# xiaoxiaokuye/CODLAD

Measured on AMD Instinct MI355X. Metric: sampled all-atom structures/sec (100-step DDPM, PED), higher is better.
Workload: dtype f32 as f16x3 split (each fp32 operand = fp16 hi + fp16 lo, 22-bit; 3 f16 MFMAs per product, fp32 accumulate); everything outside the contractions fp32; 1 GPU; cfg2: PED-shaped test set, 4 proteins L=46/87/92/129 x 10 frames x num_ensemble 10 = 400 structures per GPU, 100-step DDPM (mpnn_diffusion) + VQ(4096x3) + IC_Decoder N6 + ic_to_xyz; structures_rank0=400, nodes_rank0=35400, edges_rank0=2182800, ddpm_steps=100, parallelism=replicas x1

## Files before the change

codlad_amd/_lib.py:

```python
import ctypes as C
import os

import torch

_HERE = os.path.dirname(os.path.abspath(__file__))
ABI_VERSION = 19
LIB_PATH = os.environ.get("CODLAD_HIP_LIB") or os.path.join(_HERE, "libcodlad_hip.so")

P = C.c_void_p


class EncLayer(C.Structure):
    _fields_ = [(n, P) for n in ("W1e", "W2", "W3", "W11e", "W12", "W13", "W1a", "W1c", "W11a", "W11c")] + \
               [("Win", P * 4), ("Wout", P * 4)] + \
               [(n, P) for n in ("b1", "b2", "b3", "b11", "b12", "b13", "b_in", "b_out")]


class DecLayer(C.Structure):
    _fields_ = [(n, P) for n in ("W1e", "W2", "W3", "W1a", "W1v", "TS")] + \
               [("Win", P * 4), ("Wout", P * 4)] + \
               [(n, P) for n in ("b1", "b2", "b3", "b_in", "b_out")]


class EncLayerH(C.Structure):
    _fields_ = [(n, P) for n in ("W1e", "W2", "W3", "W11e", "W12", "W13", "W1a", "W1c", "W11a", "W11c")] + \
               [("Win", P * 4), ("Wout", P * 4)] + \
               [(n, P) for n in ("b1", "b2", "b3", "b11", "b12", "b13", "b_in", "b_out")] + \
               [(n, C.c_int) for n in ("e1", "e2", "e3", "e11", "e12", "e13", "e_in", "e_out")]


class DecLayerH(C.Structure):
    _fields_ = [(n, P) for n in ("W1e", "W2", "W3", "W1a", "W1v")] + [("Win", P * 4), ("Wout", P * 4)] + \
               [(n, P) for n in ("TS", "b1", "b2", "b3", "b_in", "b_out")] + \
               [(n, C.c_int) for n in ("e1", "e2", "e3", "e_in", "e_out")]


class DenoiserWeights(C.Structure):
    _fields_ = [(n, P) for n in ("freqs", "rbf_mu", "t_w0", "t_b0", "t_w2", "t_b2")] + \
               [("ada_w", P * 7), ("ada_b", P * 7)] + \
               [(n, P) for n in ("x_in_w", "x_in_b", "pos_w", "pos_b", "edge_wT", "norm_w", "norm_b",
                                 "We_wT", "We_b", "out_w", "out_b")] + \
               [("enc", EncLayer * 3), ("dec", DecLayer * 3), ("precision", C.c_int),
                ("enc_h", EncLayerH * 3), ("dec_h", DecLayerH * 3), ("self_condition", C.c_int), ("out_dim", C.c_int)]


class Workspace(C.Structure):
    _fields_ = [(n, P) for n in ("hV", "hVenc", "S", "PQ", "hE", "status", "tile_list")] + [("n_tiles", C.c_int32), ("xcd_bounds", P)]


class JobDesc(C.Structure):
    _fields_ = [("node_info", P), ("n_nodes", C.c_int), ("E_idx", P), ("h_E0", P), ("E1", P), ("n_snodes", C.c_int),
                ("ws", C.POINTER(Workspace))]


class DecoderWeights(C.Structure):
    _fields_ = [("angle", C.c_int), ("map_out_w", P), ("map_out_b", P), ("res_embed", P)] + \
               [(n, P * 4) for n in ("inv0_w", "inv0_b", "inv1_w", "inv1_b", "dist_w", "dist_b",
                                     "dense1_w", "dense1_b", "dense3_w", "dense3_b")] + \
               [(n, P) for n in ("bb_dist", "sc_dist", "bb_ang1_w", "bb_ang1_b", "bb_ang3_w", "bb_ang3_b",
                                 "sc_angle_emb", "sc_ang1_w", "sc_ang1_b", "sc_ang3_w", "sc_ang3_b",
                                 "bb_tor1_w", "bb_tor1_b", "bb_tor3_w", "bb_tor3_b")] + \
               [(n, P * 4) for n in ("tor1_w", "tor1_b", "tor3_w", "tor3_b")] + \
               [(n, P) for n in ("fin1_w", "fin1_b", "fin3_w", "fin3_b")]


class TpConvArgs(C.Structure):
    _fields_ = [("ptr", P), ("snd", P), ("n_recv", C.c_int32), ("xyz_recv", P), ("xyz_snd", P), ("typ_recv", P),
                ("typ_snd", P), ("r_sign", C.c_float), ("smear_stop", C.c_float), ("emb0_w", P), ("emb0_b", P),
                ("emb3_w", P), ("emb3_b", P), ("emb_in", C.c_int32), ("h_recv", P), ("d_recv", C.c_int32), ("h_snd", P),
                ("d_snd", C.c_int32), ("attr_recv_first", C.c_int32), ("fc0_w", P), ("fc0_b", P), ("fc3_w", P),
                ("fc3_b", P), ("depth", C.c_int32), ("out", P), ("accumulate", C.c_int32), ("group", C.c_int32),
                ("packed", P)]


class XyzGroup(C.Structure):
    _fields_ = [("ca_full", P), ("ic", P), ("orders", P), ("slot_to_out", P), ("xyz_out", P),
                ("B", C.c_int32), ("L", C.c_int32), ("n_atoms", C.c_int32), ("first_row", C.c_int32)]


class MetricInputs(C.Structure):
    _fields_ = [("xyz_recon", P), ("xyz", P), ("n_atoms", C.c_int64),
                ("edge_list", P), ("n_edges", C.c_int64), ("clash_list", P), ("n_clash", C.c_int64),
                ("bb_NO_list", P), ("n_bb", C.c_int64), ("interaction_list", P), ("n_inter", C.c_int64),
                ("pi_pi_list", P), ("n_pipi", C.c_int64),
                ("ic", P), ("ic_recon", P), ("ic_mask", P), ("n_ic", C.c_int64)]


class LossTerms(C.Structure):
    _fields_ = [(n, P) for n in ("kl", "nll", "vb", "mse", "xstart_mse", "eps_mse", "pred_xstart")]


class FmLossOut(C.Structure):
    _fields_ = [(n, P) for n in ("l2", "l1", "huber", "smooth_l1", "log_cosh")]


class OdeState(C.Structure):
    _fields_ = [(n, C.c_double) for n in ("t", "h", "t_end", "ratio", "hh")] + \
               [(n, C.c_int32) for n in ("accepted", "n_accept", "n_reject", "clipped", "nonfinite", "status")] + \
               [("hh_f", C.c_float), ("tf", C.c_float * 6), ("pad_", C.c_float)]


class OdeDopri5Bufs(C.Structure):
    _fields_ = [("y", P), ("y1", P), ("xin", P), ("k", P * 7), ("mods", P), ("state", P), ("norm", P)]


FM_KINDS = {"icfm": 0, "target": 1, "vp": 2}
FM_TARGET_FLOW = 3
ODE_METHODS = {"euler": 0, "midpoint": 1, "rk4": 2}
GEOM_BOND_FLAG = 1 << 30
STEREO_COLUMNS, STEREO_N_COUNTS, STEREO_KIND_PRO = 9, 6, 1
STEREO_FLAGS = {"inverted_ca": 1, "inverted_side": 2, "cis": 4, "twisted": 8, "undefined": 16}
SASA_MAX_POINTS = 1024
DSSP_MAX_RES = 4096
DSSP_CODES = " HBEGITS"
DSSP_KIND_PRO, DSSP_KIND_CHAIN_START, DSSP_GEOM_LINK, DSSP_GEOM_BEND, DSSP_UNDEFINED = 1, 2, 1, 2, 255
SAXS_MAX_Q, SAXS_MAX_TYPES, SAXS_Q_CHUNK = 512, 32, 16
SAXS_X_MAX, SAXS_X_SMALL, SAXS_SIN_ULPS = 25600.0, 0.125, 5
SAXS_HYD_PARTIALS, SAXS_HYD_Q_CHUNK, SAXS_HYD_MAX_GRID = 6, 8, 4096
ODE_NORM_WORDS = 257

_JOB = [C.POINTER(DenoiserWeights), C.POINTER(JobDesc)]

_SIGS = {
    "codlad_abi_version": (C.c_int, []),
    "codlad_probe_edge_launches": (C.c_int, [C.c_int]),
    "codlad_probe_read": (C.c_int, [C.c_int, C.POINTER(C.c_double)]),
    "codlad_dispatch_read": (C.c_int, [P, C.c_int]),
    "codlad_metrics_scratch_bytes": (C.c_int, []),
    "codlad_eval_metrics": (C.c_int, [C.POINTER(MetricInputs), P, P, P]),
    "codlad_bond_graph_counts": (C.c_int, [P, P, P, P, P, C.c_int, C.c_int, C.c_float, P, P]),
    "codlad_ens_moments": (C.c_int, [P, C.c_int, C.c_int, P, C.c_int, P, P]),
    "codlad_ens_pair_msd": (C.c_int, [P, P, C.c_int, P, P, C.c_int, C.c_int, P, C.c_int, P, C.c_int, C.c_int, P, P, P]),
    "codlad_ens_apply": (C.c_int, [P, P, C.c_int, C.c_int, P, P]),
    "codlad_ens_pairwise": (C.c_int, [P, P, C.c_int, C.c_int, C.c_int, P, C.c_int, C.c_int, P, P]),
    "codlad_geometry_check": (C.c_int, [P, C.c_int, C.c_int, P, P, P, P, C.c_int, C.c_float, C.c_float, C.c_float, P, P, P]),
    "codlad_stereo_check": (C.c_int, [P, C.c_int, C.c_int, P, P, C.c_int, P, P, P, P]),
    "codlad_relax_scratch_bytes": (C.c_longlong, [C.c_int] * 5),
    "codlad_relax_energy": (C.c_int, [P, P, C.c_int, C.c_int, P, P, P, P, P, P, C.c_int, P, C.c_int, P, P, C.c_int] +
                            [C.c_float] * 4 + [P] * 5),
    "codlad_relax": (C.c_int, [P, C.c_int, C.c_int, P, P, P, P, P, P, C.c_int, P, C.c_int, P, P, C.c_int] +
                     [C.c_float] * 6 + [C.c_int] + [P] * 9),
    "codlad_sasa": (C.c_int, [P, C.c_int, C.c_int, P, P, P, C.c_int, P, C.c_int, P, P, P, P, P, P]),
    "codlad_contact_counts": (C.c_int, [P, C.c_int, C.c_int, P, C.c_int, C.c_float, P, P]),
    "codlad_dssp_hbonds": (C.c_int, [P, C.c_int, C.c_int, P, P, C.c_int, P, P, P, P, P, P, P, P]),
    "codlad_dssp_assign": (C.c_int, [P, P, P, P, C.c_int, C.c_int, P, P, P, P]),
    "codlad_saxs_debye": (C.c_int, [P, C.c_int, C.c_int, P, C.c_int, P, P, C.c_int, P, P, P, P, P]),
    "codlad_saxs_partials": (C.c_int, [P, C.c_int, C.c_int, P, C.c_int, P, P, P, P, C.c_int, P, P, P, P, P]),
    "codlad_saxs_hydration_fit": (C.c_int, [P, C.c_int, C.c_int, P, P, C.c_int, P, C.c_int, P, P, P, P, P, P, P, P]),
    "codlad_last_error": (C.c_char_p, []),
    "codlad_struct_sizes": (None, [C.POINTER(C.c_int)]),
    "codlad_pack_block_host": (None, [P, C.c_int, C.c_float, P]),
    "codlad_features_prepass": (C.c_int, [C.POINTER(DenoiserWeights), P, P, C.c_int, C.c_int, P, P, P]),
    "codlad_step_mods": (C.c_int, [C.POINTER(DenoiserWeights), P, C.c_int, P, P]),
    "codlad_step_mods_f": (C.c_int, [C.POINTER(DenoiserWeights), P, C.c_int, P, P]),
    "codlad_ode_combine": (C.c_int, [P, P, P, C.c_int, C.c_float, C.c_size_t, P, P]),
    "codlad_ode_error_norm": (C.c_int, [P, P, P, C.c_size_t, C.c_float, C.c_float, P, P]),
    "codlad_ode_loop": (C.c_int, _JOB + [P, P, P, C.c_int, P, C.c_int, P, P]),
    "codlad_ode_dopri5_attempt": (C.c_int, _JOB + [C.POINTER(OdeDopri5Bufs), C.c_double, C.c_float, C.c_float, P]),
    "codlad_layer0_edge_terms": (C.c_int, [C.POINTER(DenoiserWeights), P, C.c_int, P, P, P]),
    "codlad_denoiser_forward": (C.c_int, _JOB + [P, P, P, P, P]),
    "codlad_status_check": (C.c_int, [P, P]),
    "codlad_set_option": (C.c_int, [C.c_int, C.c_int]),
    "codlad_edge_plan_host": (C.c_int, [P, C.c_int, C.c_int, C.c_int, C.c_int, P, P]),
    "codlad_ddpm_update": (C.c_int, [P, P, P, P, C.c_int, P, P, P]),
    "codlad_ddpm_pred_xstart": (C.c_int, [P, P, P, C.c_int, P, P]),
    "codlad_ddpm_posterior_step": (C.c_int, [P, P, P, P, P, P, C.c_float, C.c_int, P, P, P]),
    "codlad_sample_loop": (C.c_int, _JOB + [P, P, P, P, P, C.c_int, P]),
    "codlad_sample_loop_pinned": (C.c_int, _JOB + [P, P, P, P, P, C.c_int, P, P, P]),
    "codlad_ddim_loop": (C.c_int, _JOB + [P, P, P, P, P, C.c_int, C.c_int, C.c_int, P, P, P]),
    "codlad_ddim_step": (C.c_int, [P, P, P, P, P, C.c_int, C.c_int, P, P, P]),
    "codlad_dpm_loop": (C.c_int, _JOB + [P, P, P, P, C.c_int, C.c_int, P, P, P]),
    "codlad_dpm_step": (C.c_int, [P, P, P, P, P, C.c_int, P, P, P]),
    "codlad_q_sample": (C.c_int, [P, P, P, C.c_int, P, C.c_int, P, C.c_int, P, P, P, P]),
    "codlad_q_posterior": (C.c_int, [P, P, P, C.c_int, P, C.c_int, P, C.c_int, P, P, P, P]),
    "codlad_vb_terms": (C.c_int, [P, P, P, P, P, C.c_int, P, C.c_int, P, C.c_int, C.POINTER(LossTerms), P]),
    "codlad_prior_bpd": (C.c_int, [P, P, C.c_int, P, C.c_int, P, P]),
    "codlad_loss_forward": (C.c_int, _JOB + [P, P, P, P, P, P, C.c_int, C.c_int, P, C.c_int, P, C.POINTER(LossTerms), P]),
    "codlad_bpd_loop": (C.c_int, _JOB + [P, P, P, P, P, C.c_int, P, C.c_int, P, P, P, P, P, P]),
    "codlad_fm_path": (C.c_int, [P, P, P, P, C.c_int, P, C.c_float, C.c_int, C.c_double, P, P, P]),
    "codlad_fm_terms": (C.c_int, [P, P, P, C.c_int, C.POINTER(FmLossOut), P]),
    "codlad_fm_loss_forward": (C.c_int, _JOB + [P, P, P, P, C.c_int, P, C.POINTER(FmLossOut), P]),
    "codlad_fm_loss_loop": (C.c_int, _JOB + [P, P, P, C.c_int, C.c_double, P, C.c_int, P, P, C.c_int, P, P,
                                             C.POINTER(FmLossOut), P]),
    "codlad_vq_lookup": (C.c_int, [P, C.c_int, P, P, P, C.c_int, P, P, P, P]),
    "codlad_ic_decode": (C.c_int, [C.POINTER(DecoderWeights), P, P, P, P, P, C.c_int, P, P, P]),
    "codlad_cg_graph": (C.c_int, [P, P, C.c_int, C.c_float, P, P, P, P]),
    "codlad_ic_to_xyz": (C.c_int, [P, P, P, P, C.c_int, C.c_int, C.c_int, P, P]),
    "codlad_ic_to_xyz_groups": (C.c_int, [P, C.c_int, C.c_int, P]),
    "codlad_xyz_to_ic": (C.c_int, [P, C.c_int, C.c_int, P, C.c_int, P, P]),
    "codlad_tp_conv_image_bytes": (C.c_int, [C.c_int]),
    "codlad_tp_conv_pack": (C.c_int, [P, P, P]),
    "codlad_receiver_csr": (C.c_int, [P, C.c_int, C.c_int, C.c_int, P, P, P, P]),
    "codlad_bench_edge_launch": (C.c_int, [C.POINTER(DenoiserWeights), P, C.c_int, P, P, P,
                                           C.POINTER(Workspace), C.c_int, C.c_int, P]),
    "codlad_tp_conv": (C.c_int, [C.POINTER(TpConvArgs), P]),
    "codlad_tp_conv_args_size": (C.c_int, []),
    "codlad_mlp_rows": (C.c_int, [P, C.c_int, C.c_int, P, P, C.c_int, P, P, C.c_int, C.c_int, C.c_int, P, P]),
    "codlad_bead_mean": (C.c_int, [P, P, P, P, C.c_int, P, P]),
    "codlad_embed_rows": (C.c_int, [P, P, C.c_int, C.c_int, P, P]),
    "codlad_selftest_gemm128": (C.c_int, [P, P, P, C.c_int, C.c_int, P, P]),
    "codlad_selftest_gemm128_h": (C.c_int, [P, P, P, C.c_int, C.c_int, C.c_int, P, P]),
}

_lib = None


def lib():
    global _lib
    if _lib is None:
        if not os.path.exists(LIB_PATH):
            raise RuntimeError(
                f"{LIB_PATH} is missing: the HIP extension is the only implementation of this path "
                "(build it with `python -m codlad_amd.build`)")
        handle = C.CDLL(LIB_PATH, mode=C.RTLD_GLOBAL)
        for name, (res, args) in _SIGS.items():
            try:
                fn = getattr(handle, name)
            except AttributeError:
                raise RuntimeError(f"{LIB_PATH} does not export {name}: it was built from an older include/codlad_hip.h "
                                   f"(ABI version {ABI_VERSION} covers additions); rebuild it") from None
            fn.restype = res
            fn.argtypes = args
        if handle.codlad_abi_version() != ABI_VERSION:
            raise RuntimeError("libcodlad_hip.so ABI version mismatch")
        _lib = handle
    return _lib


OPT_NODEQ_MAX_TILES, OPT_EDGE_TILE_MAX_NODES, OPT_DEC_EDGE_VARIANT, OPT_TP_CONV_VARIANT, OPT_EDGE_UPD_VARIANT, OPT_EDGE_CUS, OPT_EDGE_WIDE_MAX_TILES, OPT_NODE_QUAD_MAX_TILES = 0, 1, 3, 4, 5, 6, 7, 2
OPT_EDGE_PAIR = 8
EDGE_GRID = (256, 8)


def edge_plan(K, pair=True, grid=EDGE_GRID):
    import numpy as np
    K = np.ascontiguousarray(K, dtype=np.int32)
    bounds, stats = np.zeros(9, dtype=np.int32), np.zeros(20, dtype=np.int64)
    check(lib().codlad_edge_plan_host(K.ctypes.data_as(P), K.shape[0], grid[0], grid[1], int(bool(pair)),
                                      bounds.ctypes.data_as(P), stats.ctypes.data_as(P)), "codlad_edge_plan_host")
    return bounds, stats


DISPATCH_WORDS = ("edge", "node_in", "node_upd", "chunked_in", "chunked_upd", "grid_edge_msg", "grid_edge_upd", "grid_node_in",
                  "grid_node_upd")
EDGE_KINDS = ("f32", "wide", "tile", "node", "node_upd1")
NODE_KINDS = ("f32", "w", "q", "h4", "h8")


def dispatch_read():
    out = (C.c_int32 * len(DISPATCH_WORDS))()
    n = lib().codlad_dispatch_read(out, len(DISPATCH_WORDS))
    if n != len(DISPATCH_WORDS):
        raise RuntimeError(f"codlad_dispatch_read: the library keeps {n} words, this binding knows {len(DISPATCH_WORDS)}")
    rec = dict(zip(DISPATCH_WORDS, (int(v) for v in out)))
    rec["edge"] = EDGE_KINDS[rec["edge"]]
    rec["node_in"], rec["node_upd"] = NODE_KINDS[rec["node_in"]], NODE_KINDS[rec["node_upd"]]
    rec["chunked_in"], rec["chunked_upd"] = bool(rec["chunked_in"]), bool(rec["chunked_upd"])
    return rec


def set_option(option, value):
    check(lib().codlad_set_option(option, value), "codlad_set_option")


def exported_symbols():
    return list(_SIGS)


def check(rc, what):
    if rc != 0:
        msg = lib().codlad_last_error().decode() or "unknown error"
        raise RuntimeError(f"{what} failed (rc={rc}): {msg}")


class _TensorPtr(C.c_void_p):
    """c_void_p that keeps its tensor alive for as long as the argument object lives, i.e. until
    the foreign call has been enqueued.  (A bare integer would let a temporary such as
    `x.contiguous()` be freed - and its block reused by the next temporary - before the launch.)"""


def ptr(t):
    if t is None:
        return None
    assert t.is_contiguous(), "non-contiguous tensor handed to the C ABI"
    p = _TensorPtr(t.data_ptr())
    p._keepalive = t
    return p


def stream_ptr(device=None):
    return C.c_void_p(torch.cuda.current_stream(device).cuda_stream)
```

codlad_amd/csrc/denoiser_forward.hip:

```cpp
#include "node_args.h"
#include "sampler_args.h"
#include "loss_args.h"
#include "flow_loss_args.h"
#include "ode_args.h"

static struct {
    int32_t v[CODLAD_DISPATCH_WORDS] = {};
    int grid_word = -1, node_word = -1, chunked_word = -1;
} g_dispatch;

void dispatch_note(int grid, int stream_waves, bool chunked) {
    if (g_dispatch.grid_word >= 0) g_dispatch.v[g_dispatch.grid_word] = grid;
    if (g_dispatch.node_word >= 0 && stream_waves)
        g_dispatch.v[g_dispatch.node_word] = stream_waves == 8 ? CODLAD_NODE_KIND_H8 : CODLAD_NODE_KIND_H4;
    if (g_dispatch.chunked_word >= 0) g_dispatch.v[g_dispatch.chunked_word] = chunked;
    g_dispatch.grid_word = g_dispatch.node_word = g_dispatch.chunked_word = -1;
}

extern "C" int codlad_dispatch_read(int32_t *out, int n) {
    CODLAD_REQUIRE(out && n >= 0, "bad arguments");
    for (int i = 0; i < n && i < CODLAD_DISPATCH_WORDS; ++i) out[i] = g_dispatch.v[i];
    return CODLAD_DISPATCH_WORDS;
}

static void launch_edge_now(bool update, const EdgeArgs &ea, int precision, hipStream_t st, const int2 *tile_list,
                            int n_tiles) {
    const int terms = precision == 2 ? 3 : (precision == 1 ? 4 : 0);
    auto kind = [&](int k) {
        if (k > g_dispatch.v[CODLAD_DISPATCH_EDGE]) g_dispatch.v[CODLAD_DISPATCH_EDGE] = k;
        g_dispatch.grid_word = update ? CODLAD_DISPATCH_GRID_EDGE_UPD : CODLAD_DISPATCH_GRID_EDGE_MSG;
    };
    if (!terms) { kind(CODLAD_EDGE_KIND_F32); return launch_edge_f32(update, ea, st); }
    if (tile_list && n_tiles <= option_value(CODLAD_OPT_EDGE_WIDE_MAX_TILES)) {
        kind(CODLAD_EDGE_KIND_WIDE);
        return launch_edge_wide(terms, update, ea, tile_list, n_tiles, st);
    }
    if (tile_list) { kind(CODLAD_EDGE_KIND_TILE); return launch_edge_tile(terms, update, ea, tile_list, n_tiles, st); }
    if (update) {
        const bool two_tiles_each = n_tiles > 0 && 20ll * n_tiles >= 19ll * 2 * ea.n_nodes;
        const int variant = option_value(CODLAD_OPT_EDGE_UPD_VARIANT);
        if ((variant == 1 && two_tiles_each) || variant == 2) {
            kind(CODLAD_EDGE_KIND_NODE_UPD1);
            launch_edge_upd1(terms, ea, st);
        } else {
            kind(CODLAD_EDGE_KIND_NODE);
            launch_edge_upd(terms, ea, st);
        }
    } else {
        kind(CODLAD_EDGE_KIND_NODE);
        launch_edge_msg(terms, ea, st);
    }
}

#define PROBE_MAX 4096
static struct {
    bool on = false;
    int used = 0;
    hipEvent_t ev[PROBE_MAX][2] = {};
    bool made[PROBE_MAX] = {};
    int kind[PROBE_MAX] = {};
} g_probe;

static void launch_edge(bool update, const EdgeArgs &ea, int precision, hipStream_t st, const int2 *tile_list = nullptr,
                        int n_tiles = 0) {
    const int i = g_probe.used;
    bool rec = g_probe.on && i < PROBE_MAX;
    if (rec && !g_probe.made[i]) {
        rec = hipEventCreate(&g_probe.ev[i][0]) == hipSuccess && hipEventCreate(&g_probe.ev[i][1]) == hipSuccess;
        g_probe.made[i] = rec;
    }
    if (rec) (void)hipEventRecord(g_probe.ev[i][0], st);
    launch_edge_now(update, ea, precision, st, tile_list, n_tiles);
    if (rec) {
        (void)hipEventRecord(g_probe.ev[i][1], st);
        g_probe.kind[i] = (update ? 1 : 0) + (ea.E1 ? 2 : 0);
        g_probe.used = i + 1;
    }
}

extern "C" int codlad_probe_edge_launches(int enable) {
    g_probe.on = enable != 0;
    if (enable) g_probe.used = 0;
    return 0;
}

extern "C" int codlad_probe_read(int kind, double *total_ms) {
    CODLAD_REQUIRE(total_ms && kind >= 0 && kind < 4, "bad arguments");
    double sum = 0.0;
    int n = 0;
    for (int i = 0; i < g_probe.used; ++i) {
        if (g_probe.kind[i] != kind) continue;
        float ms = 0.f;
        hipError_t e = hipEventSynchronize(g_probe.ev[i][1]);
        if (e == hipSuccess) e = hipEventElapsedTime(&ms, g_probe.ev[i][0], g_probe.ev[i][1]);
        if (e != hipSuccess) { codlad_set_error("codlad_probe_read: %s", hipGetErrorString(e)); return -(int)e - 1000; }
        sum += ms;
        ++n;
    }
    *total_ms = sum;
    return n;
}

static void launch_node(bool upd, const NodeArgs &na, int precision, hipStream_t st) {
    const int terms = precision == 2 ? 3 : (precision == 1 ? 4 : 0);
    auto kind = [&](int k) {
        g_dispatch.node_word = upd ? CODLAD_DISPATCH_NODE_UPD : CODLAD_DISPATCH_NODE_IN;
        g_dispatch.v[g_dispatch.node_word] = k;
        g_dispatch.grid_word = upd ? CODLAD_DISPATCH_GRID_NODE_UPD : CODLAD_DISPATCH_GRID_NODE_IN;
        g_dispatch.chunked_word = upd ? CODLAD_DISPATCH_CHUNKED_UPD : CODLAD_DISPATCH_CHUNKED_IN;
    };
    if (!terms) { kind(CODLAD_NODE_KIND_F32); return launch_node_f32(upd, na, st); }
    const int tiles = (na.n_nodes + 31) / 32;
    if (upd && tiles <= option_value(CODLAD_OPT_NODE_QUAD_MAX_TILES)) {
        kind(CODLAD_NODE_KIND_Q);
        launch_node_quad(terms, na, st);
    } else if (tiles <= option_value(CODLAD_OPT_NODEQ_MAX_TILES)) {
        kind(CODLAD_NODE_KIND_W);
        launch_node_wide(terms, upd, na, st);
    } else {
        kind(CODLAD_NODE_KIND_H4);
        launch_node_stream(terms, tiles > 4 * num_cu() ? 8 : 4, upd, na, st);
    }
}

struct Job {
    const codlad_denoiser_weights *w;
    const int4 *ni;
    const int32_t *E_idx;
    int n_nodes;
    const codlad_workspace *ws;
    bool split;
    float *PQ(int k) const { return ws->PQ + (size_t)k * n_nodes * HD; }
};
static Job make_job(const codlad_denoiser_weights *w, const codlad_job *d) {
    return {w, reinterpret_cast<const int4 *>(d->node_info), d->E_idx, d->n_nodes, d->ws, w->precision != 0};
}

static EdgeArgs edge_args(const Job &j, const float *hE_in, bool in_by_src) {
    EdgeArgs ea = {};
    ea.node_info = j.ni; ea.E_idx = j.E_idx; ea.n_nodes = j.n_nodes;
    ea.hE_in = hE_in; ea.in_by_src = in_by_src;
    ea.pair = option_value(CODLAD_OPT_EDGE_PAIR) != 0;
    ea.xcd_bounds = ea.pair ? j.ws->xcd_bounds : nullptr;
    return ea;
}
template <class Layer, class LayerH>
static EdgeArgs msg_args(const Job &j, const Layer &L, const LayerH &Lh, const float *hE_in, bool in_by_src) {
    EdgeArgs ea = edge_args(j, hE_in, in_by_src);
    ea.P = j.PQ(0); ea.Q = j.PQ(1); ea.W1 = L.W1e; ea.W2 = L.W2; ea.S = j.ws->S;
    ea.W1h = Lh.W1e; ea.W2h = Lh.W2;
    ea.b2 = j.split ? Lh.b2 : L.b2;
    ea.gelu_a = gelu_consts(j.split ? Lh.e1 : 0);
    ea.gelu_b = gelu_consts(j.split ? Lh.e1 + Lh.e2 : 0);
    ea.res_scale = 1.0f; ea.ln_eps = 1e-6f;
    return ea;
}
static EdgeArgs upd_args(const Job &j, const codlad_enc_layer &L, const codlad_enc_layer_h &Lh, const float *hE_in,
                         bool in_by_src, const float *m) {
    EdgeArgs eu = edge_args(j, hE_in, in_by_src);
    eu.hE_out = j.ws->hE;
    eu.P = j.PQ(2); eu.Q = j.PQ(3); eu.W1 = L.W11e; eu.W2 = L.W12; eu.W3 = L.W13;
    eu.mods3 = m + 6 * HD;
    eu.W1h = Lh.W11e; eu.W2h = Lh.W12; eu.W3h = Lh.W13;
    eu.b2 = j.split ? Lh.b12 : L.b12; eu.b3 = j.split ? Lh.b13 : L.b13;
    const int E2 = j.split ? Lh.e11 + Lh.e12 : 0, E3 = j.split ? E2 + Lh.e13 : 0;
    eu.gelu_a = gelu_consts(j.split ? Lh.e11 : 0);
    eu.gelu_b = gelu_consts(E2);
    eu.res_scale = pow2i(E3);
    eu.ln_eps = 1e-6f * pow2i(2 * E3);
    return eu;
}

static void set_node_scales(NodeArgs &na, bool split, int e_msg, int e3, int e_in, int e_out) {
    na.s_scale = 0.015625f * pow2i(split ? -e_msg : 0);
    na.t_scale = 64.0f * pow2i(split ? -e3 : 0);
    na.ffn_scale = pow2i(split ? -(e_in + e_out) : 0);
    na.gelu_ffn = gelu_consts(split ? e_in : 0);
}
template <class Layer, class LayerH>
static NodeArgs node_update_args(const Job &j, const Layer &L, const LayerH &Lh, const float *mods, bool s_partials) {
    NodeArgs na = {};
    na.node_info = j.ni; na.n_nodes = j.n_nodes; na.S = j.ws->S; na.hV = j.ws->hV; na.s_partials = s_partials;
    na.W3 = L.W3; na.b3 = j.split ? Lh.b3 : L.b3; na.mods = mods;
    na.b_in = j.split ? Lh.b_in : L.b_in; na.b_out = j.split ? Lh.b_out : L.b_out;
    set_node_scales(na, j.split, Lh.e1 + Lh.e2, Lh.e3, Lh.e_in, Lh.e_out);
    na.blk_h[0] = Lh.W3;
    for (int c = 0; c < 4; ++c) {
        na.Win[c] = L.Win[c]; na.Wout[c] = L.Wout[c];
        na.blk_h[1 + 2 * c] = Lh.Win[c]; na.blk_h[2 + 2 * c] = Lh.Wout[c];
    }
    return na;
}
static void add_proj(NodeArgs &na, int blk0, const float *W, const void *Wh, const float *b, float *out) {
    const int p = na.n_proj++;
    na.proj_w[p] = W; na.proj_b[p] = b; na.proj_out[p] = out;
    na.blk_h[blk0 + p] = Wh;
}
static void add_proj_dec_q(NodeArgs &na, const Job &j, const codlad_dec_layer &D, const codlad_dec_layer_h &Dh) {
    na.proj_flags[na.n_proj] = 3; na.TS = j.split ? Dh.TS : D.TS;
    add_proj(na, 9, D.W1v, Dh.W1v, nullptr, j.PQ(1));
}

static void enqueue_forward(const codlad_denoiser_weights *w, const codlad_job *job, const float *x,
                            const float *x_self_cond, const float *mods_t, hipStream_t st) {
    const Job j = make_job(w, job);
    const codlad_workspace *ws = job->ws;
    const int n_nodes = job->n_nodes;
    const float *h_E0 = job->h_E0, *E1 = job->E1;
    g_dispatch = {};
    const bool tilewise = j.split && ws->tile_list && ws->n_tiles > 0 &&
                          (ws->n_tiles <= 8 * num_cu() || ws->n_tiles <= option_value(CODLAD_OPT_EDGE_WIDE_MAX_TILES)) &&
                          n_nodes <= option_value(CODLAD_OPT_EDGE_TILE_MAX_NODES);
    const int2 *tile_list = tilewise ? reinterpret_cast<const int2 *>(ws->tile_list) : nullptr;

    {
        NodeArgs na = {};
        na.node_info = j.ni; na.n_nodes = n_nodes;
        na.x = x; na.x_in_w = w->x_in_w; na.x_in_b = w->x_in_b; na.hV = ws->hV;
        na.x_sc = x_self_cond; na.in_dim = w->self_condition ? 6 : 3;
        add_proj(na, 0, w->enc[0].W1a, w->enc_h[0].W1a, j.split ? w->enc_h[0].b1 : w->enc[0].b1, j.PQ(0));
        add_proj(na, 0, w->enc[0].W1c, w->enc_h[0].W1c, nullptr, j.PQ(1));
        set_node_scales(na, j.split, 0, 0, 0, 0);
        launch_node(false, na, w->precision, st);
    }
    for (int l = 0; l < 3; ++l) {
        const codlad_enc_layer &L = w->enc[l];
        const codlad_enc_layer_h &Lh = w->enc_h[l];
        const float *m = mods_t + mods_offset(l);
        const float *hE_in = l == 0 ? h_E0 : ws->hE;
        EdgeArgs ea = msg_args(j, L, Lh, hE_in, l == 0);
        if (l == 0 && E1) ea.E1 = E1;
        launch_edge(false, ea, w->precision, st, tile_list, ws->n_tiles);

        NodeArgs na = node_update_args(j, L, Lh, m, tilewise);
        add_proj(na, 9, L.W11a, Lh.W11a, j.split ? Lh.b11 : L.b11, j.PQ(2));
        add_proj(na, 9, L.W11c, Lh.W11c, nullptr, j.PQ(3));
        if (l < 2) {
            add_proj(na, 9, w->enc[l + 1].W1a, w->enc_h[l + 1].W1a, j.split ? w->enc_h[l + 1].b1 : w->enc[l + 1].b1, j.PQ(0));
            add_proj(na, 9, w->enc[l + 1].W1c, w->enc_h[l + 1].W1c, nullptr, j.PQ(1));
        } else {
            add_proj(na, 9, w->dec[0].W1a, w->dec_h[0].W1a, j.split ? w->dec_h[0].b1 : w->dec[0].b1, j.PQ(0));
            add_proj_dec_q(na, j, w->dec[0], w->dec_h[0]);
            na.hVenc_out = ws->hVenc; na.venc_is_self = 1;
        }
        launch_node(true, na, w->precision, st);

        EdgeArgs eu = upd_args(j, L, Lh, hE_in, l == 0, m);
        if (l == 0 && E1) eu.E1 = E1 + (size_t)job->n_snodes * 64 * HD;
        launch_edge(true, eu, w->precision, st, tile_list, ws->n_tiles);
    }
    for (int l = 0; l < 3; ++l) {
        const codlad_dec_layer &L = w->dec[l];
        const codlad_dec_layer_h &Lh = w->dec_h[l];
        launch_edge(false, msg_args(j, L, Lh, ws->hE, false), w->precision, st, tile_list, ws->n_tiles);

        NodeArgs na = node_update_args(j, L, Lh, mods_t + mods_offset(3 + l), tilewise);
        if (l < 2) {
            add_proj(na, 9, w->dec[l + 1].W1a, w->dec_h[l + 1].W1a, j.split ? w->dec_h[l + 1].b1 : w->dec[l + 1].b1, j.PQ(0));
            add_proj_dec_q(na, j, w->dec[l + 1], w->dec_h[l + 1]);
            na.hVenc_in = ws->hVenc;
        }
        launch_node(true, na, w->precision, st);
    }
}

static int check_ws(const codlad_workspace *ws) {
    return ws && ws->hV && ws->hVenc && ws->S && ws->PQ && ws->hE;
}

static const char *job_defect(const codlad_denoiser_weights *w, const codlad_job *job) {
    if (!w || !job || !job->node_info || !job->E_idx || !job->h_E0) return "null pointer";
    if (job->n_nodes <= 0) return "n_nodes must be positive";
    if (!check_ws(job->ws)) return "incomplete workspace";
    return nullptr;
}
#define REQUIRE_OK(defect) do { const char *msg_ = (defect); CODLAD_REQUIRE(!msg_, msg_); } while (0)

static HeadArgs head_args(const codlad_denoiser_weights *w, const codlad_job *job, const float *mods_t) {
    return {job->ws->hV, mods_t + mods_offset(6), w->out_w, w->out_b, job->n_nodes};
}

static FinalArgs final_args(const codlad_denoiser_weights *w, const codlad_job *job, const float *mods_t) {
    FinalArgs fa = {head_args(w, job, mods_t)};
    fa.status = job->ws->status; fa.n_out = w->out_dim;
    return fa;
}

extern "C" int codlad_denoiser_forward(const codlad_denoiser_weights *w, const codlad_job *job, const float *x,
                                       const float *x_self_cond, const float *mods_t, float *out, void *stream) {
    REQUIRE_OK(job_defect(w, job));
    CODLAD_REQUIRE(x && mods_t && out, "null pointer");
    hipStream_t st = (hipStream_t)stream;
    CODLAD_REQUIRE(!x_self_cond || w->self_condition, "x_self_cond given to a model without self-conditioning");
    CODLAD_REQUIRE(w->out_dim == 6 || w->out_dim == 3, "out_dim must be 6 (diffusion) or 3 (flow matching)");
    enqueue_forward(w, job, x, x_self_cond, mods_t, st);
    FinalArgs fa = final_args(w, job, mods_t);
    fa.logits = out;
    launch_final(fa, CODLAD_STEP_DDPM, nullptr, nullptr, 0, st);
    return codlad_check_launch("codlad_denoiser_forward");
}

static void sample_loop(const codlad_denoiser_weights *w, const codlad_job *job, float *x, float *x_start,
                        const float *noise, const float *mods, const float *coef, int T, const float *pin_x0,
                        const uint8_t *pin_mask, void *stream, int step = CODLAD_STEP_DDPM, int mode = 0) {
    hipStream_t st = (hipStream_t)stream;
    const bool sc = w->self_condition != 0;
    const bool reverse = step == CODLAD_STEP_DDIM_REVERSE;
    for (int k = 0; k < T; ++k) {
        const int i = reverse ? k : T - 1 - k;
        const float *mods_t = mods + (size_t)i * CODLAD_MODS_PER_STEP;
        enqueue_forward(w, job, x, sc && k > 0 ? x_start : nullptr, mods_t, st);
        FinalArgs fa = final_args(w, job, mods_t);
        fa.x = x; fa.noise = noise ? noise + (size_t)k * job->n_nodes * 3 : nullptr;
        fa.coef = coef + (size_t)i * 8; fa.x_start = x_start;
        launch_final(fa, step, pin_x0, pin_mask, mode, st);
    }
}

static const char *ddpm_loop_defect(const codlad_denoiser_weights *w, const codlad_job *job, const float *x,
                                    const float *x_start, const float *noise, const float *mods, const float *coef, int T) {
    if (const char *msg = job_defect(w, job)) return msg;
    if (!x || !noise || !mods || !coef) return "null pointer";
    if (T <= 0) return "T must be positive";
    if (w->self_condition && !x_start) return "a self-conditioned model needs the x_start buffer";
    if (w->out_dim != 6 && w->out_dim != 3)
        return "the DDPM loop needs a model with 6 outputs (mean | variance logits) or 3 (fixed-variance samplers)";
    return nullptr;
}

extern "C" int codlad_sample_loop(const codlad_denoiser_weights *w, const codlad_job *job, float *x, float *x_start,
                                  const float *noise, const float *mods, const float *coef, int T, void *stream) {
    REQUIRE_OK(ddpm_loop_defect(w, job, x, x_start, noise, mods, coef, T));
    sample_loop(w, job, x, x_start, noise, mods, coef, T, nullptr, nullptr, stream);
    return codlad_check_launch("codlad_sample_loop");
}

extern "C" int codlad_sample_loop_pinned(const codlad_denoiser_weights *w, const codlad_job *job, float *x,
                                         float *x_start, const float *noise, const float *mods, const float *coef, int T,
                                         const float *pin_x0, const uint8_t *pin_mask, void *stream) {
    REQUIRE_OK(ddpm_loop_defect(w, job, x, x_start, noise, mods, coef, T));
    CODLAD_REQUIRE(pin_x0 && pin_mask, "null pointer (pin_x0 / pin_mask)");
    sample_loop(w, job, x, x_start, noise, mods, coef, T, pin_x0, pin_mask, stream);
    return codlad_check_launch("codlad_sample_loop_pinned");
}

extern "C" int codlad_ddim_loop(const codlad_denoiser_weights *w, const codlad_job *job, float *x, float *x_start,
                                const float *noise, const float *mods, const float *coef, int T, int mode, int reverse,
                                const float *pin_x0, const uint8_t *pin_mask, void *stream) {
    CODLAD_REQUIRE(w && x && mods && coef, "null pointer");
    CODLAD_REQUIRE(reverse || noise, "null pointer (noise: only the reverse loop runs without it)");
    CODLAD_REQUIRE(!pin_x0 == !pin_mask, "null pointer (pin_x0 and pin_mask come together)");
    CODLAD_REQUIRE(T > 0, "T must be positive");
    CODLAD_REQUIRE(mode >= 0 && mode <= (CODLAD_DDPM_START_X | CODLAD_DDPM_FIXED_VAR | CODLAD_DDPM_CLIP),
                   "unknown mode bits");
    CODLAD_REQUIRE(w->out_dim == ((mode & CODLAD_DDPM_FIXED_VAR) ? 3 : 6),
                   "mode and model disagree: a learned-range sampler needs a model with 6 outputs (mean | variance "
                   "logits), a fixed-variance one (mode bit 2) a model with 3");
    CODLAD_REQUIRE(!w->self_condition || x_start, "a self-conditioned model needs the x_start buffer");
    REQUIRE_OK(job_defect(w, job));
    sample_loop(w, job, x, x_start, noise, mods, coef, T, pin_x0, pin_mask, stream,
                reverse ? CODLAD_STEP_DDIM_REVERSE : CODLAD_STEP_DDIM, mode);
    return codlad_check_launch("codlad_ddim_loop");
}

extern "C" int codlad_dpm_loop(const codlad_denoiser_weights *w, const codlad_job *job, float *x, float *x_start,
                               const float *mods, const float *coef, int T, int mode, const float *pin_x0,
                               const uint8_t *pin_mask, void *stream) {
    CODLAD_REQUIRE(w && x && mods && coef, "null pointer");
    CODLAD_REQUIRE(x_start, "null pointer (x_start: the multistep update reads the previous step's pred_xstart from it)");
    CODLAD_REQUIRE(!pin_x0 == !pin_mask, "null pointer (pin_x0 and pin_mask come together)");
    CODLAD_REQUIRE(T > 0, "T must be positive");
    CODLAD_REQUIRE(mode >= 0 && mode <= (CODLAD_DDPM_START_X | CODLAD_DDPM_FIXED_VAR | CODLAD_DDPM_CLIP),
                   "unknown mode bits");
    CODLAD_REQUIRE(w->out_dim == ((mode & CODLAD_DDPM_FIXED_VAR) ? 3 : 6),
                   "mode and model disagree: a learned-range sampler needs a model with 6 outputs (mean | variance "
                   "logits), a fixed-variance one (mode bit 2) a model with 3");
    REQUIRE_OK(job_defect(w, job));
    sample_loop(w, job, x, x_start, nullptr, mods, coef, T, pin_x0, pin_mask, stream, CODLAD_STEP_DPM, mode);
    return codlad_check_launch("codlad_dpm_loop");
}

static LossArgs loss_args(const codlad_denoiser_weights *w, const codlad_job *job, const float *mods_t,
                          const float *x_start, const float *x_t, const float *noise, const LossSamples &s) {
    LossArgs la = {};
    la.head = final_args(w, job, mods_t);
    la.x0 = x_start; la.xt = x_t; la.noise = noise; la.s = s;
    return la;
}

static const char *loss_model_defect(const codlad_denoiser_weights *w, const codlad_job *job, int T, int n_samples) {
    if (const char *msg = job_defect(w, job)) return msg;
    if (T <= 0 || n_samples <= 0) return "T and n_samples must be positive";
    if (w->out_dim != 6 && w->out_dim != 3)
        return "the loss needs a model with 6 outputs (mean | variance logits) or 3 (fixed-variance samplers)";
    return nullptr;
}

extern "C" int codlad_loss_forward(const codlad_denoiser_weights *w, const codlad_job *job, const float *x_start,
                                   const float *x_t, const float *noise, const float *x_self_cond, const float *mods_t,
                                   const float *coef, int T, int t, const int32_t *sample_off, int n_samples,
                                   float *model_out, const codlad_loss_terms *terms, void *stream) {
    REQUIRE_OK(loss_model_defect(w, job, T, n_samples));
    CODLAD_REQUIRE(x_start && x_t && mods_t && coef && sample_off && terms, "null pointer");
    CODLAD_REQUIRE(t >= 0 && t < T, "t outside [0, T)");
    CODLAD_REQUIRE(!x_self_cond || w->self_condition, "x_self_cond given to a model without self-conditioning");
    hipStream_t st = (hipStream_t)stream;
    enqueue_forward(w, job, x_t, x_self_cond, mods_t, st);
    LossArgs la = loss_args(w, job, mods_t, x_start, x_t, noise, {sample_off, nullptr, t, T, n_samples, coef});
    la.head.logits = model_out;
    la.out = *terms;
    launch_loss(la, st);
    return codlad_check_launch("codlad_loss_forward");
}

extern "C" int codlad_bpd_loop(const codlad_denoiser_weights *w, const codlad_job *job, const float *x_start,
                               const float *noise, float *x_t, const float *mods, const float *coef, int T,
                               const int32_t *sample_off, int n_samples, float *vb, float *mse, float *xstart_mse,
                               float *prior_bpd, float *total_bpd, void *stream) {
    REQUIRE_OK(loss_model_defect(w, job, T, n_samples));
    CODLAD_REQUIRE(x_start && noise && x_t && mods && coef && sample_off, "null pointer");
    CODLAD_REQUIRE(vb && mse && xstart_mse && prior_bpd && total_bpd, "null pointer (results)");
    hipStream_t st = (hipStream_t)stream;
    for (int k = 0; k < T; ++k) {
        const int i = T - 1 - k;
        const LossSamples s = {sample_off, nullptr, i, T, n_samples, coef};
        const float *eps = noise + (size_t)k * job->n_nodes * 3;
        const float *mods_t = mods + (size_t)i * CODLAD_MODS_PER_STEP;
        launch_q_affine(x_start, eps, 8, 9, 10, 11, s, x_t, nullptr, nullptr, st);
        enqueue_forward(w, job, x_t, nullptr, mods_t, st);
        LossArgs la = loss_args(w, job, mods_t, x_start, x_t, eps, s);
        la.out.vb = vb + (size_t)i * n_samples;
        la.out.eps_mse = mse + (size_t)i * n_samples;
        la.out.xstart_mse = xstart_mse + (size_t)i * n_samples;
        launch_loss(la, st);
    }
    launch_prior(x_start, {sample_off, nullptr, T - 1, T, n_samples, coef}, vb, prior_bpd, total_bpd, st);
    return codlad_check_launch("codlad_bpd_loop");
}

static FmLossArgs fm_loss_args(const codlad_denoiser_weights *w, const codlad_job *job, const float *mods_t, const float *ut,
                               const int32_t *sample_off, int n_samples) {
    FmLossArgs la = {};
    la.head = final_args(w, job, mods_t);
    la.ut = ut; la.sample_off = sample_off; la.n_samples = n_samples;
    return la;
}

static const char *fm_model_defect(const codlad_denoiser_weights *w, const codlad_job *job, int n_samples) {
    if (const char *msg = job_defect(w, job)) return msg;
    if (n_samples <= 0) return "n_samples must be positive";
    if (w->out_dim != 3) return "the flow-matching losses need a flow-matching model (3 outputs: the velocity)";
    return nullptr;
}

extern "C" int codlad_fm_loss_forward(const codlad_denoiser_weights *w, const codlad_job *job, const float *xt,
                                      const float *ut, const float *mods_t, const int32_t *sample_off, int n_samples,
                                      float *model_out, const codlad_fm_loss_out *terms, void *stream) {
    REQUIRE_OK(fm_model_defect(w, job, n_samples));
    CODLAD_REQUIRE(xt && ut && mods_t && sample_off && terms, "null pointer");
    hipStream_t st = (hipStream_t)stream;
    enqueue_forward(w, job, xt, nullptr, mods_t, st);
    FmLossArgs la = fm_loss_args(w, job, mods_t, ut, sample_off, n_samples);
    la.head.logits = model_out;
    la.out = *terms;
    launch_fm_loss(la, st);
    return codlad_check_launch("codlad_fm_loss_forward");
}

extern "C" int codlad_fm_loss_loop(const codlad_denoiser_weights *w, const codlad_job *job, const float *x0, const float *x1,
                                   const float *eps, int kind, double sigma, const float *t_host, int K, const float *mods,
                                   const int32_t *sample_off, int n_samples, float *xt, float *ut,
                                   const codlad_fm_loss_out *tables, void *stream) {
    REQUIRE_OK(fm_model_defect(w, job, n_samples));
    CODLAD_REQUIRE(t_host && mods && sample_off && xt && ut && tables, "null pointer");
    CODLAD_REQUIRE(K > 0, "K must be positive");
    CODLAD_REQUIRE(kind != CODLAD_FM_TARGET_FLOW, "unknown matcher kind (the loop draws its own locations)");
    for (int k = 0; k < K; ++k) REQUIRE_OK(fm_path_defect(x0, x1, eps, nullptr, t_host[k], kind, sigma));
    hipStream_t st = (hipStream_t)stream;
    const size_t n3 = (size_t)job->n_nodes * 3;
    for (int k = 0; k < K; ++k) {
        const float *mods_t = mods + (size_t)k * CODLAD_MODS_PER_STEP;
        launch_fm_path(fm_path_args(x0, x1, eps ? eps + (size_t)k * n3 : nullptr, {sample_off, nullptr, t_host[k], n_samples},
                                    kind, sigma, xt, ut), st);
        enqueue_forward(w, job, xt, nullptr, mods_t, st);
        FmLossArgs la = fm_loss_args(w, job, mods_t, ut, sample_off, n_samples);
        const size_t row = (size_t)k * n_samples;
        la.out.l2 = tables->l2 ? tables->l2 + row : nullptr;
        la.out.l1 = tables->l1 ? tables->l1 + row : nullptr;
        la.out.huber = tables->huber ? tables->huber + row : nullptr;
        la.out.smooth_l1 = tables->smooth_l1 ? tables->smooth_l1 + row : nullptr;
        la.out.log_cosh = tables->log_cosh ? tables->log_cosh + row : nullptr;
        launch_fm_loss(la, st);
    }
    return codlad_check_launch("codlad_fm_loss_loop");
}

static OdeStageArgs ode_stage_args(const codlad_denoiser_weights *w, const codlad_job *job, const float *mods_t) {
    OdeStageArgs a = {head_args(w, job, mods_t)};
    a.status = job->ws->status; a.self = -1;
    return a;
}

struct OdeRow {
    int n_k;
    int k[4];
    double coef[4];
};
static const OdeRow ODE_EULER[1] = {{1, {0}, {1.0}}};
static const OdeRow ODE_MIDPOINT[2] = {{1, {0}, {0.5}}, {1, {1}, {1.0}}};
static const OdeRow ODE_RK4[4] = {{1, {0}, {1.0 / 3}},
                                  {2, {1, 0}, {1.0, -1.0 / 3}},
                                  {3, {0, 1, 2}, {1.0, -1.0, 1.0}},
                                  {4, {0, 1, 2, 3}, {0.125, 0.375, 0.375, 0.125}}};

extern "C" int codlad_ode_loop(const codlad_denoiser_weights *w, const codlad_job *job, const float *y, float *traj,
                               const float *mods, int method, const float *dt_host, int n_intervals, float *scratch,
                               void *stream) {
    REQUIRE_OK(job_defect(w, job));
    CODLAD_REQUIRE(y && traj && mods && dt_host && scratch, "null pointer");
    CODLAD_REQUIRE(n_intervals > 0, "n_intervals must be positive");
    CODLAD_REQUIRE(method >= CODLAD_ODE_EULER && method <= CODLAD_ODE_RK4, "unknown method id");
    CODLAD_REQUIRE(w->out_dim == 3, "the ODE samplers need a flow-matching model (3 outputs: the velocity)");
    hipStream_t st = (hipStream_t)stream;
    const OdeRow *rows = method == CODLAD_ODE_EULER ? ODE_EULER : (method == CODLAD_ODE_MIDPOINT ? ODE_MIDPOINT : ODE_RK4);
    const int stages = method == CODLAD_ODE_EULER ? 1 : (method == CODLAD_ODE_MIDPOINT ? 2 : 4);
    const size_t n3 = (size_t)job->n_nodes * 3;
    float *xin = scratch + 4 * n3;
    if (y != traj) {
        hipError_t e = hipMemcpyAsync(traj, y, n3 * sizeof(float), hipMemcpyDeviceToDevice, st);
        if (e != hipSuccess) {
            codlad_set_error("codlad_ode_loop: %s", hipGetErrorString(e));
            return (int)e;
        }
    }
    for (int i = 0; i < n_intervals; ++i) {
        const float *y_i = traj + (size_t)i * n3;
        for (int s = 0; s < stages; ++s) {
            const float *mods_t = mods + ((size_t)i * stages + s) * CODLAD_MODS_PER_STEP;
            enqueue_forward(w, job, s == 0 ? y_i : xin, nullptr, mods_t, st);
            OdeStageArgs a = ode_stage_args(w, job, mods_t);
            a.k_out = scratch + s * n3; a.y = y_i; a.h = dt_host[i];
            a.n_k = rows[s].n_k;
            for (int m = 0; m < a.n_k; ++m) {
                a.k[m] = scratch + rows[s].k[m] * n3;
                a.coef[m] = (float)rows[s].coef[m];
                if (rows[s].k[m] == s) a.self = m;
            }
            a.out = s == stages - 1 ? traj + (size_t)(i + 1) * n3 : xin;
            launch_ode_stage(a, st);
        }
    }
    return codlad_check_launch("codlad_ode_loop");
}

static const double DP_BETA[6][6] = {{1.0 / 5},
                                     {3.0 / 40, 9.0 / 40},
                                     {44.0 / 45, -56.0 / 15, 32.0 / 9},
                                     {19372.0 / 6561, -25360.0 / 2187, 64448.0 / 6561, -212.0 / 729},
                                     {9017.0 / 3168, -355.0 / 33, 46732.0 / 5247, 49.0 / 176, -5103.0 / 18656},
                                     {35.0 / 384, 0.0, 500.0 / 1113, 125.0 / 192, -2187.0 / 6784, 11.0 / 84}};
static const double DP_C_SOL[7] = {35.0 / 384, 0.0, 500.0 / 1113, 125.0 / 192, -2187.0 / 6784, 11.0 / 84, 0.0};
static const double DP_C_ERR[7] = {35.0 / 384 - 1951.0 / 21600, 0.0, 500.0 / 1113 - 22642.0 / 50085,
                                   125.0 / 192 - 451.0 / 720, -2187.0 / 6784 - -12231.0 / 42400,
                                   11.0 / 84 - 649.0 / 6300, -1.0 / 60.0};

extern "C" int codlad_ode_dopri5_attempt(const codlad_denoiser_weights *w, const codlad_job *job,
                                         const codlad_ode_dopri5_bufs *bufs, double t_end, float rtol, float atol,
                                         void *stream) {
    REQUIRE_OK(job_defect(w, job));
    CODLAD_REQUIRE(bufs, "null pointer");
    CODLAD_REQUIRE(bufs->y && bufs->y1 && bufs->xin && bufs->mods && bufs->state && bufs->norm, "null pointer (buffers)");
    for (int j = 0; j < 7; ++j) CODLAD_REQUIRE(bufs->k[j], "null pointer (slopes)");
    CODLAD_REQUIRE(w->out_dim == 3, "the ODE samplers need a flow-matching model (3 outputs: the velocity)");
    hipStream_t st = (hipStream_t)stream;
    const size_t n3 = (size_t)job->n_nodes * 3;
    const float *hh = &bufs->state->hh_f;
    launch_ode_times(bufs->state, t_end, (float)DP_BETA[0][0], bufs->y, bufs->k[0], bufs->xin, n3, st);
    const int rc = codlad_step_mods_f(w, bufs->state->tf, 6, bufs->mods, stream);
    if (rc) return rc;
    for (int i = 0; i < 6; ++i) {
        const float *mods_t = bufs->mods + (size_t)i * CODLAD_MODS_PER_STEP;
        enqueue_forward(w, job, bufs->xin, nullptr, mods_t, st);
        OdeStageArgs a = ode_stage_args(w, job, mods_t);
        a.k_out = bufs->k[i + 1]; a.y = bufs->y; a.h_dev = hh; a.self = i + 1;
        const double *coef = i < 5 ? DP_BETA[i + 1] : DP_C_SOL;
        a.n_k = i + 2;
        for (int m = 0; m < a.n_k; ++m) {
            a.k[m] = bufs->k[m];
            a.coef[m] = (float)coef[m];
        }
        a.out = i < 5 ? bufs->xin : bufs->y1;
        launch_ode_stage(a, st);
    }
    OdeNormArgs na = {};
    na.y = bufs->y; na.y1 = bufs->y1; na.h_dev = hh; na.n = n3; na.rtol = rtol; na.atol = atol; na.out = bufs->norm;
    na.state = bufs->state; na.status = job->ws->status;
    for (int m = 0; m < 7; ++m) {
        na.k[m] = bufs->k[m];
        na.c_err[m] = (float)DP_C_ERR[m];
    }
    launch_ode_norm(na, st);
    launch_ode_commit(bufs->state, bufs->y, bufs->y1, bufs->k[0], bufs->k[6], n3, st);
    return codlad_check_launch("codlad_ode_dopri5_attempt");
}

extern "C" int codlad_bench_edge_launch(const codlad_denoiser_weights *w, const int32_t *node_info,
                                        int n_nodes, const int32_t *E_idx, const float *h_E0,
                                        const float *mods_t, const codlad_workspace *ws, int which,
                                        int layer, void *stream) {
    const codlad_job desc = {node_info, n_nodes, E_idx, h_E0, nullptr, 0, ws}, *job = &desc;
    REQUIRE_OK(job_defect(w, job));
    CODLAD_REQUIRE(mods_t, "null pointer");
    CODLAD_REQUIRE((which == 0 || which == 1) && (layer == 0 || layer == 1), "bad arguments");
    const Job j = make_job(w, job);
    const codlad_enc_layer &L = w->enc[layer];
    const codlad_enc_layer_h &Lh = w->enc_h[layer];
    const float *hE_in = layer == 0 ? h_E0 : ws->hE;
    EdgeArgs ea = which == 0 ? msg_args(j, L, Lh, hE_in, layer == 0) : upd_args(j, L, Lh, hE_in, layer == 0, mods_t);
    ea.S = ws->S;
    launch_edge(which == 1, ea, w->precision, (hipStream_t)stream, nullptr, ws->n_tiles);
    return codlad_check_launch("codlad_bench_edge_launch");
}
```

codlad_amd/csrc/edge_args.h:

```cpp
#pragma once
#include "common.h"
#include "host_util.h"

#define HD 128

struct EdgeArgs {
    const int4 *node_info;
    const int32_t *E_idx;
    const float *hE_in;
    int in_by_src;
    const float *E1;
    float *hE_out;
    const float *P, *Q;
    const float *W1, *W2, *W3;
    const void *W1h, *W2h, *W3h;
    const float *b2, *b3;
    const float *mods3;
    float *S;
    int n_nodes;
    GeluK gelu_a, gelu_b;
    float res_scale, ln_eps;
    const int32_t *xcd_bounds;
    int pair;
};

struct EdgeTileArgs : EdgeArgs {
    const int2 *tile_list;
    int n_tiles;
};

#define LDS_BLOCK_U4 4096

constexpr int NODE_WG_TILE = 256;
constexpr int XCD_CHUNKED_NODE_KERNEL_MIN = 32768;
__host__ __device__ inline int xcd_chunk_nodes(int n_nodes) {
    const int g = n_nodes >= XCD_CHUNKED_NODE_KERNEL_MIN ? NODE_WG_TILE : 32;
    const int tiles = (n_nodes + g - 1) / g;
    return g * ((tiles + 7) / 8);
}

__host__ __device__ inline bool edge_node_eligible(int K) { return K <= 16 || (K > 32 && K <= 48); }
__host__ __device__ inline bool edge_pair_ok(int K, int K_next) {
    return K > 32 && K <= 48 && edge_node_eligible(K_next);
}
__host__ __device__ inline int edge_node_cost2(int K) { return K <= 32 ? 2 : (K <= 48 ? 3 : 4); }
constexpr int XCD_BOUND_GRANULE = 32;

struct NodeSpan {
    int first, end, stride;
};
__host__ __device__ inline NodeSpan node_span_of(int n_nodes, int nwaves, int wave, int nb, int b, const int32_t *bounds) {
    if (nb % 8) return {b * nwaves + wave, n_nodes, nb * nwaves};
    int lo, hi;
    if (bounds) {
        lo = bounds[b % 8];
        hi = bounds[b % 8 + 1];
    } else {
        const int chunk = xcd_chunk_nodes(n_nodes);
        lo = (b % 8) * chunk;
        hi = lo + chunk;
    }
    if (lo > n_nodes) lo = n_nodes;
    if (hi > n_nodes) hi = n_nodes;
    return {lo + (b / 8) * nwaves + wave, hi, (nb / 8) * nwaves};
}
DEV NodeSpan wave_node_span(int n_nodes, int nwaves, int wave, const int32_t *bounds = nullptr) {
    return node_span_of(n_nodes, nwaves, wave, gridDim.x, blockIdx.x, bounds);
}

constexpr int UPD_W1_KS = 3;
constexpr int EDGE_CONST_U4 = 4 * 32;
template <bool EDGE_UPDATE, int NWAVES>
constexpr int edge_lds_u4() {
    return 2 * LDS_BLOCK_U4 + (EDGE_UPDATE ? UPD_W1_KS * 512 : 0) + EDGE_CONST_U4 + NWAVES * 32;
}
```

codlad_amd/csrc/edge_msg_kernel.hip:

```cpp
#include "edge_args.h"

constexpr int MSG_PAIR_U4 = 32 + 64 + 16;

template <int NWAVES, bool HOISTED, int TERMS>
__global__ __launch_bounds__(NWAVES * 64, NWAVES / 4) void msg_kernel_h(EdgeArgs a) {
    extern __shared__ __align__(16) u32x4 wl[];
    constexpr int NT = NWAVES * 64;
    const int tid = threadIdx.x, lane = tid & 63, wave = __builtin_amdgcn_readfirstlane(tid >> 6);
    u32x4 *consts = wl + 2 * LDS_BLOCK_U4;
    {
        const u32x4 *g1 = reinterpret_cast<const u32x4 *>(a.W1h);
        const u32x4 *g2 = reinterpret_cast<const u32x4 *>(a.W2h);
        for (int i = tid; i < LDS_BLOCK_U4; i += NT) {
            if (!HOISTED) wl[i] = g1[i];
            wl[LDS_BLOCK_U4 + i] = g2[i];
        }
        if (tid < 32) consts[tid] = reinterpret_cast<const u32x4 *>(a.b2)[tid];
        u32x4 *rep = consts + EDGE_CONST_U4 + NWAVES * 32;
        if (tid < 128) {
            const unsigned bv = reinterpret_cast<const unsigned *>(a.b2)[tid];
            for (int q = 0; q < 4; ++q) rep[q * 128 + tid] = u32x4{bv, bv, bv, bv};
        }
    }
    __syncthreads();
    const u32x4 *w1 = wl, *w2 = wl + LDS_BLOCK_U4;
    const float *c_b2 = reinterpret_cast<const float *>(consts);
    const int h = lane >> 5, c = lane & 31;
    float2 *const Pslot0 = reinterpret_cast<float2 *>(consts + EDGE_CONST_U4 + wave * 32);
    float2 *const Pslot1 = reinterpret_cast<float2 *>(consts + EDGE_CONST_U4 + NWAVES * 32 + 4 * 128 + wave * MSG_PAIR_U4);
    float4 *wait_sum = reinterpret_cast<float4 *>(Pslot1 + 64) + lane;
    int *wait_j = reinterpret_cast<int *>(Pslot1 + 64 + 2 * 64) + lane;
    const NodeSpan span = wave_node_span(a.n_nodes, NWAVES, wave, a.xcd_bounds);
    const int stride = span.stride, n_end = span.end;
    int n = __builtin_amdgcn_readfirstlane(span.first);
    if (n >= n_end) return;

    const float *xsrc = HOISTED ? a.E1 : a.hE_in;
    const bool by_src = HOISTED || a.in_by_src;
    const float2 *Prows = reinterpret_cast<const float2 *>(a.P);

    int4 info = a.node_info[n];
    int src = __builtin_amdgcn_readfirstlane(info.x), base = __builtin_amdgcn_readfirstlane(info.y);
    int K = __builtin_amdgcn_readfirstlane(info.z);
    int jA = a.E_idx[(size_t)src * 64 + (c < K ? c : 0)];
    int jB = a.E_idx[(size_t)src * 64 + (32 + c < K ? 32 + c : 0)];
    int cs = 0;
    Pslot0[lane] = Prows[(size_t)n * 64 + lane];
    int half = 0;
    int ph = 0, wn = 0, wait_src = 0, wait_base = 0, wK = 0;
    Tile x, acc, t2;
    tile_load_edge<!HOISTED>(x, xsrc + (size_t)(by_src ? src : n) * EDGE_BLOCK, c < K ? c : 0, h);
    tile_load_row(acc, a.Q + (size_t)(base + jA) * HD, h);
    float sum[4] = {0.f, 0.f, 0.f, 0.f};
    const float4 *bias_rep = reinterpret_cast<const float4 *>(consts + EDGE_CONST_U4 + NWAVES * 32) + c;

    int4 ninfo = info;
    int nsrc = src, nbase = base, nK = K, njA = jA, njB = jB;
    float2 npv = {0.f, 0.f};
    for (;;) {
        const int n2 = n + stride;
        const bool next_node = n2 < n_end;
        const bool first_half = half == 0;
        if (first_half && next_node) ninfo = a.node_info[n2];
        {
            const float2 *pl = ((ph == 2 && c < 16) ? !cs : cs) ? Pslot1 : Pslot0;
            tile_add_row(acc, reinterpret_cast<const float *>(pl), h);
        }
        if (HOISTED) {
#pragma unroll
            for (int bo = 0; bo < 4; ++bo) acc.b[bo] += x.b[bo];
        } else {
            gemm128_h_lds<TERMS, false, false, true>(acc, x, w1, lane, a.gelu_a);
        }
        if (first_half && next_node) {
            nsrc = __builtin_amdgcn_readfirstlane(ninfo.x);
            nbase = __builtin_amdgcn_readfirstlane(ninfo.y);
            nK = __builtin_amdgcn_readfirstlane(ninfo.z);
            njA = a.E_idx[(size_t)nsrc * 64 + (c < nK ? c : 0)];
            njB = a.E_idx[(size_t)nsrc * 64 + (32 + c < nK ? 32 + c : 0)];
            npv = Prows[(size_t)n2 * 64 + lane];
        }
        const bool open_pair = a.pair && ph == 0 && first_half && next_node && edge_pair_ok(K, nK);
        const bool next_half = first_half && K > 32 && !open_pair;
        const bool shared_next = ph == 1 || (open_pair && nK <= 32);
        {
            int rep_off = 0;
            asm volatile("" : "+v"(rep_off));
            const float4 *br = bias_rep + rep_off;
#pragma unroll
            for (int bo = 0; bo < 4; ++bo)
#pragma unroll
                for (int q = 0; q < 4; ++q) {
                    const float4 bv = br[q * 128 + 32 * bo];
                    t2.b[bo][4 * q + 0] = bv.x; t2.b[bo][4 * q + 1] = bv.y;
                    t2.b[bo][4 * q + 2] = bv.z; t2.b[bo][4 * q + 3] = bv.w;
                }
        }
        gemm128_h_lds<TERMS, true, true>(t2, acc, w2, lane, a.gelu_a);
        {
            int fn = next_half ? n : (next_node ? n2 : n), fs = next_half ? src : nsrc;
            int fb = next_half ? base : nbase, fK = next_half ? K : nK;
            int sn = fn, ss = fs, sb = fb, sK = fK;
            int jl = next_half ? jB : njA, jh = jl;
            int lo_off = next_half ? 32 : 0, hi_off = lo_off;
            if (shared_next) {
                if (ph == 1) {
                    fn = wn; fs = wait_src; fb = wait_base; fK = wK;
                    sn = n; ss = src; sb = base; sK = K;
                    jl = *wait_j;
                    jh = __shfl(jB, lane - 16);
                } else {
                    fn = n; fs = src; fb = base; fK = K;
                    sn = n2; ss = nsrc; sb = nbase; sK = nK;
                    jl = jB;
                    jh = __shfl(njA, lane - 16);
                }
                lo_off = 32;
                hi_off = (sK > 32 ? 32 : 0) - 16;
            }
            const bool low = c < 16;
            const int want = (low ? lo_off : hi_off) + c;
            const int pe = want < (low ? fK : sK) ? want : 0;
            const float *fblk = xsrc + (size_t)(by_src ? fs : fn) * EDGE_BLOCK, *sblk = xsrc + (size_t)(by_src ? ss : sn) * EDGE_BLOCK;
            const int pq = low ? fb + jl : sb + jh;
            tile_load_edge<!HOISTED>(x, low ? fblk : sblk, pe, h);
            tile_load_row(acc, a.Q + (size_t)pq * HD, h);
            __builtin_amdgcn_sched_barrier(0);
        }
        tile_gelu(t2, a.gelu_b);
        const int cnt = K - 32 * half;
        if (ph == 2) {
            const int wcnt = wK - 32;
            const float4 ws4 = *wait_sum;
            const float wsum[4] = {ws4.x, ws4.y, ws4.z, ws4.w};
#pragma unroll
            for (int bo = 0; bo < 4; ++bo) {
                float s0 = 0.f, s1 = 0.f;
#pragma unroll
                for (int r = 0; r < 8; ++r) {
                    s0 += ((r & 3) + 8 * (r >> 2) + 4 * h < wcnt) ? t2.b[bo][r] : 0.f;
                    s1 += ((r & 3) + 8 * (r >> 2) + 4 * h < cnt) ? t2.b[bo][8 + r] : 0.f;
                }
                sum[bo] += s1;
                const float ws = wsum[bo] + s0;
                const float tot = ws + __shfl_xor(ws, 32);
                if (h == 0) a.S[(size_t)wn * HD + 32 * bo + c] = tot;
            }
        } else if (cnt >= 32) {
#pragma unroll
            for (int bo = 0; bo < 4; ++bo) {
                f32x2 s2 = tile_pair(t2.b[bo], 0);
#pragma unroll
                for (int r = 2; r < 16; r += 2) s2 += tile_pair(t2.b[bo], r);
                sum[bo] += s2.x + s2.y;
            }
        } else {
#pragma unroll
            for (int bo = 0; bo < 4; ++bo) {
                float s0 = 0.f;
#pragma unroll
                for (int r = 0; r < 16; ++r) s0 += ((r & 3) + 8 * (r >> 2) + 4 * h < cnt) ? t2.b[bo][r] : 0.f;
                sum[bo] += s0;
            }
        }
        if (next_half) {
            half = 1;
            if (ph == 1) ph = 2;
            continue;
        }
        if (open_pair) {
            *wait_sum = make_float4(sum[0], sum[1], sum[2], sum[3]);
            *wait_j = jB;
#pragma unroll
            for (int bo = 0; bo < 4; ++bo) sum[bo] = 0.f;
            wn = n; wait_src = src; wait_base = base; wK = K;
            ph = nK > 32 ? 1 : 2;
            cs ^= 1;
        } else {
#pragma unroll
            for (int bo = 0; bo < 4; ++bo) {
                const float tot = sum[bo] + __shfl_xor(sum[bo], 32);
                if (h == 0) a.S[(size_t)n * HD + 32 * bo + c] = tot;
                sum[bo] = 0.f;
            }
            if (!next_node) break;
            ph = 0;
        }
        n = n2; src = nsrc; base = nbase; K = nK; jA = njA; jB = njB;
        (cs ? Pslot1 : Pslot0)[lane] = npv;
        half = 0;
    }
}


template <int TERMS>
static void launch_msg_t(const EdgeArgs &ea, hipStream_t st) {
    static bool attr_set = false;
    constexpr int NW = 8;
    const size_t lds = 16 * (edge_lds_u4<false, NW>() + 4 * 128 + NW * MSG_PAIR_U4);
    static_assert(16 * (edge_lds_u4<false, NW>() + 4 * 128 + NW * MSG_PAIR_U4) <= 160 * 1024, "kernel exceeds the CU's LDS");
    if (!attr_set) {
        set_max_lds(reinterpret_cast<const void *>(msg_kernel_h<NW, false, TERMS>), lds);
        set_max_lds(reinterpret_cast<const void *>(msg_kernel_h<NW, true, TERMS>), lds);
        attr_set = true;
    }
    const int groups = (ea.n_nodes + NW - 1) / NW;
    dim3 grid(groups < edge_cus() ? groups : edge_cus()), block(NW * 64);
    dispatch_note(grid.x);
    if (ea.E1 != nullptr) hipLaunchKernelGGL((msg_kernel_h<NW, true, TERMS>), grid, block, lds, st, ea);
    else hipLaunchKernelGGL((msg_kernel_h<NW, false, TERMS>), grid, block, lds, st, ea);
}

void launch_edge_msg(int terms, const EdgeArgs &ea, hipStream_t st) {
    if (terms == 3) launch_msg_t<3>(ea, st);
    else launch_msg_t<4>(ea, st);
}
```

codlad_amd/csrc/edge_plan.hip:

```cpp
#include "edge_args.h"
#include <vector>

static int64_t chunk_walk(const int32_t *K, int lo, int hi, int stride, bool pair, int64_t *pairs) {
    int64_t tiles = 0;
    for (int w = 0; w < stride; ++w)
        for (int n = lo + w; n < hi; n += stride) {
            tiles += K[n] > 32 ? 2 : 1;
            if (pair && n + stride < hi && edge_pair_ok(K[n], K[n + stride])) {
                n += stride;
                tiles += (K[n] > 32 ? 2 : 1) - 1;
                if (pairs) ++*pairs;
            }
        }
    return tiles;
}

extern "C" int codlad_edge_plan_host(const int32_t *K_host, int n_nodes, int n_workgroups, int waves_per_workgroup,
                                     int pair, int32_t *bounds_host, int64_t *stats_host) {
    CODLAD_REQUIRE(K_host && n_nodes > 0 && n_workgroups > 0 && waves_per_workgroup > 0, "bad arguments");
    int32_t bounds[9];
    const int G = XCD_BOUND_GRANULE, ng = (n_nodes + G - 1) / G;
    std::vector<int64_t> upto(ng + 1, 0);
    int64_t plain = 0;
    for (int n = 0; n < n_nodes; ++n) {
        CODLAD_REQUIRE(K_host[n] >= 1 && K_host[n] <= 64, "K outside 1..64");
        plain += K_host[n] > 32 ? 2 : 1;
        upto[n / G + 1] += pair ? edge_node_cost2(K_host[n]) : (K_host[n] > 32 ? 4 : 2);
    }
    for (int g = 0; g < ng; ++g) upto[g + 1] += upto[g];
    const int64_t total = upto[ng];
    const bool chunked = n_workgroups % 8 == 0;
    const int stride = chunked ? n_workgroups / 8 * waves_per_workgroup : n_workgroups * waves_per_workgroup;
    auto node_of = [&](int g) { return g * G < n_nodes ? g * G : n_nodes; };
    if (pair) {
        double target = total / 16.0;
        for (int pass = 0; pass < (chunked ? 3 : 1); ++pass) {
            bounds[0] = 0;
            int g = 0;
            int64_t done = 0;
            for (int x = 1; x < 8; ++x) {
                const int g0 = g;
                if (pass == 0) {
                    while (g < ng && 8 * upto[g + 1] <= total * x) ++g;
                    if (g < ng && 8 * upto[g + 1] - total * x < total * x - 8 * upto[g]) ++g;
                } else {
                    auto f = [&](int gg) { return (double)(done + chunk_walk(K_host, node_of(g0), node_of(gg), stride, true, nullptr)); };
                    const double want = target * x;
                    while (g < ng && f(g) < want) ++g;
                    while (g > g0 && f(g - 1) >= want) --g;
                    if (g > g0 && want - f(g - 1) < f(g) - want) --g;
                }
                bounds[x] = node_of(g);
                if (chunked) done += chunk_walk(K_host, node_of(g0), node_of(g), stride, true, nullptr);
            }
            bounds[8] = n_nodes;
            if (chunked) target = (done + chunk_walk(K_host, bounds[7], n_nodes, stride, true, nullptr)) / 8.0;
        }
    } else {
        const int chunk = xcd_chunk_nodes(n_nodes);
        for (int x = 0; x <= 8; ++x) bounds[x] = (int64_t)x * chunk < n_nodes ? x * chunk : n_nodes;
    }
    if (bounds_host)
        for (int x = 0; x <= 8; ++x) bounds_host[x] = bounds[x];
    if (stats_host) {
        int64_t walk = 0, pairs = 0;
        for (int x = 0; x < 8; ++x) {
            const int lo = (bounds[x] + G - 1) / G, hi = (bounds[x + 1] + G - 1) / G;
            stats_host[4 + x] = upto[hi] - upto[lo];
            stats_host[12 + x] = chunked ? chunk_walk(K_host, bounds[x], bounds[x + 1], stride, pair != 0, &pairs) : 0;
            walk += stats_host[12 + x];
        }
        if (!chunked) walk = chunk_walk(K_host, 0, n_nodes, stride, pair != 0, &pairs);
        stats_host[0] = plain;
        stats_host[1] = total;
        stats_host[2] = walk;
        stats_host[3] = pairs;
    }
    return 0;
}
```

codlad_amd/csrc/edge_upd_kernel.hip:

```cpp
#include "edge_args.h"

template <int NWAVES, bool HOISTED, int TERMS>
__global__ __launch_bounds__(NWAVES * 64, NWAVES / 4) void upd_kernel_h(EdgeArgs a) {
    extern __shared__ __align__(16) u32x4 wl[];
    constexpr int NT = NWAVES * 64;
    constexpr int W1_U4 = UPD_W1_KS * 512;
    const int tid = threadIdx.x, lane = tid & 63, wave = __builtin_amdgcn_readfirstlane(tid >> 6);
    u32x4 *consts = wl + 2 * LDS_BLOCK_U4 + W1_U4;
    {
        const u32x4 *g1 = reinterpret_cast<const u32x4 *>(a.W1h);
        const u32x4 *g2 = reinterpret_cast<const u32x4 *>(a.W2h);
        const u32x4 *g3 = reinterpret_cast<const u32x4 *>(a.W3h);
        for (int i = tid; i < LDS_BLOCK_U4; i += NT) {
            wl[i] = g2[i];
            wl[LDS_BLOCK_U4 + i] = g3[i];
        }
        if (!HOISTED)
            for (int i = tid; i < W1_U4; i += NT) wl[2 * LDS_BLOCK_U4 + i] = g1[i];
        if (tid < 32) consts[tid] = reinterpret_cast<const u32x4 *>(a.b2)[tid];
        if (tid >= 64 && tid < 96) consts[32 + (tid & 31)] = reinterpret_cast<const u32x4 *>(a.b3)[tid & 31];
        if (tid >= 128 && tid < 160) {
            const float4 *m = reinterpret_cast<const float4 *>(a.mods3);
            const int i = tid & 31;
            const float4 s = m[i], c = m[32 + i], g = m[64 + i];
            float4 *cf = reinterpret_cast<float4 *>(consts);
            cf[64 + i] = make_float4(g.x * (1.0f + c.x), g.y * (1.0f + c.y), g.z * (1.0f + c.z), g.w * (1.0f + c.w));
            cf[96 + i] = make_float4(g.x * s.x, g.y * s.y, g.z * s.z, g.w * s.w);
        }
    }
    __syncthreads();
    const u32x4 *w2 = wl, *w3 = wl + LDS_BLOCK_U4, *w1 = wl + 2 * LDS_BLOCK_U4;
    const float *c_base = reinterpret_cast<const float *>(consts);
    float *Pslot = reinterpret_cast<float *>(consts + EDGE_CONST_U4 + wave * 32);
    const int h = lane >> 5, c = lane & 31;
    const NodeSpan span = wave_node_span(a.n_nodes, NWAVES, wave, a.xcd_bounds);
    int pend_n = -1, pend_src = 0, pend_base = 0, pend_K = 0;
    for (int nv = span.first; nv < span.end; nv += span.stride) {
        const int n = __builtin_amdgcn_readfirstlane(nv);
        const int4 info = a.node_info[n];
        const int src = __builtin_amdgcn_readfirstlane(info.x), base = __builtin_amdgcn_readfirstlane(info.y);
        const int K = __builtin_amdgcn_readfirstlane(info.z);
        const int Ku = K, lh = Ku > 32;
        const bool paired = pend_n >= 0;
        bool open_pair = false;
        if (a.pair && !paired && Ku > 32 && Ku <= 48 && n + span.stride < span.end)
            open_pair = edge_pair_ok(Ku, __builtin_amdgcn_readfirstlane(a.node_info[n + span.stride].z));
        const bool ptA = paired && !lh, ptB = paired && lh;
        const bool lowA = ptA && c < 16, lowB = ptB && c < 16;
        const int wantA = ptA ? (c < 16 ? 32 + c : c - 16) : c, wantB = ptB ? 32 + (c & 15) : 32 + c;
        const bool validA = wantA < (lowA ? pend_K : K), validB = wantB < (lowB ? pend_K : K);
        const int colA = validA ? wantA : 0, colB = validB ? wantB : 0;
        const int jA = a.E_idx[(size_t)(lowA ? pend_src : src) * 64 + colA];
        const int jB = a.E_idx[(size_t)(lowB ? pend_src : src) * 64 + colB];
        reinterpret_cast<float2 *>(Pslot)[lane] = reinterpret_cast<const float2 *>(a.P + (size_t)n * HD)[lane];

        for (int half = 0; half < 2; ++half) {
            if (32 * half >= K) break;
            if (half && open_pair) break;
            const bool ptile = half ? ptB : ptA, low = half ? lowB : lowA;
            const bool valid = half ? validB : validA;
            const int colc = half ? colB : colA;
            const int j = half ? jB : jA;
            const int base_l = low ? pend_base : base;
            const float *rows_n = a.hE_in + (size_t)(a.in_by_src ? src : n) * EDGE_BLOCK;
            const float *rows_p = a.hE_in + (size_t)(a.in_by_src ? pend_src : pend_n) * EDGE_BLOCK;
            const float *rows = low ? rows_p : rows_n;
            float *out_rows = a.hE_out + (size_t)(low ? pend_n : n) * EDGE_BLOCK;
            Tile x, acc, t2;
            StreamedGemm<TERMS, UPD_W1_KS, 8 - UPD_W1_KS, false, 8, true> tail1;
            float2 pend_p = {0.f, 0.f};
            if (ptile) pend_p = reinterpret_cast<const float2 *>(a.P + (size_t)pend_n * HD)[lane];
            if (!HOISTED) tail1.start(a.W1h, lane);
            int lds_off = 0;
            asm volatile("" : "+v"(lds_off));
            const float *c_b2 = c_base + lds_off, *c_b3 = c_b2 + HD;
            const float *c_modA = c_b2 + 2 * HD, *c_modB = c_b2 + 3 * HD;
            tile_load_row(acc, a.Q + (size_t)(base_l + j) * HD, h);
            if (!low) tile_add_row(acc, Pslot, h);
            if (ptile) {
                reinterpret_cast<float2 *>(Pslot)[lane] = pend_p;
                if (low) tile_add_row(acc, Pslot, h);
            }
            if (!HOISTED) tile_load_edge<true>(x, rows, colc, h);
            if (HOISTED) {
                tile_add_edge(acc, low ? a.E1 + (size_t)pend_src * EDGE_BLOCK : a.E1 + (size_t)src * EDGE_BLOCK, colc, h);
                __builtin_amdgcn_sched_barrier(0);
                tile_load_edge<false>(x, rows, colc, h);
            } else {
                gemm_h_lds<TERMS, 0, UPD_W1_KS, false, false, true>(acc, x, w1, lane, a.gelu_a);
                tail1.run(acc, x, lane, a.gelu_a);
            }
            tile_load_row(t2, c_b2, h);
            gemm128_h_lds<TERMS, true>(t2, acc, w2, lane, a.gelu_a);
            tile_unsplit_scale_add_row(x, a.res_scale, c_b3, h);
            gemm128_h_lds<TERMS, true>(x, t2, w3, lane, a.gelu_b);
            tile_layernorm_affine(x, a.ln_eps, c_modA, c_modB, h);
            tile_presplit(x);
            if (valid) tile_store_edge<true>(x, out_rows, colc, h);
        }
        if (open_pair) {
            pend_n = n;
            pend_src = src;
            pend_base = base;
            pend_K = K;
        } else pend_n = -1;
    }
}


template <int TERMS>
static void launch_upd_t(const EdgeArgs &ea, hipStream_t st) {
    static bool attr_set = false;
    constexpr int NW = 8;
    const size_t lds = 16 * edge_lds_u4<true, NW>();
    static_assert(16 * edge_lds_u4<true, NW>() <= 160 * 1024, "kernel exceeds the CU's LDS");
    if (!attr_set) {
        set_max_lds(reinterpret_cast<const void *>(upd_kernel_h<NW, false, TERMS>), lds);
        set_max_lds(reinterpret_cast<const void *>(upd_kernel_h<NW, true, TERMS>), lds);
        attr_set = true;
    }
    const int groups = (ea.n_nodes + NW - 1) / NW;
    dim3 grid(groups < edge_cus() ? groups : edge_cus()), block(NW * 64);
    dispatch_note(grid.x);
    if (ea.E1 != nullptr) hipLaunchKernelGGL((upd_kernel_h<NW, true, TERMS>), grid, block, lds, st, ea);
    else hipLaunchKernelGGL((upd_kernel_h<NW, false, TERMS>), grid, block, lds, st, ea);
}

void launch_edge_upd(int terms, const EdgeArgs &ea, hipStream_t st) {
    if (terms == 3) launch_upd_t<3>(ea, st);
    else launch_upd_t<4>(ea, st);
}
```

codlad_amd/csrc/host_util.h:

```cpp
#pragma once
#include <hip/hip_runtime.h>
#include "../../include/codlad_hip.h"

struct EdgeArgs;
struct NodeArgs;
struct FinalArgs;

int num_cu();
void set_max_lds(const void *fn, size_t bytes);
hipError_t codlad_take_attr_error();
int option_value(int opt);
int edge_cus();
void codlad_set_error(const char *fmt, ...);
inline int codlad_hip_failed(const char *what, hipError_t e) {
    codlad_set_error("%s: %s", what, hipGetErrorString(e));
    return (int)e;
}
void dispatch_note(int grid, int stream_waves = 0, bool chunked = false);

void launch_edge_f32(bool update, const EdgeArgs &ea, hipStream_t st);
void launch_node_f32(bool upd, const NodeArgs &na, hipStream_t st);
void launch_edge_tile(int terms, bool update, const EdgeArgs &ea, const int2 *tile_list, int n_tiles, hipStream_t st);
void launch_edge_wide(int terms, bool update, const EdgeArgs &ea, const int2 *tile_list, int n_tiles, hipStream_t st);
void launch_edge_msg(int terms, const EdgeArgs &ea, hipStream_t st);
void launch_edge_upd(int terms, const EdgeArgs &ea, hipStream_t st);
void launch_edge_upd1(int terms, const EdgeArgs &ea, hipStream_t st);
void launch_node_wide(int terms, bool upd, const NodeArgs &na, hipStream_t st);
void launch_node_quad(int terms, const NodeArgs &na, hipStream_t st);
void launch_node_stream(int terms, int waves, bool upd, const NodeArgs &na, hipStream_t st);
void launch_final(const FinalArgs &fa, int step, const float *pin_x0, const uint8_t *pin_mask, int mode, hipStream_t st);
void launch_tp_conv_mfma(const codlad_tp_conv_args &a, hipStream_t st);
void launch_tp_conv_pack(const codlad_tp_conv_args &a, void *image, hipStream_t st);
int tp_conv_image_bytes(int depth);
```

codlad_amd/csrc/host_util.hip:

```cpp
#include "host_util.h"
#include "common.h"
#include <stdlib.h>

int num_cu() {
    static int n_cu = 0;
    if (!n_cu) {
        int dev = 0, n = 0;
        if (hipGetDevice(&dev) != hipSuccess ||
            hipDeviceGetAttribute(&n, hipDeviceAttributeMultiprocessorCount, dev) != hipSuccess || n <= 0)
            n = 256;
        n_cu = n;
    }
    return n_cu;
}

static hipError_t g_attr_error = hipSuccess;
void set_max_lds(const void *fn, size_t bytes) {
    const hipError_t e = hipFuncSetAttribute(fn, hipFuncAttributeMaxDynamicSharedMemorySize, (int)bytes);
    if (e != hipSuccess && g_attr_error == hipSuccess) g_attr_error = e;
}
hipError_t codlad_take_attr_error() {
    const hipError_t e = g_attr_error;
    g_attr_error = hipSuccess;
    return e;
}

struct Option {
    int id;
    const char *env;
    int (*dflt)();
    int value = -1;
};
static Option g_options[] = {
    {CODLAD_OPT_NODEQ_MAX_TILES, "CODLAD_NODEQ_MAX_TILES", [] { return 256; }},
    {CODLAD_OPT_EDGE_TILE_MAX_NODES, "CODLAD_EDGE_TILE_MAX_NODES", [] { return 1 << 30; }},
    {CODLAD_OPT_NODE_QUAD_MAX_TILES, "CODLAD_NODE_QUAD_MAX_TILES", [] { return 2 * num_cu(); }},
    {CODLAD_OPT_DEC_EDGE_VARIANT, "CODLAD_DEC_EDGE_VARIANT", [] { return 0; }},
    {CODLAD_OPT_TP_CONV_VARIANT, "CODLAD_TP_CONV_VARIANT", [] { return 0; }},
    {CODLAD_OPT_EDGE_UPD_VARIANT, "CODLAD_EDGE_UPD_VARIANT", [] { return 0; }},
    {CODLAD_OPT_EDGE_CUS, "CODLAD_EDGE_CUS", [] { return 0; }},
    {CODLAD_OPT_EDGE_WIDE_MAX_TILES, "CODLAD_EDGE_WIDE_MAX_TILES", [] { return 22 * num_cu(); }},
    {CODLAD_OPT_EDGE_PAIR, "CODLAD_EDGE_PAIR", [] { return 1; }},
};
static_assert(sizeof(g_options) / sizeof(g_options[0]) == CODLAD_N_OPTIONS, "one row per CODLAD_OPT_*");

int option_value(int opt) {
    Option &o = g_options[opt];
    if (o.id != opt) abort();
    if (o.value < 0) {
        const char *e = getenv(o.env);
        o.value = e ? atoi(e) : o.dflt();
    }
    return o.value;
}

extern "C" int codlad_set_option(int option, int value) {
    CODLAD_REQUIRE(option >= 0 && option < CODLAD_N_OPTIONS && value >= 0, "unknown option or negative value");
    g_options[option].value = value;
    return 0;
}

int edge_cus() {
    const int v = option_value(CODLAD_OPT_EDGE_CUS);
    return v > 0 && v < num_cu() ? v : num_cu();
}
```

codlad_amd/engine.py:

```python
import ctypes as C
import os

import numpy as np
import torch

from . import _lib
from .weights import DEFAULT_PRECISION, DenoiserWeights, DecoderWeights

H = 128
KNN = 64
MODS = 6016


def _require_cuda(t, what):
    if not t.is_cuda:
        raise RuntimeError(f"{what} must live on the GPU: this path has no CPU implementation")


def edge_rows(blocks, split=False):
    lead = blocks.shape[:-4]
    if not split:
        return blocks.permute(*range(len(lead)), -4, -2, -3, -1).reshape(*lead, 64, -1)
    hv = blocks.contiguous().view(torch.float16).view(*lead, 2, 4, 2, 2, 2, 32, 8)
    val = hv[..., 0, :, :, :].float() + hv[..., 1, :, :, :].float()
    n = len(lead)
    val = val.permute(*range(n), n, n + 4, n + 1, n + 2, n + 3, n + 5)
    out = torch.empty(*lead, 2, 32, 4, 2, 16, dtype=torch.float32, device=blocks.device)
    for h in range(2):
        out[..., 4 * h:4 * h + 4] = val[..., h, 0:4]
        out[..., 8 + 4 * h:8 + 4 * h + 4] = val[..., h, 4:8]
    return out.reshape(*lead, 64, 128)


class Structures:

    def __init__(self, xyz_list, z_list, device):
        self.lens = [int(x.shape[0]) for x in xyz_list]
        assert all(L >= 1 for L in self.lens)
        self.offsets = np.concatenate([[0], np.cumsum(self.lens)]).astype(np.int64)
        self.n_snodes = int(self.offsets[-1])
        self.xyz = torch.cat([x.reshape(-1, 3).float() for x in xyz_list]).contiguous().to(device)
        self.z = torch.cat([z.reshape(-1).to(torch.int32) for z in z_list]).contiguous().to(device)
        info = np.empty((self.n_snodes, 2), dtype=np.int32)
        for f, L in enumerate(self.lens):
            info[self.offsets[f]:self.offsets[f + 1], 0] = self.offsets[f]
            info[self.offsets[f]:self.offsets[f + 1], 1] = L
        self.snode_info = torch.from_numpy(info).to(device)
        self.E_idx = None
        self.h_E0 = None
        self.E1 = None
        self.features_tag = None


class Job:

    def __init__(self, structures, sample_struct, device, edge_state=None):
        st = structures
        self.structures = st
        self.device = device
        self._parts = {}
        self.sample_struct = [int(s) for s in sample_struct]
        lens = [st.lens[f] for f in self.sample_struct]
        self.sample_lens = lens
        self.sample_off = np.concatenate([[0], np.cumsum(lens)]).astype(np.int64)
        self.n_nodes = int(self.sample_off[-1])
        info = np.empty((self.n_nodes, 4), dtype=np.int32)
        z_host = st.z.cpu().numpy()
        for s, f in enumerate(self.sample_struct):
            a, b = self.sample_off[s], self.sample_off[s + 1]
            L = lens[s]
            info[a:b, 0] = np.arange(st.offsets[f], st.offsets[f] + L)
            info[a:b, 1] = a
            info[a:b, 2] = min(KNN, L)
            info[a:b, 3] = z_host[st.offsets[f]:st.offsets[f] + L]
        assert info[:, 3].min() >= 0 and info[:, 3].max() < 30, "residue type outside W_s vocabulary"
        self.node_info = torch.from_numpy(info).to(device)
        n = self.n_nodes
        f32 = dict(dtype=torch.float32, device=device)
        self.hV = torch.empty(n, H, **f32)
        self.hVenc = torch.empty(n, H, **f32)
        self.S = torch.empty(4, n, H, **f32)
        self.PQ = torch.empty(4, n, H, **f32)
        self.hE = torch.empty(n, KNN, H, **f32) if edge_state is None else edge_state
        assert tuple(self.hE.shape) == (n, KNN, H) and self.hE.is_contiguous()
        self.status = torch.zeros(1, dtype=torch.int32, device=device)
        halves = np.where(info[:, 2] > 32, 2, 1)
        tiles = np.empty((int(halves.sum()), 2), dtype=np.int32)
        tiles[:, 0] = np.repeat(np.arange(n, dtype=np.int32), halves)
        first = np.cumsum(halves) - halves
        tiles[:, 1] = np.arange(tiles.shape[0], dtype=np.int32) - np.repeat(first, halves).astype(np.int32)
        self.tile_list = torch.from_numpy(tiles).to(device)
        ws = _lib.Workspace()
        ws.hV, ws.hVenc, ws.S, ws.PQ, ws.hE, ws.status, ws.tile_list = (
            _lib.ptr(t) for t in (self.hV, self.hVenc, self.S, self.PQ, self.hE, self.status, self.tile_list))
        ws.n_tiles = tiles.shape[0]
        self.xcd_bounds = torch.from_numpy(_lib.edge_plan(info[:, 2])[0]).to(device)
        ws.xcd_bounds = _lib.ptr(self.xcd_bounds)
        self.ws = ws

    def workspace_bytes(self):
        return 4 * (self.hV.numel() * 2 + self.S.numel() + self.PQ.numel() + self.hE.numel())

    def desc(self):
        st = self.structures
        d = _lib.JobDesc()
        d.node_info, d.n_nodes = _lib.ptr(self.node_info), self.n_nodes
        d.E_idx, d.h_E0, d.E1, d.n_snodes = _lib.ptr(st.E_idx), _lib.ptr(st.h_E0), _lib.ptr(st.E1), st.n_snodes
        d.ws = C.pointer(self.ws)
        return d

    def sub_job(self, members, start):
        n = int(sum(self.sample_lens[m] for m in members))
        sub = Job(self.structures, [self.sample_struct[m] for m in members], self.device,
                  edge_state=self.hE[start:start + n])
        idx = np.concatenate([np.arange(self.sample_off[m], self.sample_off[m + 1]) for m in members])
        return sub, torch.from_numpy(idx).to(self.device)

    def parts(self, k=2):
        if k not in self._parts:
            subs, start = [], 0
            for p in range(k):
                subs.append(self.sub_job(range(p, len(self.sample_struct), k), start))
                start += subs[-1][0].n_nodes
            self._parts[k] = subs
        return self._parts[k]


class Denoiser:

    def __init__(self, state_dict, device, precision=DEFAULT_PRECISION, block_exponents=True, self_condition=False,
                 out_dim=6):
        self.device = torch.device(device)
        if self.device.type != "cuda":
            raise RuntimeError("codlad_amd runs on an MI355X only; no CPU path exists")
        self.lib = _lib.lib()
        if state_dict is None:
            self.weights = DenoiserWeights.empty(self.device, self_condition, out_dim, precision)
        else:
            self.weights = DenoiserWeights(state_dict, self.device, precision, block_exponents=block_exponents)
        self._mods_cache = {}
        self._mods_generation = self.weights.generation

    def new_structures(self, xyz_list, z_list, hoist_layer0=True):
        st = Structures(xyz_list, z_list, self.device)
        st.E_idx = torch.empty(st.n_snodes, KNN, dtype=torch.int32, device=self.device)
        st.h_E0 = torch.empty(st.n_snodes, 2, H // 4, KNN // 2, 4, dtype=torch.float32, device=self.device)
        if hoist_layer0:
            st.E1 = torch.empty(2, st.n_snodes, 2, H // 4, KNN // 2, 4, dtype=torch.float32, device=self.device)
        return st

    def compute_features(self, st):
        rc = self.lib.codlad_features_prepass(C.byref(self.weights.struct), _lib.ptr(st.xyz),
                                              _lib.ptr(st.snode_info), st.n_snodes, max(st.lens),
                                              _lib.ptr(st.E_idx), _lib.ptr(st.h_E0),
                                              _lib.stream_ptr(self.device))
        _lib.check(rc, "codlad_features_prepass")
        if st.E1 is not None:
            rc = self.lib.codlad_layer0_edge_terms(C.byref(self.weights.struct), _lib.ptr(st.snode_info),
                                                   st.n_snodes, _lib.ptr(st.h_E0), _lib.ptr(st.E1),
                                                   _lib.stream_ptr(self.device))
            _lib.check(rc, "codlad_layer0_edge_terms")
        st.features_tag = self.features_tag()
        return st

    @property
    def split_edge_state(self):
        return self.weights.precision != "f32"

    def features_tag(self):
        if self.weights.precision == "f32":
            return ("f32", self.weights.generation)
        ex = self.weights.exponents["enc0"]
        return ("split", self.weights.precision, ex["e1"], ex["e11"], self.weights.generation)

    def _fresh_features(self, st):
        if st.features_tag != self.features_tag():
            self.compute_features(st)

    def prepare_structures(self, xyz_list, z_list, hoist_layer0=True):
        return self.compute_features(self.new_structures(xyz_list, z_list, hoist_layer0))

    def make_job(self, structures, sample_struct):
        return Job(structures, sample_struct, self.device)

    def step_mods(self, t_values, refresh=False, as_float=False):
        fractional = as_float or any(float(t) != int(t) for t in t_values)
        key = tuple(float(t) for t in t_values) if fractional else tuple(int(t) for t in t_values)
        if self._mods_generation != self.weights.generation:
            self._mods_cache.clear()
            self._mods_generation = self.weights.generation
        if refresh or key not in self._mods_cache:
            mods = torch.empty(len(key), MODS, dtype=torch.float32, device=self.device)
            if fractional:
                tv = torch.tensor(key, dtype=torch.float32, device=self.device)
                rc = self.lib.codlad_step_mods_f(C.byref(self.weights.struct), _lib.ptr(tv), len(key),
                                                 _lib.ptr(mods), _lib.stream_ptr(self.device))
            else:
                tv = torch.tensor(key, dtype=torch.int64, device=self.device)
                rc = self.lib.codlad_step_mods(C.byref(self.weights.struct), _lib.ptr(tv), len(key),
                                               _lib.ptr(mods), _lib.stream_ptr(self.device))
            _lib.check(rc, "codlad_step_mods")
            if len(self._mods_cache) > 64:
                self._mods_cache.clear()
            self._mods_cache[key] = mods
        return self._mods_cache[key]

    @property
    def self_condition(self):
        return self.weights.self_condition

    def _run(self, name, desc, *args):
        rc = getattr(self.lib, name)(C.byref(self.weights.struct), C.byref(desc), *args, _lib.stream_ptr(self.device))
        _lib.check(rc, name)

    def _n_streams(self, job, streams):
        if streams is not None:
            return streams
        return 2 if job.n_nodes >= self.SPLIT_MIN_NODES and len(job.sample_struct) >= 2 else 1

    def check_status(self, job):
        _lib.check(self.lib.codlad_status_check(_lib.ptr(job.status), _lib.stream_ptr(self.device)),
                   "codlad_status_check")

    def forward(self, job, x, t_value, x_self_cond=None, check=True):
        _require_cuda(x, "x")
        x = x.contiguous().float()
        assert x.shape == (job.n_nodes, 3)
        if x_self_cond is not None:
            if not self.self_condition:
                raise ValueError("x_self_cond given to a model built without self_condition")
            _require_cuda(x_self_cond, "x_self_cond")
            x_self_cond = x_self_cond.contiguous().float()
            assert x_self_cond.shape == x.shape
        mods = self.step_mods([t_value])
        out = torch.empty(job.n_nodes, self.weights.out_dim, dtype=torch.float32, device=self.device)
        self._fresh_features(job.structures)
        self._run("codlad_denoiser_forward", job.desc(), _lib.ptr(x), _lib.ptr(x_self_cond), _lib.ptr(mods), _lib.ptr(out))
        if check:
            self.check_status(job)
        return out

    SPLIT_MIN_NODES = int(os.environ.get("CODLAD_SAMPLE_SPLIT_MIN_NODES", 8192))

    SAMPLE_KINDS = ("ddpm", "ddim", "ddim_reverse", "dpmpp")

    def sample(self, job, x_T, noise, tables, check=True, coef=None, streams=None, pin=None, kind="ddpm", x_start_out=None):
        if kind not in self.SAMPLE_KINDS:
            raise ValueError(f"kind must be one of {self.SAMPLE_KINDS}, got {kind!r}")
        reverse = kind == "ddim_reverse"
        noiseless = reverse or kind == "dpmpp"
        T = tables.num_timesteps
        _require_cuda(x_T, "x_T")
        if noiseless:
            if noise is not None:
                raise ValueError(("the reverse DDIM loop" if reverse else "the DPM-Solver++ loop") +
                                 " is deterministic: noise must be None")
        else:
            _require_cuda(noise, "noise")
            assert noise.shape == (T, job.n_nodes, 3)
        assert x_T.shape == (job.n_nodes, 3)
        if x_start_out is not None:
            _require_cuda(x_start_out, "x_start_out")
            assert x_start_out.shape == x_T.shape and x_start_out.dtype == torch.float32 and x_start_out.is_contiguous()
        if pin is not None:
            pin = self._pin_arrays(pin, job.n_nodes)
        streams = self._n_streams(job, streams)
        if streams > 1:
            parts = job.parts(streams)
            pins = None if pin is None else [(pin[0][i], pin[1][i]) for _p, i in parts]
            noises = [None if noiseless else noise[:, i] for _p, i in parts]
            starts = None if x_start_out is None else [torch.empty(p.n_nodes, 3, dtype=torch.float32, device=self.device)
                                                        for p, _i in parts]
            outs = self.sample_many([p for p, _i in parts], [x_T[i] for _p, i in parts], noises,
                                    tables, check=check, coef=coef, pins=pins, kind=kind, x_start_outs=starts)
            x0 = torch.empty(job.n_nodes, 3, dtype=torch.float32, device=self.device)
            for k, ((_p, i), o) in enumerate(zip(parts, outs)):
                x0[i] = o
                if starts is not None:
                    x_start_out[i] = starts[k]
            return x0
        if coef is None:
            coef = (tables.step_coefficients() if kind == "ddpm" else tables.dpm_solver_coefficients() if kind == "dpmpp"
                    else tables.ddim_coefficients(reverse=reverse))
        fixed_var = bool(int(coef[0, 7]) & 2)
        if self.weights.out_dim != (3 if fixed_var else 6):
            raise ValueError(f"the {kind.upper()} loop needs a model with 6 outputs (mean | variance logits), or 3 with a "
                             "fixed-variance sampler (create_diffusion(learn_sigma=False)); a flow-matching model is sampled "
                             "with codlad_amd.diffusion_and_flow.ode.odeint")
        x = x_T.detach().clone().contiguous().float()
        noise = None if noiseless else noise.contiguous().float()
        mods = self.step_mods(tables.timestep_map)
        mode = int(coef[0, 7])
        coef = torch.from_numpy(coef).to(self.device)
        self._fresh_features(job.structures)
        x_start = x_start_out if x_start_out is not None else (
            torch.empty_like(x) if self.self_condition or kind == "dpmpp" else None)
        loop = [_lib.ptr(t) for t in (x, x_start, noise, mods, coef)] + [T]
        pin_ptrs = [_lib.ptr(t) for t in (pin or (None, None))]
        if kind == "dpmpp":
            self._run("codlad_dpm_loop", job.desc(), *(_lib.ptr(t) for t in (x, x_start, mods, coef)), T, mode, *pin_ptrs)
        elif kind != "ddpm":
            self._run("codlad_ddim_loop", job.desc(), *loop, mode, int(reverse), *pin_ptrs)
        elif pin is None:
            self._run("codlad_sample_loop", job.desc(), *loop)
        else:
            self._run("codlad_sample_loop_pinned", job.desc(), *loop, *pin_ptrs)
        if check:
            self.check_status(job)
        return x

    def sample_many(self, jobs, x_Ts, noises, tables, check=True, coef=None, pins=None, kind="ddpm", x_start_outs=None):
        pins = [None] * len(jobs) if pins is None else list(pins)
        starts = [None] * len(jobs) if x_start_outs is None else list(x_start_outs)
        assert len(pins) == len(jobs) == len(starts)
        for job in jobs:
            self._fresh_features(job.structures)
        self.step_mods(tables.timestep_map)
        pins = [None if pin is None else self._pin_arrays(pin, job.n_nodes) for job, pin in zip(jobs, pins)]

        def one(job, x_T, noise, pin, start):
            return self.sample(job, x_T, noise, tables, check=False, coef=coef, streams=1, pin=pin, kind=kind,
                               x_start_out=start)

        outs = self._on_streams([lambda a=a: one(*a) for a in zip(jobs, x_Ts, noises, pins, starts)], len(jobs))
        if check:
            for job in jobs:
                self.check_status(job)
        return outs

    ODE_STAGES = {"euler": 1, "midpoint": 2, "rk4": 4}

    def _ode_fixed(self, job, y0, method, dts, mods):
        f32 = dict(dtype=torch.float32, device=self.device)
        y0 = y0.contiguous().float()
        traj = torch.empty(len(dts) + 1, job.n_nodes, 3, **f32)
        scratch = torch.empty(5, job.n_nodes, 3, **f32)
        dt = (C.c_float * len(dts))(*dts)
        self._run("codlad_ode_loop", job.desc(), _lib.ptr(y0), _lib.ptr(traj), _lib.ptr(mods), _lib.ODE_METHODS[method], dt,
                  len(dts), _lib.ptr(scratch))
        return traj

    def sample_ode(self, job, y0, ts, method="dopri5", rtol=1e-7, atol=1e-9, check=True, streams=None, max_steps=100000,
                   first_step=None):
        from .diffusion_and_flow import ode
        ts = [float(v) for v in ts]
        _require_cuda(y0, "y0")
        assert y0.shape == (job.n_nodes, 3)
        if self.weights.out_dim != 3:
            raise ValueError("sample_ode needs a flow-matching model (3 outputs: the velocity); a diffusion model is "
                             "sampled with Denoiser.sample")
        ode.check_grid(ts, method)
        self._fresh_features(job.structures)
        if method == "dopri5":
            return self._sample_dopri5(job, y0, ts, rtol, atol, check, max_steps, first_step)
        stages = self.ODE_STAGES[method]
        mods = self.step_mods(ode.stage_times(method, ts))
        dts = [b - a for a, b in zip(ts, ts[1:])]
        stats = {"n_eval": stages * len(dts), "n_accept": len(dts), "n_reject": 0}
        streams = self._n_streams(job, streams)
        if streams <= 1:
            traj = self._ode_fixed(job, y0, method, dts, mods)
            if check:
                self.check_status(job)
            return traj, stats
        parts = job.parts(streams)
        outs = self._on_streams([lambda p=p, i=i: self._ode_fixed(p, y0[i], method, dts, mods) for p, i in parts], streams)
        traj = torch.empty(len(ts), job.n_nodes, 3, dtype=torch.float32, device=self.device)
        for (_p, i), o in zip(parts, outs):
            traj[:, i] = o
        if check:
            self._check_all([p for p, _i in parts])
        return traj, stats

    def _sample_dopri5(self, job, y0, ts, rtol, atol, check, max_steps, first_step):
        from .diffusion_and_flow import ode
        f32 = dict(dtype=torch.float32, device=self.device)
        n = job.n_nodes

        def f(t, y, check=True):
            try:
                return self.forward(job, y, float(t), check=check)
            except RuntimeError as e:
                if "not finite" not in str(e):
                    raise
                raise RuntimeError(f"dopri5: the model output is not finite at t = {float(t)!r}") from e

        y = y0.detach().clone().contiguous().float()
        k = [f(ode._tt(ts[0], y), y, check or first_step is None)] + [torch.empty(n, 3, **f32) for _ in range(6)]
        h = ode._initial_step(f, ts[0], y, k[0], rtol, atol) if first_step is None else float(first_step)
        n_first = 2 if first_step is None else 1
        y1, xin = torch.empty(n, 3, **f32), torch.empty(n, 3, **f32)
        mods = torch.empty(6, MODS, **f32)
        norm = torch.empty(_lib.ODE_NORM_WORDS, dtype=torch.float64, device=self.device)
        host = _lib.OdeState()
        host.t, host.h = ts[0], h
        state = torch.frombuffer(bytearray(bytes(host)), dtype=torch.uint8).to(self.device)
        bufs = _lib.OdeDopri5Bufs()
        bufs.y, bufs.y1, bufs.xin, bufs.mods, bufs.state, bufs.norm = (
            _lib.ptr(t_) for t_ in (y, y1, xin, mods, state, norm))
        for j in range(7):
            bufs.k[j] = k[j].data_ptr()
        desc = job.desc()
        traj = torch.empty(len(ts), n, 3, **f32)
        traj[0] = y
        nxt, attempts = 1, 0
        while nxt < len(ts):
            attempts += 1
            if attempts > max_steps:
                raise RuntimeError("dopri5: max_steps exceeded")
            t_before = host.t
            self._run("codlad_ode_dopri5_attempt", desc, C.byref(bufs), C.c_double(ts[nxt]), C.c_float(rtol), C.c_float(atol))
            host = _lib.OdeState.from_buffer_copy(state.cpu().numpy().tobytes())
            if host.nonfinite or (check and host.status):
                job.status.zero_()
                raise RuntimeError(f"dopri5: the model output or the error norm is not finite in the step from t = "
                                   f"{t_before!r} (h = {host.hh!r}), attempt {attempts}: "
                                   f"{n_first + 6 * attempts} model evaluations so far")
            if host.accepted and host.t >= ts[nxt]:
                traj[nxt] = y
                nxt += 1
        return traj, {"n_eval": n_first + 6 * attempts, "n_accept": int(host.n_accept), "n_reject": int(host.n_reject)}

    @staticmethod
    def loss_table(tables, coef=None):
        coef = tables.loss_coefficients() if coef is None else coef
        coef = np.ascontiguousarray(coef, dtype=np.float32)
        if coef.shape != (tables.num_timesteps, tables.LOSS_COLUMNS):
            raise ValueError(f"coef must be a Tables.loss_coefficients table [{tables.num_timesteps}, "
                             f"{tables.LOSS_COLUMNS}], got {coef.shape}")
        return coef

    @staticmethod
    def sample_offsets(lens, device):
        off = np.concatenate([[0], np.cumsum(np.asarray(lens, dtype=np.int64))])
        if (np.diff(off) < 1).any() or off[-1] >= 2 ** 31 // 3:
            raise ValueError("every sample needs at least one node (and all of them fit 32-bit element indices)")
        return torch.from_numpy(off.astype(np.int32)).to(device)

    @staticmethod
    def _timesteps(t, n_samples, T, device):
        if isinstance(t, torch.Tensor):
            t = t.reshape(-1).tolist()
        ts = [int(t)] * n_samples if np.ndim(t) == 0 else [int(v) for v in t]
        if len(ts) != n_samples:
            raise ValueError(f"t must be one value or one per sample ({n_samples}), got {len(ts)}")
        if min(ts) < 0 or max(ts) >= T:
            raise ValueError(f"t must lie in [0, {T}), got {min(ts)} .. {max(ts)}")
        if len(set(ts)) == 1:
            return ts, ts[0], None
        return ts, None, torch.tensor(ts, dtype=torch.int32, device=device)

    @staticmethod
    def q_affine(kind, a, b, lens, t, coef):
        _require_cuda(a, "x_start")
        a = a.contiguous().float()
        if b is not None:
            _require_cuda(b, "noise" if kind == "q_sample" else "x_t")
            b = b.contiguous().float()
            if b.shape != a.shape:
                raise ValueError(f"{kind}: operands differ in shape, {tuple(a.shape)} and {tuple(b.shape)}")
        if a.numel() != 3 * int(sum(lens)):
            raise ValueError(f"{kind}: {a.numel()} values for {int(sum(lens))} nodes of 3 channels")
        T = coef.shape[0]
        _ts, shared, t_dev = Denoiser._timesteps(t, len(lens), T, a.device)
        off = Denoiser.sample_offsets(lens, a.device)
        coef_dev = torch.from_numpy(np.ascontiguousarray(coef, dtype=np.float32)).to(a.device)
        out, var, logvar = torch.empty_like(a), torch.empty_like(a), torch.empty_like(a)
        fn = {"q_sample": _lib.lib().codlad_q_sample, "q_posterior": _lib.lib().codlad_q_posterior}[kind]
        rc = fn(_lib.ptr(a), _lib.ptr(b), _lib.ptr(coef_dev), T, _lib.ptr(off), len(lens), _lib.ptr(t_dev),
                0 if shared is None else shared, _lib.ptr(out), _lib.ptr(var), _lib.ptr(logvar), _lib.stream_ptr(a.device))
        _lib.check(rc, f"codlad_{kind}")
        return out, var, logvar

    LOSS_KEYS = ("kl", "nll", "vb", "mse", "xstart_mse", "eps_mse")

    @staticmethod
    def _loss_outputs(n_samples, n_nodes, device, noise):
        res = {k: torch.empty(n_samples, dtype=torch.float32, device=device) for k in Denoiser.LOSS_KEYS
               if noise is not None or k not in ("mse", "eps_mse")}
        res["pred_xstart"] = torch.empty(n_nodes, 3, dtype=torch.float32, device=device)
        terms = _lib.LossTerms()
        for k, v in res.items():
            setattr(terms, k, v.data_ptr())
        return res, terms

    @staticmethod
    def vb_terms(model_out, x_start, x_t, noise, lens, t, coef):
        _require_cuda(x_start, "x_start")
        x_start = x_start.contiguous().float()
        n = int(sum(lens))
        coef = np.ascontiguousarray(coef, dtype=np.float32)
        _check_step_operands(x_start.reshape(n, 3), model_out, coef[0, :8], x_t=x_t, noise=noise)
        T = coef.shape[0]
        _ts, shared, t_dev = Denoiser._timesteps(t, len(lens), T, x_start.device)
        off = Denoiser.sample_offsets(lens, x_start.device)
        coef_dev = torch.from_numpy(coef).to(x_start.device)
        nz = None if noise is None else noise.contiguous().float()
        res, terms = Denoiser._loss_outputs(len(lens), n, x_start.device, nz)
        rc = _lib.lib().codlad_vb_terms(_lib.ptr(model_out.contiguous().float()), _lib.ptr(x_start),
                                        _lib.ptr(x_t.contiguous().float()), _lib.ptr(nz), _lib.ptr(coef_dev), T,
                                        _lib.ptr(off), len(lens), _lib.ptr(t_dev), 0 if shared is None else shared,
                                        C.byref(terms), _lib.stream_ptr(x_start.device))
        _lib.check(rc, "codlad_vb_terms")
        return res

    def _job_offsets(self, job):
        if getattr(job, "sample_off_dev", None) is None:
            job.sample_off_dev = self.sample_offsets(job.sample_lens, self.device)
        return job.sample_off_dev

    def q_sample(self, job, x_start, t, noise, tables, coef=None):
        assert x_start.shape == (job.n_nodes, 3) and noise.shape == (job.n_nodes, 3)
        return self.q_affine("q_sample", x_start, noise, job.sample_lens, t, self.loss_table(tables, coef))[0]

    def _t_group_job(self, job, members, start):
        cache = job.__dict__.setdefault("_t_groups", {})
        key = (start, tuple(members))
        if key not in cache:
            if len(cache) >= 64:
                cache.clear()
            cache[key] = job.sub_job(members, start)
        return cache[key]

    def _check_all(self, jobs):
        first = None
        for jb in jobs:
            try:
                self.check_status(jb)
            except RuntimeError as e:
                first = first or e
        if first is not None:
            raise first

    def _on_streams(self, tasks, n_streams=2):
        if not hasattr(self, "_streams"):
            self._streams = []
        n_streams = min(n_streams, len(tasks))
        while len(self._streams) < n_streams:
            self._streams.append(torch.cuda.Stream(device=self.device))
        cur = torch.cuda.current_stream(self.device)
        for st in self._streams[:n_streams]:
            st.wait_stream(cur)
        outs = []
        for k, task in enumerate(tasks):
            with torch.cuda.stream(self._streams[k % n_streams]):
                outs.append(task())
        for st in self._streams[:n_streams]:
            cur.wait_stream(st)
        return outs

    def _loss_forward(self, job, x_start, x_t, noise, t, coef_dev, T, mods, x_self_cond, want_model_out):
        res, terms = self._loss_outputs(len(job.sample_struct), job.n_nodes, self.device, noise)
        if want_model_out:
            res["model_out"] = torch.empty(job.n_nodes, self.weights.out_dim, dtype=torch.float32, device=self.device)
        self._run("codlad_loss_forward", job.desc(), _lib.ptr(x_start), _lib.ptr(x_t), _lib.ptr(noise), _lib.ptr(x_self_cond),
                  _lib.ptr(mods[t]), _lib.ptr(coef_dev), T, t, _lib.ptr(self._job_offsets(job)), len(job.sample_struct),
                  _lib.ptr(res.get("model_out")), C.byref(terms))
        return res

    def _check_loss_model(self, coef):
        fixed_var = bool(int(coef[0, 7]) & 2)
        if self.weights.out_dim != (3 if fixed_var else 6):
            raise ValueError("the loss needs a model with 6 outputs (mean | variance logits), or 3 with a fixed-variance "
                             "diffusion (create_diffusion(learn_sigma=False))")

    def loss_terms(self, job, x_start, t, noise, tables, coef=None, x_t=None, x_self_cond=None, check=True,
                   want_model_out=False):
        coef = self.loss_table(tables, coef)
        self._check_loss_model(coef)
        T, S = tables.num_timesteps, len(job.sample_struct)
        _require_cuda(x_start, "x_start")
        x_start = x_start.contiguous().float()
        assert x_start.shape == (job.n_nodes, 3)
        if noise is not None:
            _require_cuda(noise, "noise")
            noise = noise.contiguous().float()
            assert noise.shape == x_start.shape
        if x_t is None:
            if noise is None:
                raise ValueError("loss_terms needs noise or x_t")
            x_t = self.q_sample(job, x_start, t, noise, tables, coef)
        else:
            _require_cuda(x_t, "x_t")
            x_t = x_t.contiguous().float()
            assert x_t.shape == x_start.shape
        if x_self_cond is not None:
            if not self.self_condition:
                raise ValueError("x_self_cond given to a model built without self_condition")
            _require_cuda(x_self_cond, "x_self_cond")
            x_self_cond = x_self_cond.contiguous().float()
            assert x_self_cond.shape == x_start.shape
        ts, shared, _t_dev = self._timesteps(t, S, T, self.device)
        self._fresh_features(job.structures)
        mods = self.step_mods(tables.timestep_map)
        coef_dev = torch.from_numpy(coef).to(self.device)
        if shared is not None:
            res = self._loss_forward(job, x_start, x_t, noise, shared, coef_dev, T, mods, x_self_cond, want_model_out)
            if check:
                self.check_status(job)
            return res
        groups = [(tv, [m for m in range(S) if ts[m] == tv]) for tv in sorted(set(ts))]
        subs, start = [], 0
        for _tv, members in groups:
            subs.append(self._t_group_job(job, members, start))
            start += subs[-1][0].n_nodes
        pick = lambda a, i: None if a is None else a[i]
        tasks = [lambda tv=tv, sub=sub, i=i: self._loss_forward(sub, x_start[i], x_t[i], pick(noise, i), tv, coef_dev, T,
                                                                mods, pick(x_self_cond, i), want_model_out)
                 for (tv, _m), (sub, i) in zip(groups, subs)]
        outs = self._on_streams(tasks)
        res = {}
        for (_tv, members), (sub, i), o in zip(groups, subs, outs):
            m = torch.tensor(members, dtype=torch.int64, device=self.device)
            for k, v in o.items():
                per_node = k in ("pred_xstart", "model_out")
                if k not in res:
                    res[k] = torch.empty((job.n_nodes if per_node else S,) + tuple(v.shape[1:]), dtype=v.dtype,
                                         device=self.device)
                res[k][i if per_node else m] = v
        if check:
            self._check_all([sub for sub, _i in subs])
        return res

    def bpd(self, job, x_start, noise, tables, streams=None, coef=None, check=True):
        coef = self.loss_table(tables, coef)
        self._check_loss_model(coef)
        T, S = tables.num_timesteps, len(job.sample_struct)
        _require_cuda(x_start, "x_start")
        _require_cuda(noise, "noise")
        assert x_start.shape == (job.n_nodes, 3) and noise.shape == (T, job.n_nodes, 3)
        streams = self._n_streams(job, streams)
        self._fresh_features(job.structures)
        mods = self.step_mods(tables.timestep_map)
        coef_dev = torch.from_numpy(coef).to(self.device)

        def run(jb, x0, eps):
            x0, eps = x0.contiguous().float(), eps.contiguous().float()
            n = len(jb.sample_struct)
            f32 = dict(dtype=torch.float32, device=self.device)
            out = {k: torch.empty(T, n, **f32) for k in ("vb", "mse", "xstart_mse")}
            out.update({k: torch.empty(n, **f32) for k in ("prior_bpd", "total_bpd")})
            x_t = torch.empty_like(x0)
            self._run("codlad_bpd_loop", jb.desc(), _lib.ptr(x0), _lib.ptr(eps), _lib.ptr(x_t), _lib.ptr(mods), _lib.ptr(coef_dev),
                      T, _lib.ptr(self._job_offsets(jb)), n,
                      *(_lib.ptr(out[k]) for k in ("vb", "mse", "xstart_mse", "prior_bpd", "total_bpd")))
            return out

        if streams <= 1:
            res = run(job, x_start, noise)
            if check:
                self.check_status(job)
            return res
        parts = job.parts(streams)
        outs = self._on_streams([lambda p=p, i=i: run(p, x_start[i], noise[:, i]) for p, i in parts], streams)
        f32 = dict(dtype=torch.float32, device=self.device)
        res = {k: torch.empty(T, S, **f32) for k in ("vb", "mse", "xstart_mse")}
        res.update({k: torch.empty(S, **f32) for k in ("prior_bpd", "total_bpd")})
        for p, o in enumerate(outs):
            for k, v in o.items():
                res[k][..., p::streams] = v
        if check:
            self._check_all([p for p, _i in parts])
        return res

    FM_LOSS_KEYS = ("l2", "l1", "huber", "smooth_l1", "log_cosh")

    @staticmethod
    def _fm_kind(kind, sigma):
        if kind not in _lib.FM_KINDS:
            raise ValueError(f"kind must be one of {tuple(_lib.FM_KINDS)}, got {kind!r}")
        if isinstance(sigma, bool) or not isinstance(sigma, (int, float)):
            raise TypeError(f"sigma must be a number, got {type(sigma).__name__}")
        if not sigma >= 0:
            raise ValueError(f"sigma must be >= 0, got {sigma}")
        return _lib.FM_KINDS[kind], float(sigma)

    @staticmethod
    def _fm_times(t, n_samples, device):
        if isinstance(t, torch.Tensor):
            t = t.reshape(-1).tolist()
        ts = [t] * n_samples if np.ndim(t) == 0 else list(t)
        ts = [float(np.float32(v)) for v in ts]
        if len(ts) != n_samples:
            raise ValueError(f"t must be one value or one per sample ({n_samples}), got {len(ts)}")
        if not all(0.0 <= v <= 1.0 for v in ts):
            raise ValueError(f"t must lie in [0, 1], got {min(ts)} .. {max(ts)}")
        if len(set(ts)) == 1:
            return ts, ts[0], None
        return ts, None, torch.tensor(ts, dtype=torch.float32, device=device)

    @staticmethod
    def _fm_operand(a, name, like):
        if a is None:
            return None
        _require_cuda(a, name)
        a = a.contiguous().float()
        if like is not None and a.shape != like.shape:
            raise ValueError(f"{name} {tuple(a.shape)} does not match x1 {tuple(like.shape)}")
        return a

    @staticmethod
    def fm_path(kind, sigma, x0, x1, eps, lens, t):
        kind_id, sigma = Denoiser._fm_kind(kind, sigma)
        x1 = Denoiser._fm_operand(x1, "x1", None)
        n = int(sum(lens))
        if x1.numel() != 3 * n:
            raise ValueError(f"fm_path: {x1.numel()} values for {n} nodes of 3 channels")
        x0, eps = Denoiser._fm_operand(x0, "x0", x1), Denoiser._fm_operand(eps, "eps", x1)
        if kind != "target" and x0 is None:
            raise ValueError(f"fm_path: the {kind} matcher needs x0")
        if eps is None and (kind == "target" or sigma != 0):
            raise ValueError("fm_path: eps may be None only for icfm / vp at sigma = 0")
        _ts, shared, t_dev = Denoiser._fm_times(t, len(lens), x1.device)
        off = Denoiser.sample_offsets(lens, x1.device)
        xt, ut = torch.empty_like(x1), torch.empty_like(x1)
        rc = _lib.lib().codlad_fm_path(_lib.ptr(x0), _lib.ptr(x1), _lib.ptr(eps), _lib.ptr(off), len(lens), _lib.ptr(t_dev),
                                       0.0 if shared is None else shared, kind_id, sigma, _lib.ptr(xt), _lib.ptr(ut),
                                       _lib.stream_ptr(x1.device))
        _lib.check(rc, "codlad_fm_path")
        return xt, ut

    @staticmethod
    def _fm_outputs(shape, device):
        res = {k: torch.empty(*shape, dtype=torch.float32, device=device) for k in Denoiser.FM_LOSS_KEYS}
        out = _lib.FmLossOut()
        for k, v in res.items():
            setattr(out, k, v.data_ptr())
        return res, out

    @staticmethod
    def fm_terms(model_out, ut, lens):
        _require_cuda(model_out, "model_out")
        _require_cuda(ut, "ut")
        model_out, ut = model_out.contiguous().float(), ut.contiguous().float()
        n = int(sum(lens))
        if tuple(model_out.shape) != (n, 3) or tuple(ut.shape) != (n, 3):
            raise ValueError(f"fm_terms: model_out and ut must be [{n}, 3], got {tuple(model_out.shape)} and {tuple(ut.shape)}")
        off = Denoiser.sample_offsets(lens, ut.device)
        res, out = Denoiser._fm_outputs((len(lens),), ut.device)
        rc = _lib.lib().codlad_fm_terms(_lib.ptr(model_out), _lib.ptr(ut), _lib.ptr(off), len(lens), C.byref(out),
                                        _lib.stream_ptr(ut.device))
        _lib.check(rc, "codlad_fm_terms")
        return res

    def _check_fm_model(self):
        if self.weights.out_dim != 3:
            raise ValueError("the flow-matching losses need a flow-matching model (3 outputs: the velocity); a diffusion "
                             "model is scored with Denoiser.loss_terms / Denoiser.bpd")

    def _fm_loss_forward(self, job, xt, ut, mods_t, want_model_out):
        res, out = self._fm_outputs((len(job.sample_struct),), self.device)
        if want_model_out:
            res["model_out"] = torch.empty(job.n_nodes, 3, dtype=torch.float32, device=self.device)
        self._run("codlad_fm_loss_forward", job.desc(), _lib.ptr(xt), _lib.ptr(ut), _lib.ptr(mods_t),
                  _lib.ptr(self._job_offsets(job)), len(job.sample_struct), _lib.ptr(res.get("model_out")), C.byref(out))
        return res

    def fm_loss_terms(self, job, x1, t, kind="icfm", sigma=0.0, x0=None, eps=None, check=True, want_model_out=False):
        self._check_fm_model()
        S = len(job.sample_struct)
        xt, ut = self.fm_path(kind, sigma, x0, x1, eps, job.sample_lens, t)
        ts, shared, _t_dev = self._fm_times(t, S, self.device)
        self._fresh_features(job.structures)
        distinct = sorted(set(ts))
        mods = self.step_mods(distinct, as_float=True)
        if shared is not None:
            res = self._fm_loss_forward(job, xt, ut, mods[0], want_model_out)
            res.update(xt=xt, ut=ut)
            if check:
                self.check_status(job)
            return res
        groups = [(tv, [m for m in range(S) if ts[m] == tv]) for tv in distinct]
        subs, start = [], 0
        for _tv, members in groups:
            subs.append(self._t_group_job(job, members, start))
            start += subs[-1][0].n_nodes
        tasks = [lambda g=g, sub=sub, i=i: self._fm_loss_forward(sub, xt[i], ut[i], mods[g], want_model_out)
                 for g, (sub, i) in enumerate(subs)]
        outs = self._on_streams(tasks)
        res = {"xt": xt, "ut": ut}
        for (_tv, members), (sub, i), o in zip(groups, subs, outs):
            m = torch.tensor(members, dtype=torch.int64, device=self.device)
            for k, v in o.items():
                per_node = k == "model_out"
                if k not in res:
                    res[k] = torch.empty((job.n_nodes if per_node else S,) + tuple(v.shape[1:]), dtype=v.dtype,
                                         device=self.device)
                res[k][i if per_node else m] = v
        if check:
            self._check_all([sub for sub, _i in subs])
        return res

    def fm_loss_sweep(self, job, x1, ts, kind="icfm", sigma=0.0, x0=None, eps=None, streams=None, check=True):
        self._check_fm_model()
        kind_id, sigma = self._fm_kind(kind, sigma)
        ts = [float(np.float32(v)) for v in ts]
        K, S = len(ts), len(job.sample_struct)
        if K < 1 or not all(0.0 <= v <= 1.0 for v in ts):
            raise ValueError("fm_loss_sweep: ts must be a non-empty list of times in [0, 1]")
        x1 = self._fm_operand(x1, "x1", None)
        assert x1.shape == (job.n_nodes, 3)
        x0 = self._fm_operand(x0, "x0", x1)
        if kind != "target" and x0 is None:
            raise ValueError(f"fm_loss_sweep: the {kind} matcher needs x0")
        if eps is None:
            if kind == "target" or sigma != 0:
                raise ValueError("fm_loss_sweep: eps may be None only for icfm / vp at sigma = 0")
        else:
            _require_cuda(eps, "eps")
            if tuple(eps.shape) != (K, job.n_nodes, 3):
                raise ValueError(f"eps must be [K, n_nodes, 3] = {(K, job.n_nodes, 3)}, got {tuple(eps.shape)}")
        streams = self._n_streams(job, streams)
        self._fresh_features(job.structures)
        mods = self.step_mods(ts, as_float=True)
        t_host = (C.c_float * K)(*ts)

        def run(jb, a0, a1, ae):
            a1 = a1.contiguous().float()
            a0 = None if a0 is None else a0.contiguous().float()
            ae = None if ae is None else ae.contiguous().float()
            n = len(jb.sample_struct)
            res, out = self._fm_outputs((K, n), self.device)
            xt, ut = torch.empty_like(a1), torch.empty_like(a1)
            self._run("codlad_fm_loss_loop", jb.desc(), _lib.ptr(a0), _lib.ptr(a1), _lib.ptr(ae), kind_id, sigma, t_host, K,
                      _lib.ptr(mods), _lib.ptr(self._job_offsets(jb)), n, _lib.ptr(xt), _lib.ptr(ut), C.byref(out))
            return res

        pick = lambda a, i: None if a is None else a[i]
        if streams <= 1:
            res = run(job, x0, x1, eps)
            if check:
                self.check_status(job)
            return res
        parts = job.parts(streams)
        outs = self._on_streams([lambda p=p, i=i: run(p, pick(x0, i), x1[i], None if eps is None else eps[:, i])
                                 for p, i in parts], streams)
        res = {k: torch.empty(K, S, dtype=torch.float32, device=self.device) for k in self.FM_LOSS_KEYS}
        for p, o in enumerate(outs):
            for k, v in o.items():
                res[k][..., p::streams] = v
        if check:
            self._check_all([p for p, _i in parts])
        return res

    @staticmethod
    def _pin_arrays(pin, n_nodes):
        x0, mask = pin
        _require_cuda(x0, "pin x0")
        _require_cuda(mask, "pin mask")
        if tuple(x0.shape) != (n_nodes, 3) or tuple(mask.shape) != (n_nodes,):
            raise ValueError(f"pin: x0 must be [{n_nodes}, 3] and mask [{n_nodes}], got {tuple(x0.shape)} and {tuple(mask.shape)}")
        if not x0.is_floating_point():
            raise TypeError(f"pin: x0 must be a floating-point tensor, got {x0.dtype}")
        if mask.dtype not in (torch.bool, torch.uint8, torch.int32):
            raise TypeError(f"pin: mask must be bool, uint8 or int32, got {mask.dtype}")
        x0 = x0.contiguous().float()
        if mask.dtype != torch.uint8:
            mask = mask != 0
        return x0, mask.to(torch.uint8).contiguous()

    def ddpm_update(self, x, model_out, noise, tables, i, return_x_start=False):
        _require_cuda(x, "x")
        n = x.numel() // 3
        x = x.contiguous().float()
        out = torch.empty_like(x)
        x_start = torch.empty_like(x) if return_x_start else None
        coef = np.ascontiguousarray(tables.step_coefficients()[i])
        rc = self.lib.codlad_ddpm_update(_lib.ptr(x), _lib.ptr(model_out.contiguous().float()),
                                         _lib.ptr(noise.contiguous().float()),
                                         coef.ctypes.data_as(C.c_void_p), n, _lib.ptr(out), _lib.ptr(x_start),
                                         _lib.stream_ptr(self.device))
        _lib.check(rc, "codlad_ddpm_update")
        return (out, x_start) if return_x_start else out

    @staticmethod
    def ddpm_pred_xstart(x, model_out, coef):
        _require_cuda(x, "x")
        x = x.contiguous().float()
        out = torch.empty_like(x)
        coef = np.ascontiguousarray(coef, dtype=np.float32)
        _check_step_operands(x, model_out, coef)
        rc = _lib.lib().codlad_ddpm_pred_xstart(_lib.ptr(x), _lib.ptr(model_out.contiguous().float()),
                                                coef.ctypes.data_as(C.c_void_p), x.numel() // 3, _lib.ptr(out),
                                                _lib.stream_ptr(x.device))
        _lib.check(rc, "codlad_ddpm_pred_xstart")
        return out

    @staticmethod
    def ddpm_posterior_step(x, pred_xstart, model_out, noise, coef, grad=None, fixed_variance=0.0):
        _require_cuda(x, "x")
        x = x.contiguous().float()
        out = torch.empty_like(x)
        x_start = torch.empty_like(x)
        coef = np.ascontiguousarray(coef, dtype=np.float32)
        g = None if grad is None else grad.contiguous().float()
        _check_step_operands(x, model_out, coef, pred_xstart=pred_xstart, noise=noise, grad=g)
        rc = _lib.lib().codlad_ddpm_posterior_step(_lib.ptr(x), _lib.ptr(pred_xstart.contiguous().float()),
                                                   _lib.ptr(model_out.contiguous().float()),
                                                   _lib.ptr(noise.contiguous().float()), _lib.ptr(g),
                                                   coef.ctypes.data_as(C.c_void_p), C.c_float(fixed_variance),
                                                   x.numel() // 3, _lib.ptr(out), _lib.ptr(x_start),
                                                   _lib.stream_ptr(x.device))
        _lib.check(rc, "codlad_ddpm_posterior_step")
        return out, x_start

    @staticmethod
    def ddim_step(x, pred_xstart, noise, coef, grad=None, reverse=False):
        _require_cuda(x, "x")
        x = x.contiguous().float()
        out = torch.empty_like(x)
        x_start = torch.empty_like(x)
        coef = np.ascontiguousarray(coef, dtype=np.float32)
        if reverse != (noise is None):
            raise ValueError("the forward DDIM step takes noise, the reverse one none")
        nz = None if noise is None else noise.contiguous().float()
        g = None if grad is None else grad.contiguous().float()
        _check_step_operands(x, None, coef, pred_xstart=pred_xstart, noise=nz, grad=g)
        rc = _lib.lib().codlad_ddim_step(_lib.ptr(x), _lib.ptr(pred_xstart.contiguous().float()), _lib.ptr(nz),
                                         _lib.ptr(g), coef.ctypes.data_as(C.c_void_p), int(bool(reverse)),
                                         x.numel() // 3, _lib.ptr(out), _lib.ptr(x_start), _lib.stream_ptr(x.device))
        _lib.check(rc, "codlad_ddim_step")
        return out, x_start

    @staticmethod
    def dpm_step(x, pred_xstart, prev_xstart, coef, grad=None):
        _require_cuda(x, "x")
        x = x.contiguous().float()
        out = torch.empty_like(x)
        x_start = torch.empty_like(x)
        coef = np.ascontiguousarray(coef, dtype=np.float32)
        g = None if grad is None else grad.contiguous().float()
        prev = None if prev_xstart is None else prev_xstart.contiguous().float()
        _check_step_operands(x, None, coef, pred_xstart=pred_xstart, prev_xstart=prev, grad=g)
        if (coef[4] != 0) != (prev is not None):
            raise ValueError("prev_xstart is given exactly when the row's C (column 4) is not 0")
        rc = _lib.lib().codlad_dpm_step(_lib.ptr(x), _lib.ptr(pred_xstart.contiguous().float()), _lib.ptr(prev), _lib.ptr(g),
                                        coef.ctypes.data_as(C.c_void_p), x.numel() // 3, _lib.ptr(out), _lib.ptr(x_start),
                                        _lib.stream_ptr(x.device))
        _lib.check(rc, "codlad_dpm_step")
        return out, x_start


def _check_step_operands(x, model_out, coef, **same_as_x):
    n = x.numel() // 3
    if x.numel() != 3 * n or n == 0:
        raise ValueError(f"x must hold [n, 3] latents, got {tuple(x.shape)}")
    if coef.shape != (8,):
        raise ValueError(f"coef must be one [8] row of the step table, got {coef.shape}")
    width = 3 if int(coef[7]) & 2 else 6
    for name, t in dict(model_out=model_out, **same_as_x).items():
        if t is None:
            continue
        _require_cuda(t, name)
        want = n * (width if name == "model_out" else 3)
        if t.numel() != want:
            raise ValueError(f"{name} holds {t.numel()} values, the step needs {want} ({n} nodes)")


class Decoder:

    def __init__(self, state_dict, device, mean3=None, std3=None, angle=False, n_codes=4096):
        self.device = torch.device(device)
        if self.device.type != "cuda":
            raise RuntimeError("codlad_amd runs on an MI355X only; no CPU path exists")
        self.lib = _lib.lib()
        if state_dict is None:
            self.weights = DecoderWeights.empty(self.device, angle, n_codes)
        else:
            self.weights = DecoderWeights(state_dict, self.device, mean3, std3)
        f = dict(dtype=torch.float32, device=self.device)
        self._unit = (torch.zeros(3, **f), torch.ones(3, **f))

    @property
    def mean(self):
        return self.weights.mean

    @property
    def std(self):
        return self.weights.std

    def vq(self, x, normalised=True):
        _require_cuda(x, "latent")
        xs = x.contiguous().float()
        n = xs.numel() // 3
        idx = torch.empty(n, dtype=torch.int64, device=self.device)
        zq = torch.empty_like(xs)
        lat = torch.empty_like(xs)
        mean, std = (self.mean, self.std) if normalised else self._unit
        cb = self.weights.codebook
        rc = self.lib.codlad_vq_lookup(_lib.ptr(xs), n, _lib.ptr(mean), _lib.ptr(std), _lib.ptr(cb),
                                       cb.shape[0], _lib.ptr(idx), _lib.ptr(zq), _lib.ptr(lat),
                                       _lib.stream_ptr(self.device))
        _lib.check(rc, "codlad_vq_lookup")
        return idx, zq, lat

    @staticmethod
    def csr_from_pairs(pairs, n_nodes):
        gtr_ij = bool((pairs[:, 0] > pairs[:, 1]).any())
        gtr_ji = bool((pairs[:, 1] > pairs[:, 0]).any())
        directed = pairs if (gtr_ij and gtr_ji) else torch.cat([pairs, pairs.flip(1)], dim=0)
        recv = directed[:, 0]
        order = torch.sort(recv, stable=True).indices
        src = directed[order, 1].to(torch.int32).contiguous()
        counts = torch.bincount(recv, minlength=n_nodes)
        ptr = torch.zeros(n_nodes + 1, dtype=torch.int32, device=pairs.device)
        ptr[1:] = torch.cumsum(counts, 0).to(torch.int32)
        return ptr, src

    def build_csr(self, cg_xyz, sample_lens, cutoff=21.0, sample_range=None, max_edges=None):
        xyz = cg_xyz.to(self.device).contiguous().float()
        M = xyz.shape[0]
        rng = self.sample_ranges(sample_lens) if sample_range is None else sample_range
        assert rng.shape == (M, 2)
        deg = torch.empty(M, dtype=torch.int32, device=self.device)
        st = _lib.stream_ptr(self.device)
        _lib.check(self.lib.codlad_cg_graph(_lib.ptr(xyz), _lib.ptr(rng), M, C.c_float(cutoff), _lib.ptr(deg),
                                            None, None, st), "codlad_cg_graph(count)")
        ptr = torch.zeros(M + 1, dtype=torch.int32, device=self.device)
        ptr[1:] = torch.cumsum(deg, 0).to(torch.int32)
        n_src = max_edges if max_edges is not None else int(ptr[-1])
        src = torch.empty(max(n_src, 1), dtype=torch.int32, device=self.device)
        _lib.check(self.lib.codlad_cg_graph(_lib.ptr(xyz), _lib.ptr(rng), M, C.c_float(cutoff), None,
                                            _lib.ptr(ptr), _lib.ptr(src), st), "codlad_cg_graph(fill)")
        return ptr, src[:n_src]

    def sample_ranges(self, sample_lens):
        M = int(sum(sample_lens))
        rng = np.empty((M, 2), dtype=np.int32)
        o = 0
        for L in sample_lens:
            rng[o:o + L, 0] = o
            rng[o:o + L, 1] = L
            o += L
        return torch.from_numpy(rng).to(self.device)

    SCRATCH_WIDTH = 200

    @staticmethod
    def read_taps(scratch):
        M = scratch.shape[0]
        assert scratch.shape == (M, Decoder.SCRATCH_WIDTH) and scratch.is_contiguous()
        planes = scratch.reshape(-1).reshape(5, 40 * M)
        return {"S": planes[0].reshape(40, M).t().contiguous(), "V": planes[1].reshape(M, 40).clone(),
                "phi2": planes[2].reshape(M, 40).clone(), "phi3": planes[3].reshape(M, 40).clone()}

    def ic_decode(self, z_q, cg_z, cg_xyz, pairs=None, csr=None, scratch=None):
        _require_cuda(z_q, "z_q")
        M = z_q.shape[0]
        cg_z = cg_z.to(self.device, torch.int32).contiguous()
        lo, hi = int(cg_z.min()), int(cg_z.max())
        if lo < 0 or hi >= 25:
            raise ValueError(f"cg_z (residue types {lo}..{hi}) outside the decoder's 25-row embedding tables")
        ptr, src = csr if csr is not None else self.csr_from_pairs(pairs.to(self.device), M)
        assert ptr.numel() == M + 1 and ptr.dtype == torch.int32 and src.dtype == torch.int32
        if src.numel() == 0:
            src = torch.zeros(1, dtype=torch.int32, device=self.device)
        if scratch is None:
            scratch = torch.empty(M, self.SCRATCH_WIDTH, dtype=torch.float32, device=self.device)
        else:
            _require_cuda(scratch, "scratch")
            if scratch.shape != (M, self.SCRATCH_WIDTH) or scratch.dtype != torch.float32 or not scratch.is_contiguous():
                raise ValueError(f"scratch must be a contiguous float32 [{M}, {self.SCRATCH_WIDTH}] tensor, got "
                                 f"{scratch.dtype} {tuple(scratch.shape)}")
        ic = torch.empty(M, 13, 3, dtype=torch.float32, device=self.device)
        rc = self.lib.codlad_ic_decode(C.byref(self.weights.struct), _lib.ptr(z_q.contiguous().float()),
                                       _lib.ptr(cg_z),
                                       _lib.ptr(cg_xyz.to(self.device).contiguous().float()),
                                       _lib.ptr(ptr), _lib.ptr(src), M, _lib.ptr(scratch), _lib.ptr(ic),
                                       _lib.stream_ptr(self.device))
        _lib.check(rc, "codlad_ic_decode")
        return ic

    def ic_to_xyz(self, ca_full, ic, info):
        _require_cuda(ic, "ic")
        B, L = ic.shape[0], ic.shape[1]
        orders, slot_to_out, n_atoms = info_tables(info, L, self.device)
        out = torch.empty(B, n_atoms, 3, dtype=torch.float32, device=self.device)
        rc = self.lib.codlad_ic_to_xyz(_lib.ptr(ca_full.to(self.device).contiguous().float()),
                                       _lib.ptr(ic.contiguous().float()), _lib.ptr(orders),
                                       _lib.ptr(slot_to_out), B, L, n_atoms, _lib.ptr(out),
                                       _lib.stream_ptr(self.device))
        _lib.check(rc, "codlad_ic_to_xyz")
        return out


    def ic_to_xyz_groups(self, groups, reuse=False):
        key = tuple((ca.data_ptr(), ic.data_ptr(), id(info[0]), tuple(ic.shape)) for ca, ic, info in groups)
        cache = getattr(self, "_xyz_groups", None) if reuse else None
        if cache is None or cache[0] != key:
            desc = (_lib.XyzGroup * len(groups))()
            outs, keep, row = [], [], 0
            for g, (ca, ic, info) in enumerate(groups):
                _require_cuda(ic, "ic")
                B, L = ic.shape[0], ic.shape[1]
                orders, s2o, n_atoms = info_tables(info, L, self.device)
                ca_d, ic_d = ca.to(self.device).contiguous().float(), ic.contiguous().float()
                assert ic_d.data_ptr() == ic.data_ptr() and ca_d.shape == (B, L + 2, 3)
                out = torch.empty(B, n_atoms, 3, dtype=torch.float32, device=self.device)
                d = desc[g]
                d.ca_full, d.ic, d.orders, d.slot_to_out, d.xyz_out = (ca_d.data_ptr(), ic_d.data_ptr(), orders.data_ptr(),
                                                                       s2o.data_ptr(), out.data_ptr())
                d.B, d.L, d.n_atoms, d.first_row = B, L, n_atoms, row
                row += B * L
                outs.append(out)
                keep += [ca_d, ic_d, orders, s2o]
            table = torch.frombuffer(bytearray(bytes(desc)), dtype=torch.uint8).to(self.device)
            cache = (key, table, outs, keep, row)
            if reuse:
                self._xyz_groups = cache
        _key, table, outs, _keep, rows = cache
        rc = self.lib.codlad_ic_to_xyz_groups(_lib.ptr(table), len(groups), rows, _lib.stream_ptr(self.device))
        _lib.check(rc, "codlad_ic_to_xyz_groups")
        return outs


_INFO_CACHE = {}


def info_tables(info, L, device):
    permute, atom_idx, orders = info
    key = (id(permute), id(atom_idx), id(orders), L, str(device))
    if key not in _INFO_CACHE:
        assert orders.shape == (10, L, 3), "atom_orders does not match the batch's residue count"
        n_atoms = int(permute.numel())
        slot = atom_idx.cpu()[permute.cpu()]
        assert int(slot.max()) < 14 * L and torch.unique(slot).numel() == n_atoms
        s2o = torch.full((14 * L,), -1, dtype=torch.int32)
        s2o[slot] = torch.arange(n_atoms, dtype=torch.int32)
        o32 = orders.to(torch.int32).contiguous()
        assert int(o32.min()) >= 0
        for i in range(10):
            assert int(o32[i].max()) < 4 + i, "atom_orders references an atom that is not placed yet"
        if len(_INFO_CACHE) > 256:
            _INFO_CACHE.clear()
        _INFO_CACHE[key] = (o32.to(device), s2o.to(device), n_atoms, info)
    o, s, n, _keepalive = _INFO_CACHE[key]
    return o, s, n
```

include/codlad_hip.h:

```cpp
#ifndef CODLAD_HIP_H
#define CODLAD_HIP_H

#include <stdint.h>

#ifdef __cplusplus
extern "C" {
#endif

#define CODLAD_ABI_VERSION 19
#define CODLAD_H 128
#define CODLAD_KNN 64
#define CODLAD_MODS_PER_STEP 6016
#define CODLAD_PACKED_BLOCK 16384

int codlad_abi_version(void);
const char *codlad_last_error(void);
void codlad_struct_sizes(int *out7);

void codlad_pack_block_host(const float *src_host, int ld, float scale, float *dst_host);

typedef struct {
    const float *W1e, *W2, *W3;
    const float *W11e, *W12, *W13;
    const float *W1a, *W1c;
    const float *W11a, *W11c;
    const float *Win[4], *Wout[4];
    const float *b1, *b2, *b3, *b11, *b12, *b13, *b_in , *b_out;
} codlad_enc_layer;

typedef struct {
    const float *W1e;
    const float *W2, *W3;
    const float *W1a;
    const float *W1v;
    const float *TS;
    const float *Win[4], *Wout[4];
    const float *b1, *b2, *b3, *b_in, *b_out;
} codlad_dec_layer;

typedef struct {
    const void *W1e, *W2, *W3, *W11e, *W12, *W13, *W1a, *W1c, *W11a, *W11c;
    const void *Win[4], *Wout[4];
    const float *b1, *b2, *b3, *b11, *b12, *b13, *b_in, *b_out;
    int e1, e2, e3, e11, e12, e13, e_in, e_out;
} codlad_enc_layer_h;

typedef struct {
    const void *W1e, *W2, *W3, *W1a, *W1v;
    const void *Win[4], *Wout[4];
    const float *TS;
    const float *b1, *b2, *b3, *b_in, *b_out;
    int e1, e2, e3, e_in, e_out;
} codlad_dec_layer_h;

typedef struct {
    const float *freqs;
    const float *rbf_mu;
    const float *t_w0, *t_b0;
    const float *t_w2, *t_b2;
    const float *ada_w[7], *ada_b[7];
    const float *x_in_w, *x_in_b;
    const float *pos_w, *pos_b;
    const float *edge_wT;
    const float *norm_w, *norm_b;
    const float *We_wT, *We_b;
    const float *out_w, *out_b;
    codlad_enc_layer enc[3];
    codlad_dec_layer dec[3];
    int precision;
    codlad_enc_layer_h enc_h[3];
    codlad_dec_layer_h dec_h[3];
    int self_condition;
    int out_dim;
} codlad_denoiser_weights;

int codlad_features_prepass(const codlad_denoiser_weights *w, const float *cg_xyz,
                            const int32_t *snode_info, int n_snodes, int max_len,
                            int32_t *E_idx, float *h_E0, void *stream);

int codlad_step_mods(const codlad_denoiser_weights *w, const int64_t *t_values, int n_t,
                     float *mods, void *stream);

int codlad_step_mods_f(const codlad_denoiser_weights *w, const float *t_values, int n_t, float *mods, void *stream);

int codlad_ode_combine(const float *y, const float *const *k_host, const float *coef_host, int n_k, float h,
                       size_t n, float *out, void *stream);

#define CODLAD_ODE_NORM_BLOCKS 256
#define CODLAD_ODE_NORM_WORDS (1 + CODLAD_ODE_NORM_BLOCKS)
int codlad_ode_error_norm(const float *err, const float *y, const float *y1, size_t n, float rtol, float atol,
                          double *out_double, void *stream);

typedef struct {
    float *hV;
    float *hVenc;
    float *S;
    float *PQ;
    float *hE;
    int32_t *status;
    const int32_t *tile_list;
    int32_t n_tiles;
    const int32_t *xcd_bounds;
} codlad_workspace;

typedef struct {
    const int32_t *node_info; int n_nodes;
    const int32_t *E_idx; const float *h_E0;
    const float *E1;
    int n_snodes;
    const codlad_workspace *ws;
} codlad_job;

int codlad_edge_plan_host(const int32_t *K_host, int n_nodes, int n_workgroups, int waves_per_workgroup, int pair,
                          int32_t *bounds_host, int64_t *stats_host);

#define CODLAD_STATUS_NONFINITE 1
#define CODLAD_E_NONFINITE (-3)

int codlad_status_check(int32_t *status, void *stream);

int codlad_layer0_edge_terms(const codlad_denoiser_weights *w, const int32_t *snode_info,
                             int n_snodes, const float *h_E0, float *E1, void *stream);

int codlad_denoiser_forward(const codlad_denoiser_weights *w, const codlad_job *job, const float *x,
                            const float *x_self_cond, const float *mods_t, float *out, void *stream);

int codlad_ddpm_update(const float *x, const float *model_out, const float *noise,
                       const float *coef_host, int n_nodes, float *x_out, float *x_start_out ,
                       void *stream);

int codlad_ddpm_pred_xstart(const float *x, const float *model_out, const float *coef_host, int n_nodes,
                            float *pred_xstart, void *stream);

int codlad_ddpm_posterior_step(const float *x, const float *pred_xstart, const float *model_out, const float *noise,
                               const float *grad , const float *coef_host, float fixed_variance,
                               int n_nodes, float *x_out, float *x_start_out , void *stream);

int codlad_sample_loop(const codlad_denoiser_weights *w, const codlad_job *job, float *x, float *x_start,
                       const float *noise, const float *mods, const float *coef, int T, void *stream);

int codlad_sample_loop_pinned(const codlad_denoiser_weights *w, const codlad_job *job, float *x, float *x_start,
                              const float *noise, const float *mods, const float *coef, int T, const float *pin_x0,
                              const uint8_t *pin_mask, void *stream);

int codlad_ddim_loop(const codlad_denoiser_weights *w, const codlad_job *job, float *x, float *x_start,
                     const float *noise , const float *mods, const float *coef, int T, int mode,
                     int reverse, const float *pin_x0 , const uint8_t *pin_mask ,
                     void *stream);

int codlad_ddim_step(const float *x, const float *pred_xstart, const float *noise ,
                     const float *grad , const float *coef_host, int reverse, int n_nodes, float *x_out,
                     float *x_start_out , void *stream);

int codlad_dpm_loop(const codlad_denoiser_weights *w, const codlad_job *job, float *x, float *x_start, const float *mods,
                    const float *coef, int T, int mode, const float *pin_x0 ,
                    const uint8_t *pin_mask , void *stream);

int codlad_dpm_step(const float *x, const float *pred_xstart, const float *prev_xstart ,
                    const float *grad , const float *coef_host, int n_nodes, float *x_out,
                    float *x_start_out , void *stream);

typedef struct {
    float *kl, *nll, *vb, *mse, *xstart_mse, *eps_mse;
    float *pred_xstart;
} codlad_loss_terms;

int codlad_q_sample(const float *x_start, const float *noise , const float *coef, int T,
                    const int32_t *sample_off, int n_samples, const int32_t *t_of_sample , int t, float *x_t,
                    float *variance , float *log_variance , void *stream);

int codlad_q_posterior(const float *x_start, const float *x_t, const float *coef, int T, const int32_t *sample_off,
                       int n_samples, const int32_t *t_of_sample , int t, float *mean,
                       float *variance , float *log_variance , void *stream);

int codlad_vb_terms(const float *model_out, const float *x_start, const float *x_t, const float *noise ,
                    const float *coef, int T, const int32_t *sample_off, int n_samples,
                    const int32_t *t_of_sample , int t, const codlad_loss_terms *terms, void *stream);

int codlad_prior_bpd(const float *x_start, const float *coef, int T, const int32_t *sample_off, int n_samples,
                     float *prior_bpd, void *stream);

int codlad_loss_forward(const codlad_denoiser_weights *w, const codlad_job *job, const float *x_start, const float *x_t,
                        const float *noise , const float *x_self_cond ,
                        const float *mods_t, const float *coef, int T, int t, const int32_t *sample_off, int n_samples,
                        float *model_out , const codlad_loss_terms *terms, void *stream);

int codlad_bpd_loop(const codlad_denoiser_weights *w, const codlad_job *job, const float *x_start, const float *noise,
                    float *x_t, const float *mods, const float *coef, int T, const int32_t *sample_off, int n_samples,
                    float *vb, float *mse, float *xstart_mse, float *prior_bpd, float *total_bpd, void *stream);

#define CODLAD_FM_ICFM 0
#define CODLAD_FM_TARGET 1
#define CODLAD_FM_VP 2
#define CODLAD_FM_TARGET_FLOW 3
int codlad_fm_path(const float *x0 , const float *x1, const float *eps ,
                   const int32_t *sample_off, int n_samples, const float *t_of_sample , float t, int kind,
                   double sigma, float *xt, float *ut, void *stream);

typedef struct {
    float *l2, *l1, *huber, *smooth_l1, *log_cosh;
} codlad_fm_loss_out;

int codlad_fm_terms(const float *model_out, const float *ut, const int32_t *sample_off, int n_samples,
                    const codlad_fm_loss_out *terms, void *stream);

int codlad_fm_loss_forward(const codlad_denoiser_weights *w, const codlad_job *job, const float *xt, const float *ut,
                           const float *mods_t, const int32_t *sample_off, int n_samples,
                           float *model_out , const codlad_fm_loss_out *terms, void *stream);

int codlad_fm_loss_loop(const codlad_denoiser_weights *w, const codlad_job *job, const float *x0 ,
                        const float *x1, const float *eps , int kind, double sigma, const float *t_host,
                        int K, const float *mods, const int32_t *sample_off, int n_samples, float *xt, float *ut,
                        const codlad_fm_loss_out *tables, void *stream);

#define CODLAD_ODE_EULER 0
#define CODLAD_ODE_MIDPOINT 1
#define CODLAD_ODE_RK4 2
int codlad_ode_loop(const codlad_denoiser_weights *w, const codlad_job *job, const float *y, float *traj,
                    const float *mods, int method, const float *dt_host, int n_intervals, float *scratch, void *stream);

typedef struct {
    double t, h, t_end;
    double ratio;
    double hh;
    int32_t accepted;
    int32_t n_accept, n_reject;
    int32_t clipped;
    int32_t nonfinite;
    int32_t status;
    float hh_f;
    float tf[6];
    float pad_;
} codlad_ode_state;

typedef struct {
    float *y, *y1, *xin;
    float *k[7];
    float *mods;
    codlad_ode_state *state;
    double *norm;
} codlad_ode_dopri5_bufs;

int codlad_ode_dopri5_attempt(const codlad_denoiser_weights *w, const codlad_job *job,
                              const codlad_ode_dopri5_bufs *bufs, double t_end, float rtol, float atol, void *stream);

int codlad_vq_lookup(const float *x, int n, const float *mean3, const float *std3,
                     const float *codebook, int n_codes, int64_t *idx, float *z_q,
                     float *latent_out , void *stream);

typedef struct {
    int angle;
    const float *map_out_w, *map_out_b;
    const float *res_embed;
    const float *inv0_w[4], *inv0_b[4], *inv1_w[4], *inv1_b[4];
    const float *dist_w[4], *dist_b[4];
    const float *dense1_w[4], *dense1_b[4], *dense3_w[4], *dense3_b[4];
    const float *bb_dist, *sc_dist;
    const float *bb_ang1_w, *bb_ang1_b, *bb_ang3_w, *bb_ang3_b;
    const float *sc_angle_emb;
    const float *sc_ang1_w, *sc_ang1_b, *sc_ang3_w, *sc_ang3_b;
    const float *bb_tor1_w, *bb_tor1_b, *bb_tor3_w, *bb_tor3_b;
    const float *tor1_w[4], *tor1_b[4], *tor3_w[4], *tor3_b[4];
    const float *fin1_w, *fin1_b, *fin3_w, *fin3_b;
} codlad_decoder_weights;

int codlad_ic_decode(const codlad_decoder_weights *w, const float *z_q, const int32_t *cg_z,
                     const float *cg_xyz, const int32_t *csr_ptr, const int32_t *csr_src,
                     int M, float *scratch, float *ic_out, void *stream);

int codlad_cg_graph(const float *cg_xyz, const int32_t *sample_range, int M, float cutoff,
                    int32_t *degree, const int32_t *csr_ptr, int32_t *csr_src, void *stream);

typedef struct {
    const int32_t *ptr, *snd;
    int32_t n_recv;
    const float *xyz_recv, *xyz_snd;
    const float *typ_recv, *typ_snd;
    float r_sign, smear_stop;
    const float *emb0_w, *emb0_b, *emb3_w, *emb3_b;
    int32_t emb_in;
    const float *h_recv; int32_t d_recv;
    const float *h_snd; int32_t d_snd;
    int32_t attr_recv_first;
    const float *fc0_w, *fc0_b, *fc3_w, *fc3_b;
    int32_t depth;
    float *out;
    int32_t accumulate, group;
    const void *packed;
} codlad_tp_conv_args;
int codlad_tp_conv(const codlad_tp_conv_args *args, void *stream);
int codlad_tp_conv_args_size(void);
int codlad_tp_conv_image_bytes(int depth);
int codlad_tp_conv_pack(const codlad_tp_conv_args *args, void *image, void *stream);

int codlad_receiver_csr(const int64_t *pairs, int n_pairs, int n_nodes, int mode, int32_t *ptr, int32_t *snd, int32_t *work,
                        void *stream);

int codlad_mlp_rows(const float *x, int n, int in_dim, const float *w1, const float *b1, int hidden, const float *w2,
                    const float *b2, int out_dim, int act, int mode, float *y, void *stream);
int codlad_bead_mean(const float *h_atom, const float *h_cg, const int32_t *bead_ptr, const int32_t *bead_atoms,
                     int n_cg, float *node, void *stream);
int codlad_embed_rows(const float *table, const int32_t *idx, int n, int width, float *out, void *stream);

int codlad_ic_to_xyz(const float *ca_full, const float *ic, const int32_t *orders,
                     const int32_t *slot_to_out, int B, int L, int n_atoms, float *xyz_out,
                     void *stream);

typedef struct {
    const float *ca_full, *ic;
    const int32_t *orders, *slot_to_out;
    float *xyz_out;
    int32_t B, L, n_atoms, first_row;
} codlad_xyz_group;
int codlad_ic_to_xyz_groups(const codlad_xyz_group *groups, int n_groups, int total_rows, void *stream);

int codlad_xyz_to_ic(const float *xyz, int n_frames, int n_atoms, const int32_t *quads, int n_quads, float *ic_out,
                     void *stream);

#define CODLAD_OPT_NODEQ_MAX_TILES 0
#define CODLAD_OPT_EDGE_TILE_MAX_NODES 1
#define CODLAD_OPT_NODE_QUAD_MAX_TILES 2
#define CODLAD_OPT_DEC_EDGE_VARIANT 3
#define CODLAD_OPT_TP_CONV_VARIANT 4
#define CODLAD_OPT_EDGE_UPD_VARIANT 5
#define CODLAD_OPT_EDGE_CUS 6
#define CODLAD_OPT_EDGE_WIDE_MAX_TILES 7
#define CODLAD_OPT_EDGE_PAIR 8
#define CODLAD_N_OPTIONS 9
int codlad_set_option(int option, int value);

int codlad_probe_edge_launches(int enable);
int codlad_probe_read(int kind, double *total_ms);

#define CODLAD_DISPATCH_EDGE 0
#define CODLAD_DISPATCH_NODE_IN 1
#define CODLAD_DISPATCH_NODE_UPD 2
#define CODLAD_DISPATCH_CHUNKED_IN 3
#define CODLAD_DISPATCH_CHUNKED_UPD 4
#define CODLAD_DISPATCH_GRID_EDGE_MSG 5
#define CODLAD_DISPATCH_GRID_EDGE_UPD 6
#define CODLAD_DISPATCH_GRID_NODE_IN 7
#define CODLAD_DISPATCH_GRID_NODE_UPD 8
#define CODLAD_DISPATCH_WORDS 9
#define CODLAD_EDGE_KIND_F32 0
#define CODLAD_EDGE_KIND_WIDE 1
#define CODLAD_EDGE_KIND_TILE 2
#define CODLAD_EDGE_KIND_NODE 3
#define CODLAD_EDGE_KIND_NODE_UPD1 4
#define CODLAD_NODE_KIND_F32 0
#define CODLAD_NODE_KIND_W 1
#define CODLAD_NODE_KIND_Q 2
#define CODLAD_NODE_KIND_H4 3
#define CODLAD_NODE_KIND_H8 4
int codlad_dispatch_read(int32_t *out, int n);

int codlad_bench_edge_launch(const codlad_denoiser_weights *w, const int32_t *node_info,
                             int n_nodes, const int32_t *E_idx, const float *h_E0,
                             const float *mods_t, const codlad_workspace *ws, int which,
                             int layer, void *stream);

typedef struct {
    const float *xyz_recon, *xyz;
    int64_t n_atoms;
    const int64_t *edge_list;
    int64_t n_edges;
    const int64_t *clash_list;
    int64_t n_clash;
    const int64_t *bb_NO_list;
    int64_t n_bb;
    const int64_t *interaction_list;
    int64_t n_inter;
    const int64_t *pi_pi_list;
    int64_t n_pipi;
    const float *ic, *ic_recon, *ic_mask;
    int64_t n_ic;
} codlad_metric_inputs;

int codlad_metrics_scratch_bytes(void);
int codlad_eval_metrics(const codlad_metric_inputs *in, float *out8, void *scratch, void *stream);

int codlad_bond_graph_counts(const float *xyz, const float *xyz_recon, const float *radius, const int32_t *heavy,
                             const int32_t *struct_ptr, int n_struct, int max_atoms, float scale, int32_t *counts,
                             void *stream);

int codlad_ens_moments(const float *x, int n_conf, int n_atoms, const int32_t *sel, int n_sel, double *mom, void *stream);
int codlad_ens_pair_msd(const float *A, const double *momA, int nA, const float *B, const double *momB, int nB, int n_atoms,
                        const int32_t *sel, int n_sel, const int32_t *pairs, int n_pairs, int squared, double *out,
                        double *Rt, void *stream);
int codlad_ens_apply(const float *x, const double *Rt, int n_conf, int n_atoms, float *out, void *stream);
int codlad_ens_pairwise(const float *x, const double *mom, int G, int F, int n_atoms, const int32_t *sel, int n_sel,
                        int squared, double *out, void *stream);

#define CODLAD_GEOM_BOND_FLAG (1 << 30)
int codlad_geometry_check(const float *xyz, int n_struct, int n_atoms, const float *radius, const int32_t *excl_ptr,
                          const int32_t *excl, const int32_t *bonds, int n_bonds, float scale, float clash_dist,
                          float near_dist, int32_t *counts, float *min_dist, void *stream);

#define CODLAD_STEREO_COLUMNS 9
#define CODLAD_STEREO_COUNTS 6
#define CODLAD_STEREO_KIND_PRO 1
#define CODLAD_STEREO_INVERTED_CA 1
#define CODLAD_STEREO_INVERTED_SIDE 2
#define CODLAD_STEREO_CIS 4
#define CODLAD_STEREO_TWISTED 8
#define CODLAD_STEREO_UNDEFINED 16
int codlad_stereo_check(const float *xyz, int n_struct, int n_atoms, const int32_t *sites, const uint8_t *res_kind,
                        int n_res, float *values, uint8_t *flags, int32_t *counts, void *stream);

long long codlad_relax_scratch_bytes(int n_struct, int n_atoms, int n_pairs, int n_quads, int n_iter);
int codlad_relax_energy(const float *xyz, const float *xyz0, int n_struct, int n_atoms, const float *radius,
                        const uint8_t *fixed, const int32_t *excl_ptr, const int32_t *excl, const int32_t *pair_ptr,
                        const int32_t *pair_j, int n_pairs, const int32_t *quads, int n_quads, const int32_t *quad_ptr,
                        const int32_t *quad_ref, int n_refs, float k_r, float k_t, float k_c, float contact_scale,
                        double *energy, float *grad, float *gmax, void *scratch, void *stream);
int codlad_relax(const float *xyz, int n_struct, int n_atoms, const float *radius, const uint8_t *fixed,
                 const int32_t *excl_ptr, const int32_t *excl, const int32_t *pair_ptr, const int32_t *pair_j, int n_pairs,
                 const int32_t *quads, int n_quads, const int32_t *quad_ptr, const int32_t *quad_ref, int n_refs, float k_r,
                 float k_t, float k_c, float contact_scale, float h0, float h_max, int n_iter, float *xyz_out,
                 double *trace_energy, double *trace_trial_energy, float *trace_step, uint8_t *trace_accepted,
                 float *trace_gmax, uint8_t *converged, void *scratch, void *stream);

#define CODLAD_SASA_MAX_POINTS 1024
int codlad_sasa(const float *xyz, int n_struct, int n_atoms, const float *radius, const float *unit_area, const float *dirs,
                int n_points, const int32_t *res_ptr, int n_res, int32_t *exposed, float *atom_area, float *res_area,
                double *total, uint8_t *finite, void *stream);
int codlad_contact_counts(const float *xyz, int n_struct, int n_atoms, const int32_t *sel, int n_sel, float cut2,
                          int32_t *counts, void *stream);

#define CODLAD_DSSP_MAX_RES 4096
#define CODLAD_DSSP_KIND_PRO 1
#define CODLAD_DSSP_KIND_CHAIN_START 2
#define CODLAD_DSSP_GEOM_LINK 1
#define CODLAD_DSSP_GEOM_BEND 2
int codlad_dssp_hbonds(const float *xyz, int n_struct, int n_atoms, const int32_t *bb, const uint8_t *res_kind, int n_res,
                       uint64_t *acc, uint64_t *don, uint8_t *geom, float *kappa, float *e_best, int32_t *partner,
                       uint8_t *finite, void *stream);
#define CODLAD_DSSP_LOOP 0
#define CODLAD_DSSP_H 1
#define CODLAD_DSSP_B 2
#define CODLAD_DSSP_E 3
#define CODLAD_DSSP_G 4
#define CODLAD_DSSP_I 5
#define CODLAD_DSSP_T 6
#define CODLAD_DSSP_S 7
#define CODLAD_DSSP_UNDEFINED 255
int codlad_dssp_assign(const uint64_t *acc, const uint64_t *don, const uint8_t *geom, const uint8_t *finite, int n_struct,
                       int n_res, uint8_t *ss, int32_t *bridge, int32_t *counts, void *stream);

int codlad_selftest_gemm128(const float *W_packed, const float *bias, const float *X, int n_rows,
                            int act, float *Y, void *stream);

int codlad_selftest_gemm128_h(const void *W_split, const float *bias, const float *X, int n_rows,
                              int act_in, int terms, float *Y, void *stream);

#define CODLAD_SAXS_INV_PI 0x1.45f306p-2f
#define CODLAD_SAXS_P1 0x1.92p+1f
#define CODLAD_SAXS_P2 0x1.fb4p-11f
#define CODLAD_SAXS_P3 0x1.4442d2p-23f
#define CODLAD_SAXS_S3 -0x1.555556p-3f
#define CODLAD_SAXS_S5 0x1.11111p-7f
#define CODLAD_SAXS_S7 -0x1.a019ccp-13f
#define CODLAD_SAXS_S9 0x1.71c83ap-19f
#define CODLAD_SAXS_S11 -0x1.a5a3eap-26f
#define CODLAD_SAXS_C6 0x1.555556p-3f
#define CODLAD_SAXS_C20 0x1.99999ap-5f
#define CODLAD_SAXS_X_MAX 0x1.9p+14f
#define CODLAD_SAXS_X_SMALL 0x1p-3f
#define CODLAD_SAXS_SIN_ULPS 5
#define CODLAD_SAXS_MAX_Q 512
#define CODLAD_SAXS_MAX_TYPES 32
#define CODLAD_SAXS_Q_CHUNK 16
int codlad_saxs_debye(const float *xyz, int n_struct, int n_atoms, const int32_t *type, int n_types, const float *ff,
                      const float *q, int n_q, double *partial, double *I, double *mean, uint8_t *finite, void *stream);

#define CODLAD_SAXS_HYD_PARTIALS 6
#ifndef CODLAD_SAXS_HYD_Q_CHUNK
#define CODLAD_SAXS_HYD_Q_CHUNK 8
#endif
int codlad_saxs_partials(const float *xyz, int n_struct, int n_atoms, const int32_t *type, int n_types, const float *ff_t,
                         const float *ff_d, const float *weight, const float *q, int n_q, double *partial, double *P,
                         double *mean_P, uint8_t *finite, void *stream);
#define CODLAD_SAXS_HYD_MAX_GRID 4096
int codlad_saxs_hydration_fit(const double *P, int n_batch, int n_q, const double *f_w, const double *G, int n_c1,
                              const double *c2, int n_c2, const double *I_exp, const double *sigma, double *I_grid,
                              double *scale, double *chi2, int32_t *best, double *I_best, void *stream);

#ifdef __cplusplus
}
#endif
#endif
```

Before: 703.0 structures/s.

## Add dynamic atomic tail work-stealing to edge message and update kernels

Each wave's static strided node walk now stops a few stride-rows before the end of its XCD chunk. The remaining tail nodes are handed out dynamically through a per-chunk atomic ticket counter, which is meant to even out load imbalance at the end of the edge kernels. Per-tail XCD bounds are precomputed on the host, and counters are zeroed with a memset before each forward. Pairing of nodes is disabled across the tail boundary. The cost is extra atomics, an extra memset per forward, and some added control flow.

```diff
diff --git a/codlad_amd/_lib.py b/codlad_amd/_lib.py
--- a/codlad_amd/_lib.py
+++ b/codlad_amd/_lib.py
@@ -50,7 +50,7 @@
 
 class JobDesc(C.Structure):
     _fields_ = [("node_info", P), ("n_nodes", C.c_int), ("E_idx", P), ("h_E0", P), ("E1", P), ("n_snodes", C.c_int),
-                ("ws", C.POINTER(Workspace))]
+                ("ws", C.POINTER(Workspace)), ("edge_tail", P)]
 
 
 class DecoderWeights(C.Structure):
@@ -161,7 +161,11 @@
     "codlad_denoiser_forward": (C.c_int, _JOB + [P, P, P, P, P]),
     "codlad_status_check": (C.c_int, [P, P]),
     "codlad_set_option": (C.c_int, [C.c_int, C.c_int]),
+    "codlad_set_edge_tail": (C.c_int, [C.c_int]),
+    "codlad_edge_tail": (C.c_int, []),
     "codlad_edge_plan_host": (C.c_int, [P, C.c_int, C.c_int, C.c_int, C.c_int, P, P]),
+    "codlad_edge_plan_tail_host": (C.c_int, [P, C.c_int, C.c_int, C.c_int, C.c_int, C.c_int, P, P]),
+    "codlad_edge_span_host": (C.c_int, [C.c_int, C.c_int, C.c_int, C.c_int, C.c_int, P, C.c_int, P]),
     "codlad_ddpm_update": (C.c_int, [P, P, P, P, C.c_int, P, P, P]),
     "codlad_ddpm_pred_xstart": (C.c_int, [P, P, P, C.c_int, P, P]),
     "codlad_ddpm_posterior_step": (C.c_int, [P, P, P, P, P, P, C.c_float, C.c_int, P, P, P]),
@@ -193,6 +197,7 @@
     "codlad_receiver_csr": (C.c_int, [P, C.c_int, C.c_int, C.c_int, P, P, P, P]),
     "codlad_bench_edge_launch": (C.c_int, [C.POINTER(DenoiserWeights), P, C.c_int, P, P, P,
                                            C.POINTER(Workspace), C.c_int, C.c_int, P]),
+    "codlad_bench_edge_launch_job": (C.c_int, _JOB + [P, C.c_int, C.c_int, P]),
     "codlad_tp_conv": (C.c_int, [C.POINTER(TpConvArgs), P]),
     "codlad_tp_conv_args_size": (C.c_int, []),
     "codlad_mlp_rows": (C.c_int, [P, C.c_int, C.c_int, P, P, C.c_int, P, P, C.c_int, C.c_int, C.c_int, P, P]),
@@ -230,15 +235,27 @@
 OPT_NODEQ_MAX_TILES, OPT_EDGE_TILE_MAX_NODES, OPT_DEC_EDGE_VARIANT, OPT_TP_CONV_VARIANT, OPT_EDGE_UPD_VARIANT, OPT_EDGE_CUS, OPT_EDGE_WIDE_MAX_TILES, OPT_NODE_QUAD_MAX_TILES = 0, 1, 3, 4, 5, 6, 7, 2
 OPT_EDGE_PAIR = 8
 EDGE_GRID = (256, 8)
-
-
-def edge_plan(K, pair=True, grid=EDGE_GRID):
+EDGE_TAIL_MAX, EDGE_TAIL_SLOTS = 3, 9
+EDGE_TAIL_BOUNDS_WORDS = 16 * (EDGE_TAIL_MAX + 1)
+EDGE_TAIL_WORDS = EDGE_TAIL_BOUNDS_WORDS + 8 * EDGE_TAIL_SLOTS
+
+
+def edge_plan(K, pair=True, grid=EDGE_GRID, tail=0):
     import numpy as np
     K = np.ascontiguousarray(K, dtype=np.int32)
     bounds, stats = np.zeros(9, dtype=np.int32), np.zeros(20, dtype=np.int64)
-    check(lib().codlad_edge_plan_host(K.ctypes.data_as(P), K.shape[0], grid[0], grid[1], int(bool(pair)),
-                                      bounds.ctypes.data_as(P), stats.ctypes.data_as(P)), "codlad_edge_plan_host")
+    check(lib().codlad_edge_plan_tail_host(K.ctypes.data_as(P), K.shape[0], grid[0], grid[1], int(bool(pair)), int(tail),
+                                           bounds.ctypes.data_as(P), stats.ctypes.data_as(P)), "codlad_edge_plan_tail_host")
     return bounds, stats
+
+
+def edge_span(n_nodes, grid, workgroup, wave, bounds=None, tail=0):
+    import numpy as np
+    out = np.zeros(5, dtype=np.int32)
+    b = None if bounds is None else np.ascontiguousarray(bounds, dtype=np.int32)
+    check(lib().codlad_edge_span_host(int(n_nodes), grid[0], grid[1], workgroup, wave, None if b is None else b.ctypes.data_as(P),
+                                      int(tail), out.ctypes.data_as(P)), "codlad_edge_span_host")
+    return tuple(int(v) for v in out)
 
 
 DISPATCH_WORDS = ("edge", "node_in", "node_upd", "chunked_in", "chunked_upd", "grid_edge_msg", "grid_edge_upd", "grid_node_in",
@@ -263,6 +280,10 @@
     check(lib().codlad_set_option(option, value), "codlad_set_option")
 
 
+def set_edge_tail(value):
+    check(lib().codlad_set_edge_tail(value), "codlad_set_edge_tail")
+
+
 def exported_symbols():
     return list(_SIGS)
 
diff --git a/codlad_amd/csrc/denoiser_forward.hip b/codlad_amd/csrc/denoiser_forward.hip
--- a/codlad_amd/csrc/denoiser_forward.hip
+++ b/codlad_amd/csrc/denoiser_forward.hip
@@ -130,10 +130,20 @@
     int n_nodes;
     const codlad_workspace *ws;
     bool split;
+    int tail;
+    mutable int tail_slot;
+    int32_t *tail_buf;
     float *PQ(int k) const { return ws->PQ + (size_t)k * n_nodes * HD; }
 };
 static Job make_job(const codlad_denoiser_weights *w, const codlad_job *d) {
-    return {w, reinterpret_cast<const int4 *>(d->node_info), d->E_idx, d->n_nodes, d->ws, w->precision != 0};
+    const int tail = d->edge_tail && w->precision != 0 ? edge_tail_value() : 0;
+    return {w, reinterpret_cast<const int4 *>(d->node_info), d->E_idx, d->n_nodes, d->ws, w->precision != 0, tail, 0, d->edge_tail};
+}
+static void clear_tail_counters(const Job &j, hipStream_t st) {
+    j.tail_slot = 0;
+    if (j.tail)
+        (void)hipMemsetAsync(j.tail_buf + CODLAD_EDGE_TAIL_BOUNDS_WORDS, 0,
+                             sizeof(int32_t) * 8 * CODLAD_EDGE_TAIL_SLOTS, st);
 }
 
 static EdgeArgs edge_args(const Job &j, const float *hE_in, bool in_by_src) {
@@ -142,6 +152,11 @@
     ea.hE_in = hE_in; ea.in_by_src = in_by_src;
     ea.pair = option_value(CODLAD_OPT_EDGE_PAIR) != 0;
     ea.xcd_bounds = ea.pair ? j.ws->xcd_bounds : nullptr;
+    if (j.tail && j.tail_slot < CODLAD_EDGE_TAIL_SLOTS) {
+        ea.tail = j.tail_buf + CODLAD_EDGE_TAIL_BOUNDS_WORDS + 8 * j.tail_slot++;
+        ea.tail_nodes = j.tail;
+        if (ea.pair) ea.xcd_bounds = j.tail_buf + 16 * j.tail;
+    }
     return ea;
 }
 template <class Layer, class LayerH>
@@ -203,7 +218,7 @@
 
 static void enqueue_forward(const codlad_denoiser_weights *w, const codlad_job *job, const float *x,
                             const float *x_self_cond, const float *mods_t, hipStream_t st) {
-    const Job j = make_job(w, job);
+    Job j = make_job(w, job);
     const codlad_workspace *ws = job->ws;
     const int n_nodes = job->n_nodes;
     const float *h_E0 = job->h_E0, *E1 = job->E1;
@@ -212,6 +227,8 @@
                           (ws->n_tiles <= 8 * num_cu() || ws->n_tiles <= option_value(CODLAD_OPT_EDGE_WIDE_MAX_TILES)) &&
                           n_nodes <= option_value(CODLAD_OPT_EDGE_TILE_MAX_NODES);
     const int2 *tile_list = tilewise ? reinterpret_cast<const int2 *>(ws->tile_list) : nullptr;
+    if (tilewise) j.tail = 0;
+    clear_tail_counters(j, st);
 
     {
         NodeArgs na = {};
@@ -604,20 +621,27 @@
     return codlad_check_launch("codlad_ode_dopri5_attempt");
 }
 
+extern "C" int codlad_bench_edge_launch_job(const codlad_denoiser_weights *w, const codlad_job *job, const float *mods_t,
+                                            int which, int layer, void *stream) {
+    REQUIRE_OK(job_defect(w, job));
+    CODLAD_REQUIRE(mods_t, "null pointer");
+    CODLAD_REQUIRE((which == 0 || which == 1) && (layer == 0 || layer == 1), "bad arguments");
+    const Job j = make_job(w, job);
+    const codlad_workspace *ws = job->ws;
+    const codlad_enc_layer &L = w->enc[layer];
+    const codlad_enc_layer_h &Lh = w->enc_h[layer];
+    clear_tail_counters(j, (hipStream_t)stream);
+    const float *hE_in = layer == 0 ? job->h_E0 : ws->hE;
+    EdgeArgs ea = which == 0 ? msg_args(j, L, Lh, hE_in, layer == 0) : upd_args(j, L, Lh, hE_in, layer == 0, mods_t);
+    ea.S = ws->S;
+    launch_edge(which == 1, ea, w->precision, (hipStream_t)stream, nullptr, ws->n_tiles);
+    return codlad_check_launch("codlad_bench_edge_launch");
+}
+
 extern "C" int codlad_bench_edge_launch(const codlad_denoiser_weights *w, const int32_t *node_info,
                                         int n_nodes, const int32_t *E_idx, const float *h_E0,
                                         const float *mods_t, const codlad_workspace *ws, int which,
                                         int layer, void *stream) {
-    const codlad_job desc = {node_info, n_nodes, E_idx, h_E0, nullptr, 0, ws}, *job = &desc;
-    REQUIRE_OK(job_defect(w, job));
-    CODLAD_REQUIRE(mods_t, "null pointer");
-    CODLAD_REQUIRE((which == 0 || which == 1) && (layer == 0 || layer == 1), "bad arguments");
-    const Job j = make_job(w, job);
-    const codlad_enc_layer &L = w->enc[layer];
-    const codlad_enc_layer_h &Lh = w->enc_h[layer];
-    const float *hE_in = layer == 0 ? h_E0 : ws->hE;
-    EdgeArgs ea = which == 0 ? msg_args(j, L, Lh, hE_in, layer == 0) : upd_args(j, L, Lh, hE_in, layer == 0, mods_t);
-    ea.S = ws->S;
-    launch_edge(which == 1, ea, w->precision, (hipStream_t)stream, nullptr, ws->n_tiles);
-    return codlad_check_launch("codlad_bench_edge_launch");
-}
+    const codlad_job desc = {node_info, n_nodes, E_idx, h_E0, nullptr, 0, ws, nullptr};
+    return codlad_bench_edge_launch_job(w, &desc, mods_t, which, layer, stream);
+}
diff --git a/codlad_amd/csrc/edge_args.h b/codlad_amd/csrc/edge_args.h
--- a/codlad_amd/csrc/edge_args.h
+++ b/codlad_amd/csrc/edge_args.h
@@ -22,6 +22,8 @@
     float res_scale, ln_eps;
     const int32_t *xcd_bounds;
     int pair;
+    int32_t *tail;
+    int tail_nodes;
 };
 
 struct EdgeTileArgs : EdgeArgs {
@@ -48,9 +50,10 @@
 
 struct NodeSpan {
     int first, end, stride;
+    int lo;
 };
 __host__ __device__ inline NodeSpan node_span_of(int n_nodes, int nwaves, int wave, int nb, int b, const int32_t *bounds) {
-    if (nb % 8) return {b * nwaves + wave, n_nodes, nb * nwaves};
+    if (nb % 8) return {b * nwaves + wave, n_nodes, nb * nwaves, 0};
     int lo, hi;
     if (bounds) {
         lo = bounds[b % 8];
@@ -62,10 +65,27 @@
     }
     if (lo > n_nodes) lo = n_nodes;
     if (hi > n_nodes) hi = n_nodes;
-    return {lo + (b / 8) * nwaves + wave, hi, (nb / 8) * nwaves};
+    return {lo + (b / 8) * nwaves + wave, hi, (nb / 8) * nwaves, lo};
 }
 DEV NodeSpan wave_node_span(int n_nodes, int nwaves, int wave, const int32_t *bounds = nullptr) {
     return node_span_of(n_nodes, nwaves, wave, gridDim.x, blockIdx.x, bounds);
+}
+
+__host__ __device__ inline int edge_tail_lo(const NodeSpan &s, int tail_nodes) {
+    const int t = s.end - tail_nodes;
+    return t > s.lo ? t : s.lo;
+}
+__host__ __device__ inline int edge_tail_chunk(int nb, int b) { return nb % 8 ? 0 : b % 8; }
+DEV int edge_tail_ticket(int32_t *ctr, int lane) {
+    int t = 0;
+    if (lane == 0) t = atomicAdd(ctr, 1);
+    return __builtin_amdgcn_readfirstlane(t);
+}
+__host__ __device__ inline int edge_walk_stride(int nb, int nwaves) { return (nb % 8 ? nb : nb / 8) * nwaves; }
+inline EdgeArgs edge_args_for_grid(EdgeArgs ea, int nb, int nwaves) {
+    ea.tail_nodes = ea.tail ? ea.tail_nodes * edge_walk_stride(nb, nwaves) : 0;
+    if (!ea.tail_nodes) ea.tail = nullptr;
+    return ea;
 }
 
 constexpr int UPD_W1_KS = 3;
diff --git a/codlad_amd/csrc/edge_msg_kernel.hip b/codlad_amd/csrc/edge_msg_kernel.hip
--- a/codlad_amd/csrc/edge_msg_kernel.hip
+++ b/codlad_amd/csrc/edge_msg_kernel.hip
@@ -1,6 +1,19 @@
 #include "edge_args.h"
 
 constexpr int MSG_PAIR_U4 = 32 + 64 + 16;
+
+DEV bool msg_tail_draw(const int4 *state, int lane, int &ticket) {
+    int off = 0;
+    asm volatile("" : "+s"(off));
+    const int *t = reinterpret_cast<const int *>(state) + off;
+    const int tail_n = __builtin_amdgcn_readfirstlane(t[0]);
+    ticket = 0;
+    if (tail_n > 0) {
+        const unsigned lo32 = __builtin_amdgcn_readfirstlane(t[2]), hi32 = __builtin_amdgcn_readfirstlane(t[3]);
+        ticket = edge_tail_ticket(reinterpret_cast<int32_t *>(((unsigned long long)hi32 << 32) | lo32), lane);
+    }
+    return ticket < tail_n;
+}
 
 template <int NWAVES, bool HOISTED, int TERMS>
 __global__ __launch_bounds__(NWAVES * 64, NWAVES / 4) void msg_kernel_h(EdgeArgs a) {
@@ -21,6 +34,11 @@
             const unsigned bv = reinterpret_cast<const unsigned *>(a.b2)[tid];
             for (int q = 0; q < 4; ++q) rep[q * 128 + tid] = u32x4{bv, bv, bv, bv};
         }
+        const NodeSpan s0 = wave_node_span(a.n_nodes, NWAVES, 0, a.xcd_bounds);
+        const int lo = a.tail ? edge_tail_lo(s0, a.tail_nodes) : s0.end;
+        const unsigned long long ctr = reinterpret_cast<unsigned long long>(a.tail + edge_tail_chunk(gridDim.x, blockIdx.x));
+        if (tid == NT - 1)
+            rep[4 * 128 + NWAVES * MSG_PAIR_U4] = u32x4{(unsigned)(s0.end - lo), (unsigned)lo, (unsigned)ctr, (unsigned)(ctr >> 32)};
     }
     __syncthreads();
     const u32x4 *w1 = wl, *w2 = wl + LDS_BLOCK_U4;
@@ -30,10 +48,16 @@
     float2 *const Pslot1 = reinterpret_cast<float2 *>(consts + EDGE_CONST_U4 + NWAVES * 32 + 4 * 128 + wave * MSG_PAIR_U4);
     float4 *wait_sum = reinterpret_cast<float4 *>(Pslot1 + 64) + lane;
     int *wait_j = reinterpret_cast<int *>(Pslot1 + 64 + 2 * 64) + lane;
+    const int4 *const tail_state = reinterpret_cast<const int4 *>(consts + EDGE_CONST_U4 + NWAVES * 32 + 4 * 128 + NWAVES * MSG_PAIR_U4);
     const NodeSpan span = wave_node_span(a.n_nodes, NWAVES, wave, a.xcd_bounds);
-    const int stride = span.stride, n_end = span.end;
+    const int stride = span.stride;
     int n = __builtin_amdgcn_readfirstlane(span.first);
-    if (n >= n_end) return;
+    const int tail_lo = __builtin_amdgcn_readfirstlane(a.tail ? edge_tail_lo(span, a.tail_nodes) : span.end);
+    if (n >= tail_lo) {
+        int ticket;
+        if (!msg_tail_draw(tail_state, lane, ticket)) return;
+        n = tail_lo + ticket;
+    }
 
     const float *xsrc = HOISTED ? a.E1 : a.hE_in;
     const bool by_src = HOISTED || a.in_by_src;
@@ -57,10 +81,19 @@
     int4 ninfo = info;
     int nsrc = src, nbase = base, nK = K, njA = jA, njB = jB;
     float2 npv = {0.f, 0.f};
+    int n2 = n;
+    bool next_node = false;
     for (;;) {
-        const int n2 = n + stride;
-        const bool next_node = n2 < n_end;
         const bool first_half = half == 0;
+        if (first_half) {
+            n2 = n + stride;
+            next_node = n2 < tail_lo;
+            if (!next_node) {
+                int ticket;
+                next_node = msg_tail_draw(tail_state, lane, ticket);
+                n2 = tail_lo + ticket;
+            }
+        }
         if (first_half && next_node) ninfo = a.node_info[n2];
         {
             const float2 *pl = ((ph == 2 && c < 16) ? !cs : cs) ? Pslot1 : Pslot0;
@@ -78,9 +111,11 @@
             nK = __builtin_amdgcn_readfirstlane(ninfo.z);
             njA = a.E_idx[(size_t)nsrc * 64 + (c < nK ? c : 0)];
             njB = a.E_idx[(size_t)nsrc * 64 + (32 + c < nK ? 32 + c : 0)];
-            npv = Prows[(size_t)n2 * 64 + lane];
-        }
-        const bool open_pair = a.pair && ph == 0 && first_half && next_node && edge_pair_ok(K, nK);
+            int lane_off = lane << 3;
+            asm volatile("" : "+v"(lane_off));
+            npv = *reinterpret_cast<const float2 *>(reinterpret_cast<const char *>(Prows + (size_t)n2 * 64) + lane_off);
+        }
+        const bool open_pair = a.pair && ph == 0 && first_half && next_node && n2 < tail_lo && edge_pair_ok(K, nK);
         const bool next_half = first_half && K > 32 && !open_pair;
         const bool shared_next = ph == 1 || (open_pair && nK <= 32);
         {
@@ -194,19 +229,20 @@
 
 
 template <int TERMS>
-static void launch_msg_t(const EdgeArgs &ea, hipStream_t st) {
+static void launch_msg_t(const EdgeArgs &ea_in, hipStream_t st) {
     static bool attr_set = false;
     constexpr int NW = 8;
-    const size_t lds = 16 * (edge_lds_u4<false, NW>() + 4 * 128 + NW * MSG_PAIR_U4);
-    static_assert(16 * (edge_lds_u4<false, NW>() + 4 * 128 + NW * MSG_PAIR_U4) <= 160 * 1024, "kernel exceeds the CU's LDS");
+    const size_t lds = 16 * (edge_lds_u4<false, NW>() + 4 * 128 + NW * MSG_PAIR_U4 + 1);
+    static_assert(16 * (edge_lds_u4<false, NW>() + 4 * 128 + NW * MSG_PAIR_U4 + 1) <= 160 * 1024, "kernel exceeds the CU's LDS");
     if (!attr_set) {
         set_max_lds(reinterpret_cast<const void *>(msg_kernel_h<NW, false, TERMS>), lds);
         set_max_lds(reinterpret_cast<const void *>(msg_kernel_h<NW, true, TERMS>), lds);
         attr_set = true;
     }
-    const int groups = (ea.n_nodes + NW - 1) / NW;
+    const int groups = (ea_in.n_nodes + NW - 1) / NW;
     dim3 grid(groups < edge_cus() ? groups : edge_cus()), block(NW * 64);
     dispatch_note(grid.x);
+    const EdgeArgs ea = edge_args_for_grid(ea_in, grid.x, NW);
     if (ea.E1 != nullptr) hipLaunchKernelGGL((msg_kernel_h<NW, true, TERMS>), grid, block, lds, st, ea);
     else hipLaunchKernelGGL((msg_kernel_h<NW, false, TERMS>), grid, block, lds, st, ea);
 }
diff --git a/codlad_amd/csrc/edge_plan.hip b/codlad_amd/csrc/edge_plan.hip
--- a/codlad_amd/csrc/edge_plan.hip
+++ b/codlad_amd/csrc/edge_plan.hip
@@ -1,23 +1,26 @@
 #include "edge_args.h"
 #include <vector>
 
-static int64_t chunk_walk(const int32_t *K, int lo, int hi, int stride, bool pair, int64_t *pairs) {
+static int64_t chunk_walk(const int32_t *K, int lo, int hi, int stride, bool pair, int64_t *pairs, int tail_nodes) {
+    const int tail_lo = edge_tail_lo(NodeSpan{lo, hi, stride, lo}, tail_nodes);
     int64_t tiles = 0;
     for (int w = 0; w < stride; ++w)
-        for (int n = lo + w; n < hi; n += stride) {
+        for (int n = lo + w; n < tail_lo; n += stride) {
             tiles += K[n] > 32 ? 2 : 1;
-            if (pair && n + stride < hi && edge_pair_ok(K[n], K[n + stride])) {
+            if (pair && n + stride < tail_lo && edge_pair_ok(K[n], K[n + stride])) {
                 n += stride;
                 tiles += (K[n] > 32 ? 2 : 1) - 1;
                 if (pairs) ++*pairs;
             }
         }
+    for (int n = tail_lo; n < hi; ++n) tiles += K[n] > 32 ? 2 : 1;
     return tiles;
 }
 
-extern "C" int codlad_edge_plan_host(const int32_t *K_host, int n_nodes, int n_workgroups, int waves_per_workgroup,
-                                     int pair, int32_t *bounds_host, int64_t *stats_host) {
+extern "C" int codlad_edge_plan_tail_host(const int32_t *K_host, int n_nodes, int n_workgroups, int waves_per_workgroup,
+                                          int pair, int tail, int32_t *bounds_host, int64_t *stats_host) {
     CODLAD_REQUIRE(K_host && n_nodes > 0 && n_workgroups > 0 && waves_per_workgroup > 0, "bad arguments");
+    CODLAD_REQUIRE(tail >= 0 && tail <= CODLAD_EDGE_TAIL_MAX, "tail outside 0 .. CODLAD_EDGE_TAIL_MAX");
     int32_t bounds[9];
     const int G = XCD_BOUND_GRANULE, ng = (n_nodes + G - 1) / G;
     std::vector<int64_t> upto(ng + 1, 0);
@@ -30,7 +33,8 @@
     for (int g = 0; g < ng; ++g) upto[g + 1] += upto[g];
     const int64_t total = upto[ng];
     const bool chunked = n_workgroups % 8 == 0;
-    const int stride = chunked ? n_workgroups / 8 * waves_per_workgroup : n_workgroups * waves_per_workgroup;
+    const int stride = edge_walk_stride(n_workgroups, waves_per_workgroup);
+    const int R = tail * stride;
     auto node_of = [&](int g) { return g * G < n_nodes ? g * G : n_nodes; };
     if (pair) {
         double target = total / 16.0;
@@ -44,17 +48,17 @@
                     while (g < ng && 8 * upto[g + 1] <= total * x) ++g;
                     if (g < ng && 8 * upto[g + 1] - total * x < total * x - 8 * upto[g]) ++g;
                 } else {
-                    auto f = [&](int gg) { return (double)(done + chunk_walk(K_host, node_of(g0), node_of(gg), stride, true, nullptr)); };
+                    auto f = [&](int gg) { return (double)(done + chunk_walk(K_host, node_of(g0), node_of(gg), stride, true, nullptr, R)); };
                     const double want = target * x;
                     while (g < ng && f(g) < want) ++g;
                     while (g > g0 && f(g - 1) >= want) --g;
                     if (g > g0 && want - f(g - 1) < f(g) - want) --g;
                 }
                 bounds[x] = node_of(g);
-                if (chunked) done += chunk_walk(K_host, node_of(g0), node_of(g), stride, true, nullptr);
+                if (chunked) done += chunk_walk(K_host, node_of(g0), node_of(g), stride, true, nullptr, R);
             }
             bounds[8] = n_nodes;
-            if (chunked) target = (done + chunk_walk(K_host, bounds[7], n_nodes, stride, true, nullptr)) / 8.0;
+            if (chunked) target = (done + chunk_walk(K_host, bounds[7], n_nodes, stride, true, nullptr, R)) / 8.0;
         }
     } else {
         const int chunk = xcd_chunk_nodes(n_nodes);
@@ -67,10 +71,10 @@
         for (int x = 0; x < 8; ++x) {
             const int lo = (bounds[x] + G - 1) / G, hi = (bounds[x + 1] + G - 1) / G;
             stats_host[4 + x] = upto[hi] - upto[lo];
-            stats_host[12 + x] = chunked ? chunk_walk(K_host, bounds[x], bounds[x + 1], stride, pair != 0, &pairs) : 0;
+            stats_host[12 + x] = chunked ? chunk_walk(K_host, bounds[x], bounds[x + 1], stride, pair != 0, &pairs, R) : 0;
             walk += stats_host[12 + x];
         }
-        if (!chunked) walk = chunk_walk(K_host, 0, n_nodes, stride, pair != 0, &pairs);
+        if (!chunked) walk = chunk_walk(K_host, 0, n_nodes, stride, pair != 0, &pairs, R);
         stats_host[0] = plain;
         stats_host[1] = total;
         stats_host[2] = walk;
@@ -78,3 +82,19 @@
     }
     return 0;
 }
+
+extern "C" int codlad_edge_plan_host(const int32_t *K_host, int n_nodes, int n_workgroups, int waves_per_workgroup,
+                                     int pair, int32_t *bounds_host, int64_t *stats_host) {
+    return codlad_edge_plan_tail_host(K_host, n_nodes, n_workgroups, waves_per_workgroup, pair, 0, bounds_host, stats_host);
+}
+
+extern "C" int codlad_edge_span_host(int n_nodes, int n_workgroups, int waves_per_workgroup, int workgroup, int wave,
+                                     const int32_t *bounds_host, int tail, int32_t *out5) {
+    CODLAD_REQUIRE(out5 && n_nodes > 0 && n_workgroups > 0 && waves_per_workgroup > 0, "bad arguments");
+    CODLAD_REQUIRE(workgroup >= 0 && workgroup < n_workgroups && wave >= 0 && wave < waves_per_workgroup, "no such wave");
+    CODLAD_REQUIRE(tail >= 0 && tail <= CODLAD_EDGE_TAIL_MAX, "tail outside 0 .. CODLAD_EDGE_TAIL_MAX");
+    const NodeSpan s = node_span_of(n_nodes, waves_per_workgroup, wave, n_workgroups, workgroup, bounds_host);
+    const int tail_lo = edge_tail_lo(s, tail * edge_walk_stride(n_workgroups, waves_per_workgroup));
+    out5[0] = s.first; out5[1] = tail_lo; out5[2] = s.stride; out5[3] = tail_lo; out5[4] = s.end;
+    return 0;
+}
diff --git a/codlad_amd/csrc/edge_upd_kernel.hip b/codlad_amd/csrc/edge_upd_kernel.hip
--- a/codlad_amd/csrc/edge_upd_kernel.hip
+++ b/codlad_amd/csrc/edge_upd_kernel.hip
@@ -35,7 +35,16 @@
     const int h = lane >> 5, c = lane & 31;
     const NodeSpan span = wave_node_span(a.n_nodes, NWAVES, wave, a.xcd_bounds);
     int pend_n = -1, pend_src = 0, pend_base = 0, pend_K = 0;
-    for (int nv = span.first; nv < span.end; nv += span.stride) {
+    const int tail_lo = __builtin_amdgcn_readfirstlane(a.tail ? edge_tail_lo(span, a.tail_nodes) : span.end);
+    const int tail_n = span.end - tail_lo;
+    int32_t *const tail_ctr = a.tail + edge_tail_chunk(gridDim.x, blockIdx.x);
+    for (int nv = span.first;; nv += span.stride) {
+        if (nv >= tail_lo) {
+            if (tail_n <= 0) break;
+            const int ticket = edge_tail_ticket(tail_ctr, lane);
+            if (ticket >= tail_n) break;
+            nv = tail_lo + ticket;
+        }
         const int n = __builtin_amdgcn_readfirstlane(nv);
         const int4 info = a.node_info[n];
         const int src = __builtin_amdgcn_readfirstlane(info.x), base = __builtin_amdgcn_readfirstlane(info.y);
@@ -43,7 +52,7 @@
         const int Ku = K, lh = Ku > 32;
         const bool paired = pend_n >= 0;
         bool open_pair = false;
-        if (a.pair && !paired && Ku > 32 && Ku <= 48 && n + span.stride < span.end)
+        if (a.pair && !paired && Ku > 32 && Ku <= 48 && n + span.stride < tail_lo)
             open_pair = edge_pair_ok(Ku, __builtin_amdgcn_readfirstlane(a.node_info[n + span.stride].z));
         const bool ptA = paired && !lh, ptB = paired && lh;
         const bool lowA = ptA && c < 16, lowB = ptB && c < 16;
@@ -109,7 +118,7 @@
 
 
 template <int TERMS>
-static void launch_upd_t(const EdgeArgs &ea, hipStream_t st) {
+static void launch_upd_t(const EdgeArgs &ea_in, hipStream_t st) {
     static bool attr_set = false;
     constexpr int NW = 8;
     const size_t lds = 16 * edge_lds_u4<true, NW>();
@@ -119,9 +128,10 @@
         set_max_lds(reinterpret_cast<const void *>(upd_kernel_h<NW, true, TERMS>), lds);
         attr_set = true;
     }
-    const int groups = (ea.n_nodes + NW - 1) / NW;
+    const int groups = (ea_in.n_nodes + NW - 1) / NW;
     dim3 grid(groups < edge_cus() ? groups : edge_cus()), block(NW * 64);
     dispatch_note(grid.x);
+    const EdgeArgs ea = edge_args_for_grid(ea_in, grid.x, NW);
     if (ea.E1 != nullptr) hipLaunchKernelGGL((upd_kernel_h<NW, true, TERMS>), grid, block, lds, st, ea);
     else hipLaunchKernelGGL((upd_kernel_h<NW, false, TERMS>), grid, block, lds, st, ea);
 }
diff --git a/codlad_amd/csrc/host_util.h b/codlad_amd/csrc/host_util.h
--- a/codlad_amd/csrc/host_util.h
+++ b/codlad_amd/csrc/host_util.h
@@ -10,6 +10,7 @@
 void set_max_lds(const void *fn, size_t bytes);
 hipError_t codlad_take_attr_error();
 int option_value(int opt);
+int edge_tail_value();
 int edge_cus();
 void codlad_set_error(const char *fmt, ...);
 inline int codlad_hip_failed(const char *what, hipError_t e) {
diff --git a/codlad_amd/csrc/host_util.hip b/codlad_amd/csrc/host_util.hip
--- a/codlad_amd/csrc/host_util.hip
+++ b/codlad_amd/csrc/host_util.hip
@@ -60,6 +60,22 @@
     return 0;
 }
 
+static int g_edge_tail = -1;
+int edge_tail_value() {
+    if (g_edge_tail < 0) {
+        const char *e = getenv("CODLAD_EDGE_TAIL");
+        int v = e ? atoi(e) : 2;
+        g_edge_tail = v < 0 ? 0 : (v > CODLAD_EDGE_TAIL_MAX ? CODLAD_EDGE_TAIL_MAX : v);
+    }
+    return g_edge_tail;
+}
+extern "C" int codlad_set_edge_tail(int value) {
+    CODLAD_REQUIRE(value >= 0 && value <= CODLAD_EDGE_TAIL_MAX, "value outside 0 .. CODLAD_EDGE_TAIL_MAX");
+    g_edge_tail = value;
+    return 0;
+}
+extern "C" int codlad_edge_tail(void) { return edge_tail_value(); }
+
 int edge_cus() {
     const int v = option_value(CODLAD_OPT_EDGE_CUS);
     return v > 0 && v < num_cu() ? v : num_cu();
diff --git a/codlad_amd/engine.py b/codlad_amd/engine.py
--- a/codlad_amd/engine.py
+++ b/codlad_amd/engine.py
@@ -96,6 +96,11 @@
         ws.n_tiles = tiles.shape[0]
         self.xcd_bounds = torch.from_numpy(_lib.edge_plan(info[:, 2])[0]).to(device)
         ws.xcd_bounds = _lib.ptr(self.xcd_bounds)
+        rows = np.zeros((_lib.EDGE_TAIL_MAX + 1, 16), dtype=np.int32)
+        for t in range(_lib.EDGE_TAIL_MAX + 1):
+            rows[t, :9] = _lib.edge_plan(info[:, 2], tail=t)[0]
+        self.edge_tail = torch.empty(_lib.EDGE_TAIL_WORDS, dtype=torch.int32, device=device)
+        self.edge_tail[:_lib.EDGE_TAIL_BOUNDS_WORDS] = torch.from_numpy(rows.reshape(-1)).to(device)
         self.ws = ws
 
     def workspace_bytes(self):
@@ -107,6 +112,7 @@
         d.node_info, d.n_nodes = _lib.ptr(self.node_info), self.n_nodes
         d.E_idx, d.h_E0, d.E1, d.n_snodes = _lib.ptr(st.E_idx), _lib.ptr(st.h_E0), _lib.ptr(st.E1), st.n_snodes
         d.ws = C.pointer(self.ws)
+        d.edge_tail = _lib.ptr(self.edge_tail)
         return d
 
     def sub_job(self, members, start):
diff --git a/include/codlad_hip.h b/include/codlad_hip.h
--- a/include/codlad_hip.h
+++ b/include/codlad_hip.h
@@ -102,6 +102,10 @@
     int32_t n_tiles;
     const int32_t *xcd_bounds;
 } codlad_workspace;
+#define CODLAD_EDGE_TAIL_MAX 3
+#define CODLAD_EDGE_TAIL_SLOTS 9
+#define CODLAD_EDGE_TAIL_BOUNDS_WORDS (16 * (CODLAD_EDGE_TAIL_MAX + 1))
+#define CODLAD_EDGE_TAIL_WORDS (CODLAD_EDGE_TAIL_BOUNDS_WORDS + 8 * CODLAD_EDGE_TAIL_SLOTS)
 
 typedef struct {
     const int32_t *node_info; int n_nodes;
@@ -109,10 +113,15 @@
     const float *E1;
     int n_snodes;
     const codlad_workspace *ws;
+    int32_t *edge_tail;
 } codlad_job;
 
 int codlad_edge_plan_host(const int32_t *K_host, int n_nodes, int n_workgroups, int waves_per_workgroup, int pair,
                           int32_t *bounds_host, int64_t *stats_host);
+int codlad_edge_plan_tail_host(const int32_t *K_host, int n_nodes, int n_workgroups, int waves_per_workgroup, int pair,
+                               int tail, int32_t *bounds_host, int64_t *stats_host);
+int codlad_edge_span_host(int n_nodes, int n_workgroups, int waves_per_workgroup, int workgroup, int wave,
+                          const int32_t *bounds_host, int tail, int32_t *out5);
 
 #define CODLAD_STATUS_NONFINITE 1
 #define CODLAD_E_NONFINITE (-3)
@@ -328,6 +337,8 @@
 #define CODLAD_OPT_EDGE_PAIR 8
 #define CODLAD_N_OPTIONS 9
 int codlad_set_option(int option, int value);
+int codlad_set_edge_tail(int value);
+int codlad_edge_tail(void);
 
 int codlad_probe_edge_launches(int enable);
 int codlad_probe_read(int kind, double *total_ms);
@@ -358,6 +369,8 @@
                              int n_nodes, const int32_t *E_idx, const float *h_E0,
                              const float *mods_t, const codlad_workspace *ws, int which,
                              int layer, void *stream);
+int codlad_bench_edge_launch_job(const codlad_denoiser_weights *w, const codlad_job *job, const float *mods_t, int which,
+                                 int layer, void *stream);
 
 typedef struct {
     const float *xyz_recon, *xyz;
```

New measurement: 706.8 structures/s (median of 6 runs). No clear change (+0.5%).
